# main--/rust-lz-fear

Hardware: AMD Instinct MI355X
Metric: GiB/s compress + decompress, 4 MiB independent blocks, 1/2/4/8 MI355X (higher is better)
Workload: dtype u8

## Files before the change

rust-lz-fear_amd/build.py:

```python
import hashlib
import os
import subprocess
from concurrent.futures import ThreadPoolExecutor

PKG_DIR = os.path.dirname(os.path.abspath(__file__))
CSRC = os.path.join(PKG_DIR, "csrc")
ROOT = os.path.dirname(PKG_DIR)
LIB_PATH = os.environ.get("LZF_LIB_PATH") or os.path.join(PKG_DIR, "liblzfear_hip.so")
ANALYSIS_LIB_PATH = os.path.join(PKG_DIR, "liblzfear_hip_analysis.so")

PRODUCT_HIP = ["capi.hip", "lz4_decompress_batched.hip", "lz4_decompress_paired.hip", "lz4_decompress_seg.hip", "lz4_decompress_fed.hip", "lz4_decoded_size.hip", "lz4_compress.hip",
               "lz4_compress_compact.hip", "lz4_compress_team.hip", "aux_kernels.hip", "frame_device.hip"]
ANALYSIS_HIP = ["analysis/lz4_decompress.hip"]
CXX_SOURCES = ["frame.cpp", "host_staging.cpp"]
HEADERS = ["kernels.h", "lzf_device.h", "lz4_decompress_batch_phase.inc", "lz4_decompress_parse_phase.inc", "lz4_decompress_feed_phase.inc",
           "analysis/capi_analysis.inc",
           "lzf_copy_helpers.h", "lzf_parse_helpers.h", "lzf_compress_common.h", "lzf_simt.h", "lz4_compress_team.inc",
           "host_staging.h", "lzf_frame_scan.h", "frame_jobs.h", "lzf_frame_layout.h", "lzf_size_rules.h", "lzf_chain_step.h", "frame_deliver_body.inc",
           os.path.join(ROOT, "include", "lzfear_hip.h"), os.path.join(ROOT, "include", "lzfear_frame.h")]


def _path(d):
    return d if os.path.isabs(d) else os.path.join(CSRC, d)


def hipcc():
    for c in ("/opt/rocm/bin/hipcc", "hipcc"):
        if os.path.isabs(c) and os.path.exists(c):
            return c
    return "hipcc"


def _sources(analysis):
    return PRODUCT_HIP + (ANALYSIS_HIP if analysis else []) + CXX_SOURCES


def _newest_header():
    return max((os.path.getmtime(_path(h)) for h in HEADERS if os.path.exists(_path(h))), default=0.0)


LAST_BUILD = {}


def build_library(force=False, verbose=False, defines=(), out=None, analysis=False):
    defines = list(defines)
    if (analysis or any(d.startswith("LZF_DBG") for d in defines)) and "LZF_ANALYSIS" not in defines:
        defines.append("LZF_ANALYSIS")
    analysis = "LZF_ANALYSIS" in defines
    extra = sorted(d for d in defines if d != "LZF_ANALYSIS")
    if out is None and extra:
        out = os.path.join(PKG_DIR, "liblzfear_hip_" + hashlib.sha1(" ".join(extra).encode()).hexdigest()[:10] + ".so")
    out = out or (ANALYSIS_LIB_PATH if analysis else LIB_PATH)
    srcs_t = max([os.path.getmtime(_path(s)) for s in _sources(analysis)] + [_newest_header()])
    if not force and os.path.exists(out) and os.path.getmtime(out) >= srcs_t:
        LAST_BUILD[out] = "reused (the library is newer than every source and header)"
        if verbose:
            print(f"[build] {os.path.basename(out)}: {LAST_BUILD[out]}", flush=True)
        return out
    tag = "product" if not defines else hashlib.sha1(" ".join(sorted(defines)).encode()).hexdigest()[:12]
    objdir = os.path.join(PKG_DIR, "_obj", tag)
    os.makedirs(objdir, exist_ok=True)
    hdr_t = _newest_header()
    base = [hipcc(), "--offload-arch=gfx950", "-O3", "-std=c++17", "-fPIC", "-I", os.path.join(ROOT, "include")] + [f"-D{d}" for d in defines]
    jobs = []
    for s in _sources(analysis):
        src = _path(s)
        obj = os.path.join(objdir, os.path.splitext(os.path.basename(s))[0] + ".o")
        stale = force or not os.path.exists(obj) or os.path.getmtime(obj) < max(os.path.getmtime(src), hdr_t)
        jobs.append((src, obj, stale))
    todo = [(s, o) for s, o, st in jobs if st]

    def compile_one(so):
        cmd = base + ["-c", so[0], "-o", so[1]]
        if verbose:
            print(" ".join(cmd), flush=True)
        subprocess.check_call(cmd)

    if todo:
        with ThreadPoolExecutor(max_workers=min(len(todo), os.cpu_count() or 4)) as ex:
            list(ex.map(compile_one, todo))
    objs = [o for _, o, _ in jobs]
    if todo or not os.path.exists(out) or os.path.getmtime(out) < max(os.path.getmtime(o) for o in objs):
        cmd = [hipcc(), "--offload-arch=gfx950", "-shared", "-fPIC", "-o", out] + objs + ["-lpthread"]
        if verbose:
            print(" ".join(cmd), flush=True)
        subprocess.check_call(cmd)
    LAST_BUILD[out] = f"compiled {len(todo)} of {len(jobs)} sources with hipcc --offload-arch=gfx950, linked"
    if verbose:
        print(f"[build] {os.path.basename(out)}: {LAST_BUILD[out]}", flush=True)
    return out


DIST_LIB_PATH = os.path.join(PKG_DIR, "liblzfear_dist.so")


def build_dist_library(force=False, verbose=False):
    core = build_library(force=False, verbose=verbose)
    src = _path("dist_gather.hip")
    deps = [src, os.path.join(ROOT, "include", "lzfear_dist.h"), os.path.join(ROOT, "include", "lzfear_hip.h")]
    out = DIST_LIB_PATH
    if not force and os.path.exists(out) and os.path.getmtime(out) >= max(os.path.getmtime(d) for d in deps):
        LAST_BUILD[out] = "reused (the library is newer than every source and header)"
    else:
        cmd = [hipcc(), "--offload-arch=gfx950", "-O3", "-std=c++17", "-fPIC", "-shared", "-I", os.path.join(ROOT, "include"), "-o", out, src,
               "-L", os.path.dirname(core), "-l:" + os.path.basename(core), "-L", "/opt/rocm/lib", "-lrccl", "-Wl,-rpath,$ORIGIN", "-Wl,-rpath,/opt/rocm/lib"]
        if verbose:
            print(" ".join(cmd), flush=True)
        subprocess.check_call(cmd)
        LAST_BUILD[out] = "compiled dist_gather.hip with hipcc --offload-arch=gfx950, linked against librccl + liblzfear_hip"
    if verbose:
        print(f"[build] {os.path.basename(out)}: {LAST_BUILD[out]}", flush=True)
    return out


def build_analysis_library(force=False, verbose=False):
    return build_library(force=force, verbose=verbose, analysis=True)


if __name__ == "__main__":
    import sys
    print(build_library(force="--force" in sys.argv, verbose=True, analysis="--analysis" in sys.argv))
```

rust-lz-fear_amd/csrc/capi.hip:

```cpp
#include <hip/hip_runtime.h>
#include <cstdio>
#include <cstdlib>
#include <cstring>
#include <string>
#include <mutex>
#include <vector>
#include "kernels.h"
#include "host_staging.h"

namespace {

thread_local std::string g_last_error;
thread_local const char* g_last_decompress = "";
thread_local const char* g_last_compress = "";

int fail_hip(hipError_t e, const char* what) {
    char buf[256];
    snprintf(buf, sizeof buf, "%s: %s", what, hipGetErrorString(e));
    g_last_error = buf;
    return LZF_E_HIP;
}
#define HIP_TRY(expr)                                          \
    do {                                                       \
        hipError_t e__ = (expr);                               \
        if (e__ != hipSuccess) return fail_hip(e__, #expr);    \
    } while (0)
#define LAUNCH(...)                                            \
    do {                                                       \
        hipLaunchKernelGGL(__VA_ARGS__);                       \
        HIP_TRY(hipGetLastError());                            \
    } while (0)

int ensure_device() {
    int n = 0;
    hipError_t e = hipGetDeviceCount(&n);
    if (e != hipSuccess || n <= 0) {
        g_last_error = "no HIP device available (the lz-fear HIP codec has no CPU fallback)";
        (void)hipGetLastError();
        return LZF_E_NO_DEVICE;
    }
    return n;
}

struct Geometry { uint32_t cu, lds, wall_khz; };
const Geometry& geometry() {
    static const Geometry g = [] {
        Geometry r{256u, 160u * 1024u, 100000u};
        hipDeviceProp_t p; int dev = 0;
        if (hipGetDevice(&dev) == hipSuccess && hipGetDeviceProperties(&p, dev) == hipSuccess) {
            r.cu = (uint32_t)p.multiProcessorCount;
            if (p.maxSharedMemoryPerMultiProcessor >= 64u * 1024u) r.lds = (uint32_t)p.maxSharedMemoryPerMultiProcessor;
            int khz = 0;
            if (hipDeviceGetAttribute(&khz, hipDeviceAttributeWallClockRate, dev) == hipSuccess && khz >= 1000) r.wall_khz = (uint32_t)khz; else (void)hipGetLastError();
        } else (void)hipGetLastError();
#ifdef LZF_ANALYSIS
        if (const char* e = getenv("LZF_FAKE_CU")) { const long v = atol(e); if (v >= 1 && v <= 4096) r.cu = (uint32_t)v; }
#endif
        return r;
    }();
    return g;
}
uint32_t cu_count() { return geometry().cu; }
uint32_t per_cu(uint32_t lds_bytes) { const uint32_t n = geometry().lds / lds_bytes; return n ? n : 1u; }

inline size_t align_up(size_t v, size_t a) { return (v + a - 1) / a * a; }

struct AsyncScratch {
    void* p = nullptr; hipStream_t st = nullptr;
    ~AsyncScratch() { if (p) { (void)hipFreeAsync(p, st); } }
    hipError_t release() { void* q = p; p = nullptr; return q ? hipFreeAsync(q, st) : hipSuccess; }
};

void keep_pool_memory() {
    static thread_local int done_for = -1;
    int dev = 0;
    if (hipGetDevice(&dev) != hipSuccess || dev == done_for) return;
    hipMemPool_t pool = nullptr;
    if (hipDeviceGetDefaultMemPool(&pool, dev) == hipSuccess) {
        uint64_t keep = ~0ull;
        (void)hipMemPoolSetAttribute(pool, hipMemPoolAttrReleaseThreshold, &keep);
    }
    (void)hipGetLastError();
    done_for = dev;
}

constexpr auto k_paired48 = lzf::lzf_decompress_paired_kernel<4096, 48, 640>;
constexpr auto k_paired24 = lzf::lzf_decompress_paired_kernel<4096, 24, 384>;
constexpr auto k_staged16 = lzf::lzf_decompress_batched_kernel<4096, 16, 256, true>;
constexpr auto k_compact = lzf::lzf_compress_compact_kernel<false>;
constexpr auto k_compact_dry = lzf::lzf_compress_compact_kernel<true>;
constexpr auto k_general_u32 = lzf::lzf_compress_wave_kernel<LZF_TABLE_U32>;
constexpr auto k_general_u16 = lzf::lzf_compress_wave_kernel<LZF_TABLE_U16>;
constexpr uint32_t kTeamLds = 163840u;
constexpr uint32_t kTeamRounds = 1u;

constexpr uint32_t kSegMaxIn = 4u * 1024u * 1024u + 32u * 1024u;
constexpr uint32_t kSegMinIn = 64u * 1024u;
constexpr uint32_t kSegRingSlack = 8u * 1024u;
inline uint32_t seg_blocks_per_cu(uint32_t ring) { return per_cu(ring + kSegRingSlack); }
constexpr uint32_t kSegRankMax = 1024u;
inline uint32_t seg_max_jobs() { const uint32_t n = seg_blocks_per_cu(32768u) * cu_count(); return n < kSegRankMax ? n : kSegRankMax; }
inline uint32_t seg_ring_for(uint32_t n) {
    return n <= seg_blocks_per_cu(131072u) * cu_count() && geometry().lds >= 131072u + kSegRingSlack ? 131072u
         : n <= seg_blocks_per_cu(65536u) * cu_count() && geometry().lds >= 65536u + kSegRingSlack ? 65536u : 32768u;
}
constexpr uint64_t kSegRecsPerJob = 448u * 1024u;

struct SegScratch {
    void* base = nullptr;
    lzf::seg_ctx ctx{};
    size_t bytes = 0;
    uint32_t* est = nullptr;
};
inline uint32_t seg_nch_host(uint32_t len) { return len <= lzf::kSegChunk ? 1u : 1u + (len - lzf::kSegChunk + lzf::kSegStride - 1u) / lzf::kSegStride; }

bool seg_alloc(SegScratch& s, const lzf_decompress_job* d_jobs, lzf_job_result* d_results, uint32_t n, uint32_t min_in, hipStream_t st, uint64_t max_in_hint = ~0ull) {
    lzf::seg_ctx& c = s.ctx;
    c.jobs = d_jobs; c.results = d_results; c.n_jobs = n;
#ifdef LZF_ANALYSIS
    { static const uint32_t force = [] { const char* e = getenv("LZF_SEG_FORCE"); return !e ? 0u : !strcmp(e, "stager") ? 1u : !strcmp(e, "resolver") ? 2u : !strcmp(e, "noscratch") ? 3u : !strcmp(e, "swait") ? 8u : 0u; }();
      if (force == 3u) return false;
      c.dbg_force = force; }
#endif
    const uint32_t max_in = max_in_hint < kSegMaxIn ? (uint32_t)(max_in_hint < lzf::kSegChunk ? lzf::kSegChunk : max_in_hint) : kSegMaxIn;
    c.max_in = max_in; c.min_in = min_in;
    c.maxch = seg_nch_host(max_in);
    c.maxtile = (max_in + lzf::kSegTile - 1u) / lzf::kSegTile;
    { const uint64_t per_job = (uint64_t)max_in / 3u + 192u; c.rec_cap = (uint64_t)n * (per_job < kSegRecsPerJob ? per_job : kSegRecsPerJob); }
    c.ring_bytes = seg_ring_for(n);
#ifdef LZF_ANALYSIS
    { static const uint32_t ring = [] { const char* e = getenv("LZF_SEG_RING"); return e ? (uint32_t)atol(e) : 0u; }();
      if (ring == 32768u || ring == 65536u || ring == 131072u) c.ring_bytes = ring; }
#endif
    size_t off = 0;
    auto take = [&](size_t bytes) { const size_t o = off; off = align_up(off + bytes, 256); return o; };
    const size_t o_st = take(sizeof(lzf::seg_job) * (size_t)n);
    const size_t o_top = take(sizeof(unsigned long long));
    const size_t o_x = take(sizeof(uint32_t) * (size_t)n * c.maxch);
    const size_t o_vf = take(sizeof(uint32_t) * (size_t)n * c.maxch);
    const size_t o_tt = take(sizeof(uint32_t) * (size_t)n * c.maxtile);
    const size_t o_to = take(sizeof(uint32_t) * (size_t)n * c.maxtile);
    const size_t o_bits = take(sizeof(uint32_t) * (size_t)n * c.maxch * lzf::kSegChunkWords);
    const size_t o_recs = take(sizeof(lzf::u32x4) * (size_t)c.rec_cap);
    const size_t o_ord = take(sizeof(uint32_t) * (size_t)n);
    const size_t o_len = take(sizeof(uint32_t) * (size_t)n);
    const size_t o_est = take(sizeof(uint32_t) * (size_t)n);
    if (hipMallocAsync(&s.base, off, st) != hipSuccess) { (void)hipGetLastError(); s.base = nullptr; return false; }
    s.bytes = off;
    uint8_t* b = static_cast<uint8_t*>(s.base);
    c.st = reinterpret_cast<lzf::seg_job*>(b + o_st);
    c.rec_top = reinterpret_cast<unsigned long long*>(b + o_top);
    c.xexit = reinterpret_cast<uint32_t*>(b + o_x);
    c.vfrom = reinterpret_cast<uint32_t*>(b + o_vf);
    c.tile_tok = reinterpret_cast<uint32_t*>(b + o_tt);
    c.tile_out = reinterpret_cast<uint32_t*>(b + o_to);
    c.bits = reinterpret_cast<uint32_t*>(b + o_bits);
    c.recs = reinterpret_cast<lzf::u32x4*>(b + o_recs);
    c.n_cu = cu_count();
    c.order = (n > c.n_cu && n <= seg_max_jobs()) ? reinterpret_cast<uint32_t*>(b + o_ord) : nullptr;
    c.by_len = (n >= (c.n_cu + 7u) / 8u && n <= seg_max_jobs()) ? reinterpret_cast<uint32_t*>(b + o_len) : nullptr;
    c.rec_by_len = n >= (c.n_cu + 3u) / 4u ? 1u : 0u;
    c.g_off = 0u; c.g_n = n; c.grouped = 0u; c.res_prio = 0u; c.fed = 0u;
    s.est = reinterpret_cast<uint32_t*>(b + o_est);
    return true;
}
inline uint32_t seg_grid(uint32_t target, uint32_t n, uint32_t cap) {
    uint32_t g = target / n; if (g < 1u) g = 1u; if (g > cap) g = cap; return g;
}
int seg_launch_prep(const lzf::seg_ctx& c, hipStream_t st) {
    if (c.by_len && !c.grouped) LAUNCH(lzf::lzf_seg_by_len_kernel, dim3(1), dim3(1024), 0, st, c);
    LAUNCH(lzf::lzf_seg_plan_kernel, dim3((c.n_jobs + 255u) / 256u), dim3(256), 0, st, c);
    return LZF_OK;
}
int seg_launch_front(const lzf::seg_ctx& c, uint32_t upto, hipStream_t st) {
    const uint32_t n = c.g_n;
    uint32_t tg_parse = 1024u * c.n_cu, tg_tile = 2048u * c.n_cu;
#ifdef LZF_ANALYSIS
    { static const char* e = getenv("LZF_SEG_GRID"); if (e) { unsigned a = 0, b = 0; if (sscanf(e, "%u,%u", &a, &b) == 2 && a && b) { tg_parse = a; tg_tile = b; } } }
#endif
    if (upto >= 2) LAUNCH(lzf::lzf_seg_parse_kernel, dim3(seg_grid(tg_parse, n, c.maxch), n), dim3(64), 0, st, c);
    if (upto >= 3) LAUNCH(lzf::lzf_seg_seam_kernel, dim3(n), dim3(64), 0, st, c);
    if (upto >= 4) LAUNCH(lzf::lzf_seg_tilesum_kernel, dim3(seg_grid(tg_tile, n, c.maxtile), n), dim3(64), 0, st, c);
    if (upto >= 5) LAUNCH(lzf::lzf_seg_scan_kernel, dim3(n), dim3(64), 0, st, c);
    if (upto >= 6 && c.order) LAUNCH(lzf::lzf_seg_order_kernel, dim3(1), dim3(1024), 0, st, c);
    if (upto >= 6) LAUNCH(lzf::lzf_seg_records_kernel, dim3(seg_grid(tg_tile, n, c.maxtile), n), dim3(64), 0, st, c);
    return LZF_OK;
}
int seg_launch_records(const lzf::seg_ctx& c, hipStream_t st) {
    const uint32_t n = c.g_n;
    uint32_t tg_tile = 2048u * c.n_cu;
#ifdef LZF_ANALYSIS
    { static const char* e = getenv("LZF_SEG_GRID"); if (e) { unsigned a = 0, b = 0; if (sscanf(e, "%u,%u", &a, &b) == 2 && a && b) tg_tile = b; } }
#endif
    uint32_t pad = 0;
#ifdef LZF_ANALYSIS
    { static const uint32_t e = [] { const char* v = getenv("LZF_SEG_REC_PAD"); return v ? (uint32_t)atol(v) : 0u; }(); pad = e; }
#endif
    LAUNCH(lzf::lzf_seg_records_kernel, dim3(seg_grid(tg_tile, n, c.maxtile), n), dim3(64), pad, st, c);
    return LZF_OK;
}
int seg_launch_resolve(const lzf::seg_ctx& c, hipStream_t st) {
    const uint32_t n = c.g_n;
    if (c.ring_bytes == 131072u) LAUNCH(lzf::lzf_seg_resolve_pair_kernel<131072>, dim3(n), dim3(128), 0, st, c);
    else if (c.ring_bytes == 65536u) LAUNCH(lzf::lzf_seg_resolve_pair_kernel<65536>, dim3(n), dim3(128), 0, st, c);
    else LAUNCH(lzf::lzf_seg_resolve_pair_kernel<32768>, dim3(n), dim3(128), 0, st, c);
    return LZF_OK;
}
int seg_launch(const lzf::seg_ctx& c, uint32_t upto, hipStream_t st) {
    int rc = seg_launch_prep(c, st);
    if (rc == LZF_OK) rc = seg_launch_front(c, upto, st);
    if (rc == LZF_OK && upto >= 8) rc = seg_launch_resolve(c, st);
    return rc;
}

constexpr uint32_t kSegMaxGroups = 4;
struct SegGroups { uint32_t n = 1; uint32_t size[kSegMaxGroups] = {}; };
SegGroups seg_groups(uint32_t n_jobs) {
    SegGroups g; g.size[0] = n_jobs;
    if (n_jobs > seg_max_jobs()) return g;
    const uint32_t ncu = cu_count();
    uint32_t pct[kSegMaxGroups] = {100}; uint32_t k = 1;
    if (n_jobs >= (ncu + 7u) / 8u) { pct[0] = pct[1] = pct[2] = pct[3] = 25; k = 4; }
#ifdef LZF_ANALYSIS
    { static const char* e = getenv("LZF_SEG_GROUPS");
      if (e) { uint32_t v[kSegMaxGroups] = {}, got = 0, sum = 0; const char* q = e;
               while (got < kSegMaxGroups && *q) { char* end = nullptr; const unsigned long x = strtoul(q, &end, 10); if (end == q) break; v[got++] = (uint32_t)x; sum += (uint32_t)x; q = *end == ',' ? end + 1 : end; if (*end != ',') break; }
               if (got >= 1 && sum == 100u && v[0]) { for (uint32_t i = 0; i < kSegMaxGroups; ++i) pct[i] = v[i]; k = got; } } }
#endif
    if (k <= 1u || n_jobs < 2u * k) return g;
    uint32_t left = n_jobs; g.n = 0;
    for (uint32_t i = 0; i < k && left; ++i) {
        uint32_t sz = i + 1u == k ? left : (uint32_t)((uint64_t)n_jobs * pct[i] / 100u);
        if (sz > left) sz = left;
        if (!sz) continue;
        g.size[g.n++] = sz; left -= sz;
    }
    if (left && g.n) g.size[g.n - 1u] += left;
    return g;
}
struct SegLanes {
    std::mutex mu;
    hipStream_t s[kSegMaxGroups - 1u] = {};
    hipEvent_t front[kSegMaxGroups - 1u] = {}, done[kSegMaxGroups - 1u] = {};
    bool ok = false;
};
SegLanes* seg_lanes() {
    constexpr int kMaxDev = 64;
    static std::mutex mu;
    static SegLanes* by_dev[kMaxDev] = {};
    int dev = 0;
    if (hipGetDevice(&dev) != hipSuccess || dev < 0 || dev >= kMaxDev) { (void)hipGetLastError(); return nullptr; }
    std::lock_guard<std::mutex> lk(mu);
    if (!by_dev[dev]) {
        SegLanes* L = new SegLanes();
        int least = 0, greatest = 0;
        if (hipDeviceGetStreamPriorityRange(&least, &greatest) != hipSuccess) { (void)hipGetLastError(); least = greatest = 0; }
        bool ok = true;
        for (uint32_t i = 0; i < kSegMaxGroups - 1u && ok; ++i)
            ok = hipStreamCreateWithPriority(&L->s[i], hipStreamNonBlocking, greatest) == hipSuccess &&
                 hipEventCreateWithFlags(&L->front[i], hipEventDisableTiming) == hipSuccess &&
                 hipEventCreateWithFlags(&L->done[i], hipEventDisableTiming) == hipSuccess;
        if (!ok) (void)hipGetLastError();
        L->ok = ok;
        by_dev[dev] = L;
    }
    return by_dev[dev]->ok ? by_dev[dev] : nullptr;
}
int seg_enqueue_groups(SegScratch& s, const SegGroups& g, SegLanes& L, hipStream_t st) {
    lzf::seg_ctx c = s.ctx;
    std::lock_guard<std::mutex> lk(L.mu);
    int rc = seg_launch_prep(c, st);
    if (rc == LZF_OK) rc = seg_launch_front(c, 5u, st);
    if (rc != LZF_OK) return rc;
    static_assert(kSegMaxGroups == 4, "lzf_seg_rank_kernel takes the group sizes as a uint4");
    LAUNCH(lzf::lzf_seg_rank_kernel, dim3(1), dim3(1024), 0, st, c, s.est, make_uint4(g.size[0], g.n > 1u ? g.size[1] : 0u, g.n > 2u ? g.size[2] : 0u, g.n > 3u ? g.size[3] : 0u));
    c.by_len = s.est; c.grouped = 1u; c.res_prio = 1u;
#ifdef LZF_ANALYSIS
    { static const int pr = [] { const char* e = getenv("LZF_SEG_PRIO"); return e ? atoi(e) : 1; }(); c.res_prio = pr ? 1u : 0u; }
#endif
    uint32_t off = 0, forked = 0;
    const uint32_t ticks_per_us = geometry().wall_khz / 1000u;
    uint32_t pause_ticks = 10u * ticks_per_us;
#ifdef LZF_ANALYSIS
    { static const int us = [] { const char* e = getenv("LZF_SEG_PAUSE_US"); return e ? atoi(e) : -1; }(); if (us >= 0) pause_ticks = (uint32_t)us * ticks_per_us; }
#endif
    for (uint32_t k = 0; k < g.n && rc == LZF_OK; ++k) {
        c.g_off = off; c.g_n = g.size[k]; off += g.size[k];
        rc = seg_launch_records(c, st);
        if (rc != LZF_OK) break;
        if (k + 1u < g.n) {
            if (hipEventRecord(L.front[k], st) != hipSuccess || hipStreamWaitEvent(L.s[k], L.front[k], 0) != hipSuccess) { (void)hipGetLastError(); rc = LZF_E_HIP; break; }
            rc = seg_launch_resolve(c, L.s[k]);
            ++forked;
            if (pause_ticks) LAUNCH(lzf::lzf_seg_pause_kernel, dim3(1), dim3(64), 0, st, pause_ticks);
            if (hipEventRecord(L.done[k], L.s[k]) != hipSuccess) { (void)hipGetLastError(); --forked; if (rc == LZF_OK) rc = LZF_E_HIP; if (hipStreamSynchronize(L.s[k]) != hipSuccess) (void)hipGetLastError(); }
        } else {
            rc = seg_launch_resolve(c, st);
        }
    }
    for (uint32_t k = 0; k < forked; ++k)
        if (hipStreamWaitEvent(st, L.done[k], 0) != hipSuccess) { (void)hipGetLastError(); if (hipStreamSynchronize(L.s[k]) != hipSuccess) (void)hipGetLastError(); if (rc == LZF_OK) rc = LZF_E_HIP; }
    return rc;
}
int seg_launch_grouped(SegScratch& s, const SegGroups& g, SegLanes& L, hipStream_t st) {
    const int rc = seg_enqueue_groups(s, g, L, st);
    if (rc != LZF_OK)
        for (uint32_t k = 0; k < kSegMaxGroups - 1u; ++k) if (hipStreamSynchronize(L.s[k]) != hipSuccess) (void)hipGetLastError();
    return rc;
}
int seg_decompress(const lzf_decompress_job* d_jobs, lzf_job_result* d_results, uint32_t n, uint32_t min_in, hipStream_t st, bool* used, uint64_t max_in_hint, uint32_t* ring_used) {
    SegScratch s;
    *used = false; *ring_used = 0u;
    if (max_in_hint < min_in) return LZF_OK;
    if (!seg_alloc(s, d_jobs, d_results, n, min_in, st, max_in_hint)) return LZF_OK;
    *used = true; *ring_used = s.ctx.ring_bytes;
    const SegGroups g = seg_groups(n);
    SegLanes* lanes = g.n > 1u ? seg_lanes() : nullptr;
    int rc = lanes ? seg_launch_grouped(s, g, *lanes, st) : seg_launch(s.ctx, 8u, st);
    if (rc == LZF_OK) {
        hipLaunchKernelGGL(k_paired48, dim3(n), dim3(128), 0, st, d_jobs, d_results, n, (const uint32_t*)nullptr, (const lzf::seg_job*)s.ctx.st);
        if (hipGetLastError() != hipSuccess) rc = LZF_E_HIP;
    }
    if (hipFreeAsync(s.base, st) != hipSuccess && rc == LZF_OK) rc = LZF_E_HIP;
    if (rc != LZF_OK) g_last_error = "segmented decompress: launch failed";
    return rc;
}

constexpr auto k_fed32 = lzf::lzf_decompress_fed_kernel<4096, 32, 352>;
constexpr uint32_t kFedMinInDefault = 65536u;
constexpr uint64_t kFedMinHint = 262144u;
inline uint32_t fed_min_in() {
#ifdef LZF_ANALYSIS
    static const long v = [] { const char* e = getenv("LZF_FED_MIN_IN"); return e ? atol(e) : -1L; }();
    if (v >= 0) return (uint32_t)v;
#endif
    return kFedMinInDefault;
}
inline uint64_t fed_min_hint() {
#ifdef LZF_ANALYSIS
    static const bool open_ = getenv("LZF_FED_MIN_IN") != nullptr;
    if (open_) return 0u;
#endif
    return kFedMinHint;
}
constexpr uint64_t kFedMaxScratch = 24ull << 30;
constexpr uint32_t kFedMaxJobs = 65535u;
constexpr uint32_t kFedLdsAlloc = 6400u;
constexpr uint32_t kFedWavesPerCu = 4u * (LZF_FED_WAVES > 0 ? (uint32_t)LZF_FED_WAVES : 5u);
struct FedGeometry { uint32_t slots, xcc_mask; };
FedGeometry fed_geometry(hipStream_t st) {
    constexpr int kMaxDev = 64;
    static std::mutex mu;
    static FedGeometry by_dev[kMaxDev] = {};
    int dev = 0;
    if (hipGetDevice(&dev) != hipSuccess || dev < 0 || dev >= kMaxDev) { (void)hipGetLastError(); return FedGeometry{8u * cu_count(), 0u}; }
    std::lock_guard<std::mutex> lk(mu);
    if (by_dev[dev].slots) return by_dev[dev];
    FedGeometry answer{0u, 0u};
    uint32_t* d = nullptr;
    if (hipMalloc(&d, 4u * sizeof(uint32_t)) == hipSuccess) {
        const uint32_t init[4] = {0u, 0xFFFFFFFFu, 0u, 0u};
        lzf::fed_args a{}; a.census = d;
        if (hipMemcpyAsync(d, init, sizeof init, hipMemcpyHostToDevice, st) == hipSuccess) {
            hipLaunchKernelGGL(k_fed32, dim3(40u * cu_count()), dim3(64), 0, st, a);
            uint32_t got[4] = {0, 0, 0, 0};
            if (hipGetLastError() == hipSuccess && hipMemcpyAsync(got, d, sizeof got, hipMemcpyDeviceToHost, st) == hipSuccess && hipStreamSynchronize(st) == hipSuccess &&
                got[1] != 0xFFFFFFFFu && got[1] >= cu_count()) { answer.slots = got[1]; answer.xcc_mask = got[2]; }
        }
        (void)hipFree(d);
    }
    (void)hipGetLastError();
    if (!answer.slots) {
        const uint32_t by_lds = per_cu(kFedLdsAlloc);
        answer.slots = (by_lds < kFedWavesPerCu ? by_lds : kFedWavesPerCu) * cu_count();
    }
#ifdef LZF_ANALYSIS
    if (getenv("LZF_FED_VERBOSE")) fprintf(stderr, "[lzf] bitmap-fed kernel: %u workgroups resident at once (%u compute units), XCD mask 0x%x\n", answer.slots, cu_count(), answer.xcc_mask);
#endif
    by_dev[dev] = answer;
    return answer;
}
struct FedCall {
    SegScratch s; const lzf_decompress_job* jobs = nullptr; lzf_job_result* res = nullptr; uint32_t n = 0; const uint32_t* perm = nullptr;
    size_t o_tick = 0, o_fst = 0; bool live = false;
};
int fed_front(FedCall& f, const lzf_decompress_job* d_jobs, lzf_job_result* d_results, uint32_t n, const uint32_t* perm, hipStream_t st, uint64_t max_in_hint) {
    f.jobs = d_jobs; f.res = d_results; f.n = n; f.perm = perm; f.live = false;
    lzf::seg_ctx& c = f.s.ctx;
    c = lzf::seg_ctx{};
    c.jobs = d_jobs; c.results = d_results; c.n_jobs = n;
    const uint32_t max_in = max_in_hint < kSegMaxIn ? (uint32_t)(max_in_hint < lzf::kSegChunk ? lzf::kSegChunk : max_in_hint) : kSegMaxIn;
    c.max_in = max_in; c.min_in = fed_min_in();
    c.maxch = seg_nch_host(max_in);
    c.maxtile = (max_in + lzf::kSegTile - 1u) / lzf::kSegTile;
    c.n_cu = cu_count();
    c.g_off = 0u; c.g_n = n; c.fed = 1u;
    size_t off = 0;
    auto take = [&](size_t bytes) { const size_t o = off; off = align_up(off + bytes, 256); return o; };
    const size_t o_st = take(sizeof(lzf::seg_job) * (size_t)n);
    const size_t o_top = take(sizeof(unsigned long long));
    const size_t o_x = take(sizeof(uint32_t) * (size_t)n * c.maxch);
    const size_t o_vf = take(sizeof(uint32_t) * (size_t)n * c.maxch);
    const size_t o_bits = take(sizeof(uint32_t) * (size_t)n * c.maxch * lzf::kSegChunkWords);
    f.o_tick = take(sizeof(uint32_t) * 32u * lzf::kFedTicketStride);
    f.o_fst = take(sizeof(lzf::fed_state) * (size_t)n);
    if (off > kFedMaxScratch) return LZF_OK;
    if (hipMallocAsync(&f.s.base, off, st) != hipSuccess) { (void)hipGetLastError(); f.s.base = nullptr; return LZF_OK; }
    uint8_t* b = static_cast<uint8_t*>(f.s.base);
    c.st = reinterpret_cast<lzf::seg_job*>(b + o_st);
    c.rec_top = reinterpret_cast<unsigned long long*>(b + o_top);
    c.xexit = reinterpret_cast<uint32_t*>(b + o_x);
    c.vfrom = reinterpret_cast<uint32_t*>(b + o_vf);
    c.bits = reinterpret_cast<uint32_t*>(b + o_bits);
    f.live = true;
    const int rc = seg_launch(c, 3u, st);
    if (rc != LZF_OK) { (void)hipFreeAsync(f.s.base, st); f.s.base = nullptr; f.live = false; g_last_error = "bitmap-fed decompress: launch failed"; }
    return rc;
}
int fed_back(FedCall& f, hipStream_t st, uint32_t slots_per_cu) {
    if (!f.live) return LZF_OK;
    lzf::seg_ctx& c = f.s.ctx;
    const uint32_t n = f.n;
    uint8_t* b = static_cast<uint8_t*>(f.s.base);
    const FedGeometry fg = fed_geometry(st);
    uint32_t slots = fg.slots;
    if (slots_per_cu && slots_per_cu * cu_count() < slots) slots = slots_per_cu * cu_count();
    uint32_t pieces = n > slots && fg.xcc_mask ? 16u : 1u;
    uint32_t pad = 0;
#ifdef LZF_ANALYSIS
    { static const long e = [] { const char* v = getenv("LZF_FED_PIECES"); return v ? atol(v) : 0L; }(); if (e >= 1 && e <= 4096) pieces = (uint32_t)e; }
    { static const long e = [] { const char* v = getenv("LZF_FED_SLOTS"); return v ? atol(v) : 0L; }(); if (e > 0 && !slots_per_cu) slots = (uint32_t)e * cu_count(); }
    { static const uint32_t e = [] { const char* v = getenv("LZF_FED_PAD_LDS"); return v ? (uint32_t)atol(v) : 0u; }(); pad = e; }
#endif
    if ((uint64_t)n * pieces > 0xFFFFFFF0ull) pieces = 1u;
    if (!fg.xcc_mask) pieces = 1u;
    int rc = LZF_OK;
    lzf::fed_args a{f.jobs, f.res, c.st, c.bits, c.vfrom, f.perm, reinterpret_cast<lzf::fed_state*>(b + f.o_fst), reinterpret_cast<uint32_t*>(b + f.o_tick), fg.xcc_mask ? fg.xcc_mask : 1u, n, c.maxch, pieces, nullptr};
    hipLaunchKernelGGL(lzf::lzf_fed_reset_kernel, dim3((n + 255u) / 256u), dim3(256), 0, st, a);
    hipLaunchKernelGGL(k_fed32, dim3(slots < n ? slots : n), dim3(64), pad, st, a);
    if (hipGetLastError() != hipSuccess) rc = LZF_E_HIP;
    if (rc == LZF_OK) {
        hipLaunchKernelGGL(k_paired24, dim3(n), dim3(128), 0, st, f.jobs, f.res, n, f.perm, (const lzf::seg_job*)c.st);
        if (hipGetLastError() != hipSuccess) rc = LZF_E_HIP;
    }
    if (hipFreeAsync(f.s.base, st) != hipSuccess && rc == LZF_OK) rc = LZF_E_HIP;
    f.s.base = nullptr; f.live = false;
    if (rc != LZF_OK) g_last_error = "bitmap-fed decompress: launch failed";
    return rc;
}
int fed_decompress(const lzf_decompress_job* d_jobs, lzf_job_result* d_results, uint32_t n, const uint32_t* perm, hipStream_t st, bool* used, uint64_t max_in_hint) {
    *used = false;
    if (n > kFedMaxJobs || max_in_hint <= fed_min_in() || max_in_hint <= fed_min_hint()) return LZF_OK;
    FedCall f;
    int rc = fed_front(f, d_jobs, d_results, n, perm, st, max_in_hint);
    if (rc != LZF_OK || !f.live) return rc;
    *used = true;
    return fed_back(f, st, 0u);
}

#ifdef LZF_ANALYSIS
#include "analysis/capi_analysis.inc"
#endif

}

extern "C" {

int lzf_abi_version(void) { return LZFEAR_ABI_VERSION; }
const char* lzf_last_error(void) { return g_last_error.c_str(); }
const char* lzf_last_decompress_launch(void) { return g_last_decompress; }
const char* lzf_last_compress_launch(void) { return g_last_compress; }
int lzf_device_count(void) { return ensure_device(); }

int lzf_compress_batch(const lzf_compress_job* d_jobs, lzf_job_result* d_results, uint32_t n_jobs,
                       uint32_t table_kinds, void* hip_stream) {
    if (n_jobs == 0) return LZF_OK;
    if (!d_jobs || !d_results) { g_last_error = "lzf_compress_batch: NULL job/result array"; return LZF_E_INVALID; }
    int rc = ensure_device();
    if (rc < 0) return rc;
    hipStream_t st = static_cast<hipStream_t>(hip_stream);
    keep_pool_memory();
    if ((table_kinds & (LZF_KINDS_U32 | LZF_KINDS_U16)) == 0) table_kinds |= LZF_KINDS_U32 | LZF_KINDS_U16;
    uint32_t use_compact = 1u, use_order = 1u;
    uint32_t team_max = geometry().lds >= kTeamLds ? kTeamRounds * cu_count() : 0u;
#ifdef LZF_ANALYSIS
    { static const uint32_t which = [] { const char* e = getenv("LZF_COMPRESS_KERNEL"); return !e ? 0u : !strcmp(e, "general") ? 1u : !strcmp(e, "compact") ? 3u : 0u; }();
      static const uint32_t order = analysis_order("LZF_COMPRESS_ORDER");
      use_compact = which == 1u ? 0u : 1u; use_order = order;
      static const long tm = [] { const char* e = getenv("LZF_COMPRESS_TEAM_MAX"); return e ? atol(e) : -1L; }();
      if (tm >= 0 && geometry().lds >= kTeamLds) team_max = (uint32_t)tm;
      if (which != 0u) team_max = 0u; }
#endif
    const bool use_team = use_compact && n_jobs <= team_max;
    const bool fresh_only = use_compact && (table_kinds & LZF_KINDS_U32_FRESH_ONLY);
    uint32_t* perm = nullptr;
    AsyncScratch scratch_owner; scratch_owner.st = st;
    void*& scratch = scratch_owner.p;
    const bool want_order = use_order && use_compact && (table_kinds & LZF_KINDS_U32) && (use_order == 2u || n_jobs > per_cu(lzf::kCompactLdsBytes) * cu_count() || (fresh_only && n_jobs > 4u * cu_count()));
    uint32_t piece = 65536u, parts = 1u;
#ifdef LZF_ANALYSIS
    { static const char* e = getenv("LZF_PROBE"); if (e) { unsigned a = 0, b = 0; if (sscanf(e, "%u,%u", &a, &b) == 2 && a >= 4096u && b >= 1u && b <= 16u) { piece = a; parts = b; } } }
#endif
    const size_t n_probes = want_order ? (size_t)n_jobs * parts : 0u;
    const size_t probes_off = 256;
    const size_t res_off = probes_off + align_up(sizeof(lzf_compress_job) * n_probes, 256);
    const size_t perm_off = res_off + align_up(sizeof(lzf_job_result) * n_probes, 256);
    if (want_order) {
        if (hipMallocAsync(&scratch, perm_off + sizeof(uint32_t) * (want_order ? (size_t)n_jobs : 0u), st) != hipSuccess) { (void)hipGetLastError(); scratch = nullptr; }
    }
    if (scratch && want_order) {
        lzf_compress_job* probes = reinterpret_cast<lzf_compress_job*>(static_cast<uint8_t*>(scratch) + probes_off);
        lzf_job_result* pres = reinterpret_cast<lzf_job_result*>(static_cast<uint8_t*>(scratch) + res_off);
        perm = reinterpret_cast<uint32_t*>(static_cast<uint8_t*>(scratch) + perm_off);
        LAUNCH(lzf::lzf_cost_probe_jobs_kernel, dim3((uint32_t)((n_probes + 255u) / 256u)), dim3(256), 0, st, d_jobs, probes, n_jobs, piece, parts);
        LAUNCH(k_compact_dry, dim3((uint32_t)n_probes), dim3(64), 0, st, probes, pres, (uint32_t)n_probes, (const uint32_t*)nullptr, 0u);
        LAUNCH(lzf::lzf_order_by_cost_kernel, dim3(1), dim3(1024), 0, st, d_jobs, pres, perm, n_jobs, piece, parts);
    }
    if (table_kinds & LZF_KINDS_U32) {
#ifdef LZF_DBG_DRY_MAIN
        if (use_compact) LAUNCH(k_compact_dry, dim3(n_jobs), dim3(64), 0, st, d_jobs, d_results, n_jobs, (const uint32_t*)perm, 0u);
#else
        if (use_team) {
            LAUNCH(lzf::lzf_compress_team_kernel, dim3(n_jobs), dim3(192), 0, st, d_jobs, d_results, n_jobs, (const uint32_t*)perm, fresh_only ? 1u : 0u);
            if (!fresh_only) LAUNCH(lzf::lzf_compress_team_carry_kernel, dim3(n_jobs), dim3(192), 0, st, d_jobs, d_results, n_jobs, (const uint32_t*)perm);
        }
        else if (use_compact) {
            uint32_t pad = 0;
#ifdef LZF_ANALYSIS
            { static const uint32_t e = [] { const char* v = getenv("LZF_COMPACT_PAD_LDS"); return v ? (uint32_t)atol(v) : 0u; }(); pad = e; }
#endif
            LAUNCH(k_compact, dim3(n_jobs), dim3(64), pad, st, d_jobs, d_results, n_jobs, (const uint32_t*)perm, fresh_only ? 1u : 0u);
        }
#endif
        if (!fresh_only) LAUNCH(k_general_u32, dim3(n_jobs), dim3(64), 0, st, d_jobs, d_results, n_jobs, use_team ? 2u : use_compact, (const uint32_t*)perm);
    }
    if (table_kinds & LZF_KINDS_U16)
        LAUNCH(k_general_u16, dim3(n_jobs), dim3(64), 0, st, d_jobs, d_results, n_jobs, 0u, (const uint32_t*)perm);
    g_last_compress = !(table_kinds & LZF_KINDS_U32) ? "lzf_compress_wave_kernel<U16>"
                    : !use_compact ? "lzf_compress_wave_kernel (analysis: general)"
                    : use_team ? (fresh_only ? "lzf_compress_team_kernel" : "lzf_compress_team_kernel + lzf_compress_team_carry_kernel + lzf_compress_wave_kernel")
                               : (fresh_only ? "lzf_compress_compact_kernel" : "lzf_compress_compact_kernel + lzf_compress_wave_kernel");
    HIP_TRY(scratch_owner.release());
    return LZF_OK;
}

int lzf_decompress_batch(const lzf_decompress_job* d_jobs, lzf_job_result* d_results, uint32_t n_jobs, void* hip_stream) {
    return lzf_decompress_batch_sized(d_jobs, d_results, n_jobs, ~0ull, hip_stream);
}

int lzf_decompress_batch_sized(const lzf_decompress_job* d_jobs, lzf_job_result* d_results, uint32_t n_jobs, uint64_t max_input_len, void* hip_stream) {
    if (n_jobs == 0) return LZF_OK;
    if (!d_jobs || !d_results) { g_last_error = "lzf_decompress_batch: NULL job/result array"; return LZF_E_INVALID; }
    int rc = ensure_device();
    if (rc < 0) return rc;
    hipStream_t st = static_cast<hipStream_t>(hip_stream);
    keep_pool_memory();
    uint32_t use_order = 1u;
    bool perm_ok = true;
#ifdef LZF_ANALYSIS
    const int forced = analysis_decompress_variant();
    { static const uint32_t order = analysis_order("LZF_DECOMPRESS_ORDER"); use_order = order; }
    if (forced != kVariantAuto) perm_ok = analysis_perm_ok(forced);
#endif
    AsyncScratch perm_owner; perm_owner.st = st;
    uint32_t* perm = nullptr;
    if (perm_ok && (use_order == 2u || (use_order == 1u && n_jobs > per_cu(20u * 1024u) * cu_count()))) {
        if (hipMallocAsync(&perm_owner.p, 2u * sizeof(uint32_t) * (size_t)n_jobs, st) != hipSuccess) { (void)hipGetLastError(); perm_owner.p = nullptr; }
        perm = static_cast<uint32_t*>(perm_owner.p);
        if (perm) {
            uint32_t* const est = perm + n_jobs;
            uint32_t len_shift = 2u;
#ifdef LZF_ANALYSIS
            { static const uint32_t k = [] { const char* e = getenv("LZF_ORDER_LEN_SHIFT"); return e ? (uint32_t)atol(e) : 2u; }(); len_shift = k; }
#endif
            LAUNCH(lzf::lzf_decompress_cost_kernel, dim3(n_jobs), dim3(64), 0, st, d_jobs, n_jobs, est, len_shift);
            LAUNCH(lzf::lzf_order_by_estimate_kernel, dim3(1), dim3(1024), 0, st, (const uint32_t*)est, perm, n_jobs);
        }
    }
    const uint32_t* cperm = perm;
#ifdef LZF_ANALYSIS
    if (forced != kVariantAuto) {
        g_last_decompress = "analysis variant (LZF_DECOMPRESS_KERNEL)";
        rc = analysis_launch_decompress(forced, d_jobs, d_results, n_jobs, cperm, st);
        HIP_TRY(perm_owner.release());
        return rc;
    }
#endif
    uint32_t seg_min_in = kSegMinIn; bool seg_on = n_jobs <= seg_max_jobs();
#ifdef LZF_ANALYSIS
    { static const int mode = [] { const char* e = getenv("LZF_DECOMPRESS_KERNEL"); return !e ? 0 : !strcmp(e, "seg") ? 1 : (!strcmp(e, "noseg") || !strcmp(e, "fed")) ? 2 : 0; }();
      static const uint32_t min_in = [] { const char* e = getenv("LZF_SEG_MIN_IN"); return e ? (uint32_t)atol(e) : 0u; }();
      if (mode == 1) { seg_on = true; seg_min_in = min_in; }
      if (mode == 2) seg_on = false; }
#endif
    if (seg_on) {
        bool used = false; uint32_t ring = 0;
        rc = seg_decompress(d_jobs, d_results, n_jobs, seg_min_in, st, &used, max_input_len, &ring);
        if (used) g_last_decompress = ring == 131072u ? "segmented: lzf_seg_resolve_pair_kernel<131072> + lzf_decompress_paired_kernel<4096,48,640>"
                                     : ring == 65536u ? "segmented: lzf_seg_resolve_pair_kernel<65536> + lzf_decompress_paired_kernel<4096,48,640>"
                                                      : "segmented: lzf_seg_resolve_pair_kernel<32768> + lzf_decompress_paired_kernel<4096,48,640>";
        if (rc != LZF_OK || used) { HIP_TRY(perm_owner.release()); return rc; }
    }
    const uint32_t resident48 = per_cu(20u * 1024u) * cu_count();
    const uint32_t resident24 = per_cu(12800u) * cu_count();
    bool fed_on = n_jobs > resident24;
#ifdef LZF_ANALYSIS
    { static const int mode = [] { const char* e = getenv("LZF_DECOMPRESS_KERNEL"); return !e ? 0 : !strcmp(e, "fed") ? 1 : !strcmp(e, "nofed") ? 2 : 0; }();
      if (mode == 1) fed_on = true;
      if (mode == 2) fed_on = false; }
#endif
    if (fed_on) {
        bool used = false;
        rc = fed_decompress(d_jobs, d_results, n_jobs, cperm, st, &used, max_input_len);
        if (used) g_last_decompress = "bitmap-fed: lzf_seg_parse_kernel + lzf_decompress_fed_kernel<4096,32,352> + lzf_decompress_paired_kernel<4096,24,384>";
        if (rc != LZF_OK || used) { HIP_TRY(perm_owner.release()); return rc; }
    }
    g_last_decompress = n_jobs <= resident48 ? "lzf_decompress_paired_kernel<4096,48,640>" : n_jobs <= 8u * resident48 ? "lzf_decompress_paired_kernel<4096,24,384>"
                                                                                                             : "lzf_decompress_batched_kernel<4096,16,256,staged>";
    if (n_jobs <= resident48)
        LAUNCH(k_paired48, dim3(n_jobs), dim3(128), 0, st, d_jobs, d_results, n_jobs, cperm, (const lzf::seg_job*)nullptr);
    else if (n_jobs <= 8u * resident48)
        LAUNCH(k_paired24, dim3(n_jobs), dim3(128), 0, st, d_jobs, d_results, n_jobs, cperm, (const lzf::seg_job*)nullptr);
    else
        LAUNCH(k_staged16, dim3(n_jobs), dim3(64), 0, st, d_jobs, d_results, n_jobs, cperm);
    HIP_TRY(perm_owner.release());
    return LZF_OK;
}

int lzf_decompressed_size_batch(const lzf_decompress_job* d_jobs, lzf_job_result* d_results, uint32_t n_jobs, uint64_t max_input_len, void* hip_stream) {
    (void)max_input_len;
    if (n_jobs == 0) return LZF_OK;
    if (!d_jobs || !d_results) { g_last_error = "lzf_decompressed_size_batch: NULL job/result array"; return LZF_E_INVALID; }
    int rc = ensure_device();
    if (rc < 0) return rc;
    hipStream_t st = static_cast<hipStream_t>(hip_stream);
    keep_pool_memory();
    constexpr auto k_size = lzf::lzf_decoded_size_kernel<48, 768>;
    static thread_local int resident_for = -1; static thread_local uint32_t resident = 0;
    int dev = 0;
    HIP_TRY(hipGetDevice(&dev));
    if (dev != resident_for) {
        int per = 0;
        HIP_TRY(hipOccupancyMaxActiveBlocksPerMultiprocessor(&per, k_size, 64, 0));
        resident = per > 0 ? (uint32_t)per : 1u; resident_for = dev;
    }
    const uint64_t room = (uint64_t)resident * cu_count();
    const bool ordered = n_jobs > room;
    AsyncScratch ticket; ticket.st = st;
    HIP_TRY(hipMallocAsync(&ticket.p, 256 + (ordered ? sizeof(uint32_t) * (size_t)n_jobs : 0u), st));
    HIP_TRY(hipMemsetAsync(ticket.p, 0, 4, st));
    uint32_t* const perm = ordered ? static_cast<uint32_t*>(ticket.p) + 64 : nullptr;
    if (ordered) LAUNCH(lzf::lzf_order_by_input_len_kernel, dim3(1), dim3(1024), 0, st, d_jobs, perm, n_jobs);
    const uint32_t grid = n_jobs < room ? n_jobs : (uint32_t)room;
    LAUNCH(k_size, dim3(grid), dim3(64), 0, st, d_jobs, d_results, n_jobs, static_cast<uint32_t*>(ticket.p), (const uint32_t*)perm);
    HIP_TRY(ticket.release());
    return LZF_OK;
}

int lzf_table_seed_from_dictionary(lzf_u32_table* d_table, const uint8_t* d_dict, uint64_t dict_len, void* hip_stream) {
    if (!d_table || (!d_dict && dict_len)) { g_last_error = "lzf_table_seed_from_dictionary: NULL argument"; return LZF_E_INVALID; }
    if (dict_len > 0xFFFFFFFFull) { g_last_error = "dictionary beyond u32 positions (reference panics, mod.rs:67)"; return LZF_E_INVALID; }
    int rc = ensure_device();
    if (rc < 0) return rc;
    hipStream_t st = static_cast<hipStream_t>(hip_stream);
    HIP_TRY(hipMemsetAsync(d_table, 0, sizeof(lzf_u32_table), st));
    if (dict_len >= 8) {
        const uint64_t count = (dict_len - 8) / 3 + 1;
        uint32_t blocks = (uint32_t)((count + 255) / 256);
        if (blocks > 1024) blocks = 1024;
        hipLaunchKernelGGL(lzf::lzf_seed_table_kernel, dim3(blocks), dim3(256), 0, st, d_table, d_dict, dict_len);
        HIP_TRY(hipGetLastError());
    }
    return LZF_OK;
}

int lzf_table_offset(void* d_table, uint32_t table_kind, uint64_t add, void* hip_stream) {
    if (!d_table || table_kind > LZF_TABLE_U16) { g_last_error = "lzf_table_offset: bad argument"; return LZF_E_INVALID; }
    int rc = ensure_device();
    if (rc < 0) return rc;
    hipLaunchKernelGGL(lzf::lzf_table_offset_kernel, dim3(1), dim3(64), 0, static_cast<hipStream_t>(hip_stream), d_table, table_kind, add);
    HIP_TRY(hipGetLastError());
    return LZF_OK;
}

int lzf_table_offset_batch(void* const* d_tables, const uint64_t* d_adds, uint32_t n, uint32_t table_kind, void* hip_stream) {
    if (n == 0) return LZF_OK;
    if (!d_tables || !d_adds || table_kind > LZF_TABLE_U16) { g_last_error = "lzf_table_offset_batch: bad argument"; return LZF_E_INVALID; }
    int rc = ensure_device();
    if (rc < 0) return rc;
    hipLaunchKernelGGL(lzf::lzf_table_offset_batch_kernel, dim3((n + 255u) / 256u), dim3(256), 0, static_cast<hipStream_t>(hip_stream), d_tables, d_adds, n, table_kind);
    HIP_TRY(hipGetLastError());
    return LZF_OK;
}

int lzf_chain_decompress_step(const lzf_chain_step* d_steps, lzf_chain_state* d_state, uint32_t n_streams,
                              lzf_decompress_job* d_jobs, const lzf_job_result* d_results, void* hip_stream) {
    if (n_streams == 0) return LZF_OK;
    if (!d_steps || !d_state || !d_jobs || !d_results) { g_last_error = "lzf_chain_decompress_step: NULL argument"; return LZF_E_INVALID; }
    int rc = ensure_device();
    if (rc < 0) return rc;
    hipLaunchKernelGGL(lzf::lzf_chain_decompress_step_kernel, dim3(n_streams), dim3(256), 0, static_cast<hipStream_t>(hip_stream), d_steps, d_state, n_streams, d_jobs, d_results);
    HIP_TRY(hipGetLastError());
    return LZF_OK;
}

int lzf_copy_ranges(const uint8_t* const* d_src, uint8_t* const* d_dst, const uint64_t* d_len, uint32_t n, uint64_t max_len, void* hip_stream) {
    if (n == 0 || max_len == 0) return LZF_OK;
    if (!d_src || !d_dst || !d_len) { g_last_error = "lzf_copy_ranges: NULL argument"; return LZF_E_INVALID; }
    int rc = ensure_device();
    if (rc < 0) return rc;
    const uint64_t pieces = (max_len + 65535ull) / 65536ull;
    if (pieces > 0x7FFFFFFFull) { g_last_error = "lzf_copy_ranges: max_len too large"; return LZF_E_INVALID; }
    for (uint32_t base = 0; base < n; base += 65535u) {
        const uint32_t cnt = n - base < 65535u ? n - base : 65535u;
        hipLaunchKernelGGL(lzf::lzf_copy_ranges_kernel, dim3((uint32_t)pieces, cnt), dim3(256), 0, static_cast<hipStream_t>(hip_stream),
                           d_src + base, d_dst + base, d_len + base, cnt);
    }
    HIP_TRY(hipGetLastError());
    return LZF_OK;
}

int lzf_xxh32_batch(const uint8_t* const* d_ptrs, const uint64_t* d_lens, uint32_t* d_out, uint32_t n, void* hip_stream) {
    if (n == 0) return LZF_OK;
    if (!d_ptrs || !d_lens || !d_out) { g_last_error = "lzf_xxh32_batch: NULL argument"; return LZF_E_INVALID; }
    int rc = ensure_device();
    if (rc < 0) return rc;
    if (n <= 8192u) hipLaunchKernelGGL(lzf::lzf_xxh32_wave_kernel, dim3(n), dim3(64), 0, static_cast<hipStream_t>(hip_stream), d_ptrs, d_lens, d_out, n);
    else hipLaunchKernelGGL(lzf::lzf_xxh32_kernel, dim3((n + 15) / 16), dim3(64), 0, static_cast<hipStream_t>(hip_stream), d_ptrs, d_lens, d_out, n);
    HIP_TRY(hipGetLastError());
    return LZF_OK;
}

#ifdef LZF_ANALYSIS
int lzf_debug_seg(const lzf_decompress_job* d_jobs, lzf_job_result* d_results, uint32_t n, uint32_t min_in, uint32_t upto,
                  void* h_state, void* h_bits, void* h_xexit, void* h_vfrom, void* h_tile_tok, void* h_tile_out, void* h_recs, uint64_t recs_bytes,
                  uint32_t* geom) {
    int rc = ensure_device();
    if (rc < 0) return rc;
    SegScratch s;
    if (!seg_alloc(s, d_jobs, d_results, n, min_in, nullptr)) return LZF_E_HIP;
    const lzf::seg_ctx& c = s.ctx;
    rc = seg_launch(c, upto, nullptr);
    HIP_TRY(hipDeviceSynchronize());
    if (geom) { geom[0] = c.maxch; geom[1] = c.maxtile; geom[2] = lzf::kSegChunkWords; geom[3] = (uint32_t)c.rec_cap; }
    if (h_state) HIP_TRY(hipMemcpy(h_state, c.st, sizeof(lzf::seg_job) * n, hipMemcpyDeviceToHost));
    if (h_bits) HIP_TRY(hipMemcpy(h_bits, c.bits, sizeof(uint32_t) * (size_t)n * c.maxch * lzf::kSegChunkWords, hipMemcpyDeviceToHost));
    if (h_xexit) HIP_TRY(hipMemcpy(h_xexit, c.xexit, sizeof(uint32_t) * (size_t)n * c.maxch, hipMemcpyDeviceToHost));
    if (h_vfrom) HIP_TRY(hipMemcpy(h_vfrom, c.vfrom, sizeof(uint32_t) * (size_t)n * c.maxch, hipMemcpyDeviceToHost));
    if (h_tile_tok) HIP_TRY(hipMemcpy(h_tile_tok, c.tile_tok, sizeof(uint32_t) * (size_t)n * c.maxtile, hipMemcpyDeviceToHost));
    if (h_tile_out) HIP_TRY(hipMemcpy(h_tile_out, c.tile_out, sizeof(uint32_t) * (size_t)n * c.maxtile, hipMemcpyDeviceToHost));
    if (h_recs) { uint64_t nb = sizeof(lzf::u32x4) * c.rec_cap; if (nb > recs_bytes) nb = recs_bytes; HIP_TRY(hipMemcpy(h_recs, c.recs, nb, hipMemcpyDeviceToHost)); }
    HIP_TRY(hipFree(s.base));
    return rc;
}
#endif

int lzf_compress_batch_host(const lzf_compress_job* jobs, lzf_job_result* results, uint32_t n_jobs) {
    if (n_jobs == 0) return LZF_OK;
    if (!jobs || !results) { g_last_error = "lzf_compress_batch_host: NULL argument"; return LZF_E_INVALID; }
    int rc = ensure_device();
    if (rc < 0) return rc;
    using lzf_host::Seg; using lzf_host::Staging;
    std::vector<size_t> in_off(n_jobs), out_off(n_jobs), tab_off(n_jobs);
    size_t in_total = 0, out_total = 0;
    uint32_t kinds = 0;
    std::vector<Seg> up;
    static_assert(sizeof(lzf_u32_table) == sizeof(lzf_u16_table), "table structs share a slab slot size");
    for (uint32_t i = 0; i < n_jobs; ++i) {
        if (jobs[i].table_kind > LZF_TABLE_U16) { g_last_error = "bad table_kind"; return LZF_E_INVALID; }
        kinds |= jobs[i].table_kind == LZF_TABLE_U32 ? LZF_KINDS_U32 : LZF_KINDS_U16;
        in_off[i] = in_total; in_total = align_up(in_total + jobs[i].input_len, 256);
        if (jobs[i].input_len) up.push_back({in_off[i], const_cast<uint8_t*>(jobs[i].input), (size_t)jobs[i].input_len});
    }
    for (uint32_t i = 0; i < n_jobs; ++i) {
        tab_off[i] = in_total;
        if (jobs[i].table) { up.push_back({tab_off[i], static_cast<uint8_t*>(jobs[i].table), sizeof(lzf_u32_table)}); in_total = align_up(in_total + sizeof(lzf_u32_table), 256); }
    }
    for (uint32_t i = 0; i < n_jobs; ++i) { out_off[i] = out_total; out_total = align_up(out_total + jobs[i].out_cap, 256); }
    Staging& sg = Staging::get();
    std::lock_guard<std::mutex> guard(sg.lock());
    hipStream_t cs = sg.stream(0);
    uint8_t* const din = static_cast<uint8_t*>(sg.device(0, in_total));
    uint8_t* const dout = static_cast<uint8_t*>(sg.device(1, out_total));
    lzf_compress_job* const djobs = static_cast<lzf_compress_job*>(sg.device(3, sizeof(lzf_compress_job) * n_jobs));
    lzf_job_result* const dres = static_cast<lzf_job_result*>(sg.device(4, sizeof(lzf_job_result) * n_jobs));
    if (!cs || !din || !dout || !djobs || !dres || !sg.pinned(in_total > out_total ? in_total : out_total)) return fail_hip(hipErrorOutOfMemory, "staging memory");
    std::vector<lzf_compress_job> dj(jobs, jobs + n_jobs);
    for (uint32_t i = 0; i < n_jobs; ++i) {
        dj[i].input = din + in_off[i];
        dj[i].out = dout + out_off[i];
        if (jobs[i].table) dj[i].table = din + tab_off[i];
    }
    HIP_TRY(sg.upload(up, in_total, din));
    HIP_TRY(hipMemcpyAsync(djobs, dj.data(), sizeof(lzf_compress_job) * n_jobs, hipMemcpyHostToDevice, cs));
    HIP_TRY(sg.join_copies(cs));
    rc = lzf_compress_batch(djobs, dres, n_jobs, kinds, cs);
    if (rc != LZF_OK) { (void)hipDeviceSynchronize(); return rc; }
    HIP_TRY(hipMemcpyAsync(results, dres, sizeof(lzf_job_result) * n_jobs, hipMemcpyDeviceToHost, cs));
    HIP_TRY(hipStreamSynchronize(cs));
    std::vector<Seg> down;
    for (uint32_t i = 0; i < n_jobs; ++i) {
        if (results[i].status == LZF_OK && results[i].out_len) down.push_back({out_off[i], jobs[i].out, (size_t)results[i].out_len});
        if (jobs[i].table && !(jobs[i].flags & LZF_CJOB_TABLE_READONLY) && results[i].status != LZF_CONTRACT)
            HIP_TRY(hipMemcpyAsync(jobs[i].table, din + tab_off[i], sizeof(lzf_u32_table), hipMemcpyDeviceToHost, cs));
    }
    HIP_TRY(sg.download(down, out_total, dout, cs));
    HIP_TRY(hipStreamSynchronize(cs));
    return LZF_OK;
}

int lzf_decompress_batch_host(const lzf_decompress_job* jobs, lzf_job_result* results, uint32_t n_jobs) {
    if (n_jobs == 0) return LZF_OK;
    if (!jobs || !results) { g_last_error = "lzf_decompress_batch_host: NULL argument"; return LZF_E_INVALID; }
    int rc = ensure_device();
    if (rc < 0) return rc;
    using lzf_host::Seg; using lzf_host::Staging;
    std::vector<size_t> in_off(n_jobs), pre_off(n_jobs), out_off(n_jobs);
    size_t in_total = 0, out_total = 0;
    std::vector<Seg> up, up_out;
    for (uint32_t i = 0; i < n_jobs; ++i) {
        if (jobs[i].out_existing_len > jobs[i].out_cap) { g_last_error = "out_existing_len > out_cap"; return LZF_E_INVALID; }
        in_off[i] = in_total; in_total = align_up(in_total + jobs[i].input_len, 256);
        if (jobs[i].input_len) up.push_back({in_off[i], const_cast<uint8_t*>(jobs[i].input), (size_t)jobs[i].input_len});
    }
    for (uint32_t i = 0; i < n_jobs; ++i) {
        pre_off[i] = in_total; in_total = align_up(in_total + jobs[i].prefix_len, 256);
        if (jobs[i].prefix_len) up.push_back({pre_off[i], const_cast<uint8_t*>(jobs[i].prefix), (size_t)jobs[i].prefix_len});
    }
    for (uint32_t i = 0; i < n_jobs; ++i) {
        out_off[i] = out_total; out_total = align_up(out_total + jobs[i].out_cap, 256);
        if (jobs[i].out_existing_len) up_out.push_back({out_off[i], jobs[i].out, (size_t)jobs[i].out_existing_len});
    }
    Staging& sg = Staging::get();
    std::lock_guard<std::mutex> guard(sg.lock());
    hipStream_t cs = sg.stream(0);
    uint8_t* const din = static_cast<uint8_t*>(sg.device(0, in_total));
    uint8_t* const dout = static_cast<uint8_t*>(sg.device(1, out_total));
    lzf_decompress_job* const djobs = static_cast<lzf_decompress_job*>(sg.device(3, sizeof(lzf_decompress_job) * n_jobs));
    lzf_job_result* const dres = static_cast<lzf_job_result*>(sg.device(4, sizeof(lzf_job_result) * n_jobs));
    if (!cs || !din || !dout || !djobs || !dres || !sg.pinned(in_total > out_total ? in_total : out_total)) return fail_hip(hipErrorOutOfMemory, "staging memory");
    std::vector<lzf_decompress_job> dj(jobs, jobs + n_jobs);
    for (uint32_t i = 0; i < n_jobs; ++i) {
        dj[i].input = din + in_off[i];
        dj[i].prefix = din + pre_off[i];
        dj[i].out = dout + out_off[i];
    }
    if (!up_out.empty()) {
        HIP_TRY(sg.upload(up_out, out_total, dout));
        HIP_TRY(sg.join_copies(cs));
        HIP_TRY(hipStreamSynchronize(cs));
    }
    HIP_TRY(sg.upload(up, in_total, din));
    HIP_TRY(hipMemcpyAsync(djobs, dj.data(), sizeof(lzf_decompress_job) * n_jobs, hipMemcpyHostToDevice, cs));
    HIP_TRY(sg.join_copies(cs));
    uint64_t max_in = 0;
    for (uint32_t i = 0; i < n_jobs; ++i) if (jobs[i].input_len > max_in) max_in = jobs[i].input_len;
    rc = lzf_decompress_batch_sized(djobs, dres, n_jobs, max_in, cs);
    if (rc != LZF_OK) { (void)hipDeviceSynchronize(); return rc; }
    HIP_TRY(hipMemcpyAsync(results, dres, sizeof(lzf_job_result) * n_jobs, hipMemcpyDeviceToHost, cs));
    HIP_TRY(hipStreamSynchronize(cs));
    std::vector<Seg> down;
    for (uint32_t i = 0; i < n_jobs; ++i) {
        uint64_t n = results[i].out_len;
        if (n > jobs[i].out_cap) n = jobs[i].out_cap;
        if (n > jobs[i].out_existing_len)
            down.push_back({out_off[i] + (size_t)jobs[i].out_existing_len, jobs[i].out + jobs[i].out_existing_len, (size_t)(n - jobs[i].out_existing_len)});
    }
    HIP_TRY(sg.download(down, out_total, dout, cs));
    return LZF_OK;
}

int lzf_decompressed_size_batch_host(const lzf_decompress_job* jobs, lzf_job_result* results, uint32_t n_jobs) {
    if (n_jobs == 0) return LZF_OK;
    if (!jobs || !results) { g_last_error = "lzf_decompressed_size_batch_host: NULL argument"; return LZF_E_INVALID; }
    int rc = ensure_device();
    if (rc < 0) return rc;
    using lzf_host::Seg; using lzf_host::Staging;
    std::vector<size_t> in_off(n_jobs);
    size_t in_total = 0;
    uint64_t max_in = 0;
    std::vector<Seg> up;
    for (uint32_t i = 0; i < n_jobs; ++i) {
        in_off[i] = in_total; in_total = align_up(in_total + jobs[i].input_len, 256);
        if (jobs[i].input_len) {
            if (!jobs[i].input) { g_last_error = "lzf_decompressed_size_batch_host: NULL input"; return LZF_E_INVALID; }
            up.push_back({in_off[i], const_cast<uint8_t*>(jobs[i].input), (size_t)jobs[i].input_len});
        }
        if (jobs[i].input_len > max_in) max_in = jobs[i].input_len;
    }
    Staging& sg = Staging::get();
    std::lock_guard<std::mutex> guard(sg.lock());
    hipStream_t cs = sg.stream(0);
    uint8_t* const din = static_cast<uint8_t*>(sg.device(0, in_total ? in_total : 256));
    lzf_decompress_job* const djobs = static_cast<lzf_decompress_job*>(sg.device(3, sizeof(lzf_decompress_job) * n_jobs));
    lzf_job_result* const dres = static_cast<lzf_job_result*>(sg.device(4, sizeof(lzf_job_result) * n_jobs));
    if (!cs || !din || !djobs || !dres || !sg.pinned(in_total ? in_total : 256)) return fail_hip(hipErrorOutOfMemory, "staging memory");
    std::vector<lzf_decompress_job> dj(jobs, jobs + n_jobs);
    for (uint32_t i = 0; i < n_jobs; ++i) dj[i].input = din + in_off[i];
    HIP_TRY(sg.upload(up, in_total, din));
    HIP_TRY(hipMemcpyAsync(djobs, dj.data(), sizeof(lzf_decompress_job) * n_jobs, hipMemcpyHostToDevice, cs));
    HIP_TRY(sg.join_copies(cs));
    rc = lzf_decompressed_size_batch(djobs, dres, n_jobs, max_in, cs);
    if (rc != LZF_OK) { (void)hipDeviceSynchronize(); return rc; }
    HIP_TRY(hipMemcpyAsync(results, dres, sizeof(lzf_job_result) * n_jobs, hipMemcpyDeviceToHost, cs));
    HIP_TRY(hipStreamSynchronize(cs));
    return LZF_OK;
}

int lzf_table_replace_host(void* table, uint32_t table_kind, const uint8_t* input, uint64_t input_len, uint64_t pos, uint64_t* previous) {
    if (!table || (!input && input_len) || table_kind > LZF_TABLE_U16) { g_last_error = "lzf_table_replace_host: bad argument"; return LZF_E_INVALID; }
    if (pos > input_len) return LZF_CONTRACT;
    const uint64_t rem = input_len - pos;
    if (table_kind == LZF_TABLE_U32) {
        lzf_u32_table* t = static_cast<lzf_u32_table*>(table);
        const uint64_t o = pos + t->offset;
        if (o > 0xFFFFFFFFull || o < pos) return LZF_CONTRACT;
        uint64_t v = 0;
        if (rem >= 8) memcpy(&v, input + pos, 8);
        const uint32_t slot = (uint32_t)(((v << 24) * 889523592379ull) >> 52);
        const uint32_t old = t->dict[slot];
        t->dict[slot] = (uint32_t)o;
        if (previous) *previous = old > t->offset ? old - t->offset : 0;
    } else {
        lzf_u16_table* t = static_cast<lzf_u16_table*>(table);
        const uint64_t o = pos + t->offset;
        if (o > 0xFFFFull || o < pos) return LZF_CONTRACT;
        if (rem < 4) return LZF_CONTRACT;
        uint32_t v; memcpy(&v, input + pos, 4);
        const uint32_t slot = (uint32_t)(v * 2654435761u) >> 19;
        const uint16_t old = t->dict[slot];
        t->dict[slot] = (uint16_t)o;
        if (previous) *previous = old > t->offset ? old - t->offset : 0;
    }
    return LZF_OK;
}

int lzf_table_offset_host(void* table, uint32_t table_kind, uint64_t add) {
    if (!table || table_kind > LZF_TABLE_U16) { g_last_error = "lzf_table_offset_host: bad argument"; return LZF_E_INVALID; }
    if (table_kind == LZF_TABLE_U32) static_cast<lzf_u32_table*>(table)->offset += add;
    else static_cast<lzf_u16_table*>(table)->offset += add;
    return LZF_OK;
}

int lzf_compress2_host_writer(const uint8_t* input, uint64_t input_len, uint64_t cursor, void* table, uint32_t table_kind,
                              lzf_write_all_fn write_all, void* ctx, int* writer_error) {
    if ((!input && input_len) || !write_all || table_kind > LZF_TABLE_U16) { g_last_error = "lzf_compress2_host_writer: bad argument"; return LZF_E_INVALID; }
    if (writer_error) *writer_error = 0;
    const uint64_t payload = cursor < input_len ? input_len - cursor : 0;
    const uint64_t bound = payload + payload / 255 + 16;
    std::vector<uint8_t> out(bound);
    static_assert(sizeof(lzf_u32_table) == sizeof(lzf_u16_table), "one scratch copy serves both table kinds");
    std::vector<uint8_t> t0(sizeof(lzf_u32_table), 0), t1;
    if (table) memcpy(t0.data(), table, t0.size());
    t1 = t0;
    lzf_compress_job job{};
    job.input = input; job.input_len = input_len; job.cursor = cursor;
    job.out = out.data(); job.out_cap = bound; job.table = table ? t1.data() : nullptr; job.table_kind = table_kind;
    lzf_job_result res{};
    int rc = lzf_compress_batch_host(&job, &res, 1);
    if (rc != LZF_OK) return rc;
    if (res.status != LZF_OK) return res.status;
    const uint8_t* p = out.data();
    const uint8_t* const end = p + res.out_len;
    int werr = 0;
    auto put = [&](const uint8_t* d, size_t n) -> bool { if (n == 0) return true; werr = write_all(ctx, d, n); return werr == 0; };
    auto put_tail = [&](const uint8_t*& q) -> bool {
        size_t k = 0; while (q[k] == 0xFF) ++k;
        for (size_t i = 0; i < k / 4; ++i) { if (!put(q, 4)) return false; q += 4; }
        for (size_t i = 0; i < k % 4; ++i) { if (!put(q, 1)) return false; q += 1; }
        if (!put(q, 1)) return false;
        q += 1;
        return true;
    };
    bool refused = false;
    const uint8_t* group = p;
    while (p < end && !refused) {
        group = p;
        const uint8_t tok = *p;
        const uint8_t* q = p + 1;
        if (!put(p, 1)) { refused = true; break; }
        size_t L = tok >> 4;
        if (L == 15) { const uint8_t* t = q; while (*t == 0xFF) { L += 255; ++t; } L += *t; if (!put_tail(q)) { refused = true; break; } }
        if (!put(q, L)) { refused = true; break; }
        q += L;
        if (q >= end) { p = q; break; }
        if (!put(q, 2)) { refused = true; break; }
        q += 2;
        if ((tok & 15) == 15) { if (!put_tail(q)) { refused = true; break; } }
        p = q;
    }
    if (!refused) {
        if (table) memcpy(table, t1.data(), t1.size());
        return LZF_OK;
    }
    if (writer_error) *writer_error = werr;
    if (table) {
        const uint8_t* q = group; const uint8_t tok = *q++; size_t L = tok >> 4;
        if (L == 15) { while (*q == 0xFF) { L += 255; ++q; } L += *q++; }
        q += L;
        if (q < end) { q += 2; if ((tok & 15) == 15) { while (*q == 0xFF) ++q; ++q; } }
        const uint64_t gsize = (uint64_t)(q - group);
        t1 = t0;
        job.out_cap = (uint64_t)(group - out.data()) + gsize - 1;
        job.table = t1.data();
        rc = lzf_compress_batch_host(&job, &res, 1);
        if (rc != LZF_OK) return rc;
        memcpy(table, t1.data(), t1.size());
    }
    return LZF_OUTPUT_FULL;
}

int lzf_xxh32_batch_host(const uint8_t* const* ptrs, const uint64_t* lens, uint32_t* out, uint32_t n) {
    if (n == 0) return LZF_OK;
    if (!ptrs || !lens || !out) { g_last_error = "lzf_xxh32_batch_host: NULL argument"; return LZF_E_INVALID; }
    int rc = ensure_device();
    if (rc < 0) return rc;
    using lzf_host::Seg; using lzf_host::Staging;
    std::vector<Seg> up; std::vector<const uint8_t*> dp(n);
    size_t total = 0;
    for (uint32_t i = 0; i < n; ++i) { if (lens[i]) up.push_back({total, const_cast<uint8_t*>(ptrs[i]), (size_t)lens[i]}); dp[i] = reinterpret_cast<const uint8_t*>(total); total = align_up(total + lens[i], 256); }
    Staging& sg = Staging::get();
    std::lock_guard<std::mutex> guard(sg.lock());
    hipStream_t cs = sg.stream(0);
    uint8_t* const din = static_cast<uint8_t*>(sg.device(0, total));
    const size_t lp = 0, ll = align_up(sizeof(void*) * n, 256), lo = ll + align_up(sizeof(uint64_t) * n, 256);
    uint8_t* const dl = static_cast<uint8_t*>(sg.device(5, lo + sizeof(uint32_t) * n));
    if (!cs || !din || !dl || !sg.pinned(total)) return fail_hip(hipErrorOutOfMemory, "staging memory");
    for (uint32_t i = 0; i < n; ++i) dp[i] = din + reinterpret_cast<size_t>(dp[i]);
    HIP_TRY(sg.upload(up, total, din));
    HIP_TRY(hipMemcpyAsync(dl + lp, dp.data(), sizeof(void*) * n, hipMemcpyHostToDevice, cs));
    HIP_TRY(hipMemcpyAsync(dl + ll, lens, sizeof(uint64_t) * n, hipMemcpyHostToDevice, cs));
    HIP_TRY(sg.join_copies(cs));
    rc = lzf_xxh32_batch(reinterpret_cast<const uint8_t* const*>(dl + lp), reinterpret_cast<const uint64_t*>(dl + ll), reinterpret_cast<uint32_t*>(dl + lo), n, cs);
    if (rc != LZF_OK) { (void)hipDeviceSynchronize(); return rc; }
    HIP_TRY(hipMemcpyAsync(out, dl + lo, sizeof(uint32_t) * n, hipMemcpyDeviceToHost, cs));
    HIP_TRY(hipStreamSynchronize(cs));
    return LZF_OK;
}

}
```

rust-lz-fear_amd/csrc/kernels.h:

```cpp
#pragma once
#include "lzf_device.h"

namespace lzf {
#ifdef LZF_ANALYSIS
__global__ void lzf_decompress_wave_kernel(const lzf_decompress_job* __restrict__ jobs,
                                           lzf_job_result* __restrict__ results, uint32_t n_jobs, const uint32_t* __restrict__ perm);
#endif
template <int RING, int S, int TOKCAP, bool STAGE>
__global__ __launch_bounds__(64) void lzf_decompress_batched_kernel(const lzf_decompress_job* __restrict__ jobs,
                                              lzf_job_result* __restrict__ results, uint32_t n_jobs, const uint32_t* __restrict__ perm);
#ifdef LZF_ANALYSIS
#define LZF_DECOMPRESS_VARIANTS(X) \
    X(staged16, 4096, 16, 256, true)    \
    X(staged32, 4096, 32, 512, true)    \
    X(direct4w, 4096, 256, 2048, false)
#else
#define LZF_DECOMPRESS_VARIANTS(X) X(staged16, 4096, 16, 256, true)
#endif
#define LZF_EXT(NAME, R, S_, T, ST) extern template __global__ void lzf_decompress_batched_kernel<R, S_, T, ST>(const lzf_decompress_job*, lzf_job_result*, uint32_t, const uint32_t*);
LZF_DECOMPRESS_VARIANTS(LZF_EXT)
#undef LZF_EXT
template <int S, int TOKCAP>
__global__ __launch_bounds__(64) void lzf_decoded_size_kernel(const lzf_decompress_job* __restrict__ jobs, lzf_job_result* __restrict__ results,
                                                              uint32_t n_jobs, uint32_t* __restrict__ ticket, const uint32_t* __restrict__ perm);
extern template __global__ void lzf_decoded_size_kernel<48, 768>(const lzf_decompress_job*, lzf_job_result*, uint32_t, uint32_t*, const uint32_t*);
struct seg_job;
template <int RING, int S, int TOKCAP>
__global__ __launch_bounds__(128) void lzf_decompress_paired_kernel(const lzf_decompress_job* __restrict__ jobs, lzf_job_result* __restrict__ results, uint32_t n_jobs,
                                             const uint32_t* __restrict__ perm, const seg_job* __restrict__ done);
#ifdef LZF_ANALYSIS
#define LZF_PAIRED_VARIANTS(X) \
    X(paired16, 4096, 16, 256) \
    X(paired24, 4096, 24, 384) \
    X(paired48, 4096, 48, 640) \
    X(paired128, 4096, 128, 1280) \
    X(paired256, 4096, 256, 2048)
#else
#define LZF_PAIRED_VARIANTS(X) \
    X(paired24, 4096, 24, 384) \
    X(paired48, 4096, 48, 640)
#endif
#define LZF_EXTP(NAME, RG, S_, T) extern template __global__ void lzf_decompress_paired_kernel<RG, S_, T>(const lzf_decompress_job*, lzf_job_result*, uint32_t, const uint32_t*, const seg_job*);
LZF_PAIRED_VARIANTS(LZF_EXTP)
#undef LZF_EXTP
struct seg_job {
    uint32_t eligible, failed, done, nch;
    uint32_t ntile, ntok, outb, pad;
    uint64_t rec_off;
    uint64_t pad2;
};
struct seg_ctx {
    const lzf_decompress_job* jobs;
    lzf_job_result* results;
    seg_job* st;
    uint32_t* bits;
    uint32_t* xexit;
    uint32_t* vfrom;
    uint32_t* tile_tok;
    uint32_t* tile_out;
    u32x4* recs;
    unsigned long long* rec_top;
    uint64_t rec_cap;
    uint32_t n_jobs, maxch, maxtile, max_in, min_in;
    uint32_t ring_bytes;
    uint32_t* order;
    uint32_t n_cu;
    uint32_t* by_len;
    uint32_t rec_by_len;
    uint32_t dbg_force;
    uint32_t g_off, g_n, grouped;
    uint32_t res_prio;
    uint32_t fed;
};
struct fed_state { uint32_t flag, cstart, expect, o; };
constexpr uint32_t kFedEnded = 0x80000000u;
constexpr uint32_t kFedTicketStride = 32u;
struct fed_args {
    const lzf_decompress_job* jobs;
    lzf_job_result* results;
    seg_job* st;
    const uint32_t* bits;
    const uint32_t* vfrom;
    const uint32_t* perm;
    fed_state* state;
    uint32_t* ticket;
    uint32_t xcc_mask;
    uint32_t n_jobs, maxch;
    uint32_t pieces;
    uint32_t* census;
};
__global__ void lzf_fed_reset_kernel(fed_args a);
#define LZF_FED_VARIANTS(X) X(fed32, 4096, 32, 352)
#ifdef LZF_DBG_FED_WAVES
#define LZF_FED_WAVES LZF_DBG_FED_WAVES
#else
#define LZF_FED_WAVES 6
#endif
#if LZF_FED_WAVES > 0
#define LZF_FED_BOUNDS __launch_bounds__(64, LZF_FED_WAVES)
#else
#define LZF_FED_BOUNDS __launch_bounds__(64)
#endif
template <int RING, int W, int TOKCAP>
__global__ LZF_FED_BOUNDS void lzf_decompress_fed_kernel(fed_args a);
#define LZF_EXTF(NAME, RG, W_, T) extern template __global__ void lzf_decompress_fed_kernel<RG, W_, T>(fed_args);
LZF_FED_VARIANTS(LZF_EXTF)
#undef LZF_EXTF
__device__ __forceinline__ uint32_t seg_job_of(const seg_ctx& c, uint32_t i) { return c.by_len ? c.by_len[i + c.g_off] : i + c.g_off; }
constexpr uint32_t kSegRegion = 256, kSegChunk = 64u * kSegRegion, kSegOverlap = 2048, kSegStride = kSegChunk - kSegOverlap;
constexpr uint32_t kSegChunkWords = kSegChunk / 32u, kSegTile = 2048;
__global__ void lzf_seg_plan_kernel(seg_ctx c);
__global__ void lzf_seg_order_kernel(seg_ctx c);
__global__ void lzf_seg_pause_kernel(uint32_t ticks);
__global__ void lzf_seg_rank_kernel(seg_ctx c, uint32_t* __restrict__ by_tok, uint4 group_sizes);
__global__ void lzf_seg_by_len_kernel(seg_ctx c);
__global__ void lzf_seg_parse_kernel(seg_ctx c);
__global__ void lzf_seg_seam_kernel(seg_ctx c);
__global__ void lzf_seg_tilesum_kernel(seg_ctx c);
__global__ void lzf_seg_scan_kernel(seg_ctx c);
__global__ void lzf_seg_records_kernel(seg_ctx c);
template <int R>
__global__ __launch_bounds__(128) void lzf_seg_resolve_pair_kernel(seg_ctx c);
extern template __global__ void lzf_seg_resolve_pair_kernel<32768>(seg_ctx);
extern template __global__ void lzf_seg_resolve_pair_kernel<65536>(seg_ctx);
extern template __global__ void lzf_seg_resolve_pair_kernel<131072>(seg_ctx);
template <int KIND>
__global__ __launch_bounds__(64) void lzf_compress_wave_kernel(const lzf_compress_job* __restrict__ jobs,
                                         lzf_job_result* __restrict__ results, uint32_t n_jobs, uint32_t skip_compact,
                                         const uint32_t* __restrict__ perm);
extern template __global__ void lzf_compress_wave_kernel<LZF_TABLE_U32>(const lzf_compress_job*, lzf_job_result*, uint32_t, uint32_t, const uint32_t*);
extern template __global__ void lzf_compress_wave_kernel<LZF_TABLE_U16>(const lzf_compress_job*, lzf_job_result*, uint32_t, uint32_t, const uint32_t*);
constexpr uint32_t kCompactLdsBytes = (4096u / 2u + 4096u / 32u + 64u) * 4u;
template <bool DRY>
__global__ __launch_bounds__(64) void lzf_compress_compact_kernel(const lzf_compress_job* __restrict__ jobs,
                                            lzf_job_result* __restrict__ results, uint32_t n_jobs, const uint32_t* __restrict__ perm,
                                            uint32_t alone);
extern template __global__ void lzf_compress_compact_kernel<false>(const lzf_compress_job*, lzf_job_result*, uint32_t, const uint32_t*, uint32_t);
extern template __global__ void lzf_compress_compact_kernel<true>(const lzf_compress_job*, lzf_job_result*, uint32_t, const uint32_t*, uint32_t);
__global__ void lzf_compress_team_kernel(const lzf_compress_job* __restrict__ jobs, lzf_job_result* __restrict__ results, uint32_t n_jobs,
                                         const uint32_t* __restrict__ perm, uint32_t alone);
__global__ void lzf_compress_team_carry_kernel(const lzf_compress_job* __restrict__ jobs, lzf_job_result* __restrict__ results, uint32_t n_jobs, const uint32_t* __restrict__ perm);
__global__ void lzf_cost_probe_jobs_kernel(const lzf_compress_job* __restrict__ jobs, lzf_compress_job* __restrict__ probes, uint32_t n,
                                           uint32_t piece, uint32_t parts);
__global__ void lzf_order_by_input_len_kernel(const lzf_decompress_job* __restrict__ jobs, uint32_t* __restrict__ perm, uint32_t n);
__global__ void lzf_decompress_cost_kernel(const lzf_decompress_job* __restrict__ jobs, uint32_t n, uint32_t* __restrict__ est, uint32_t len_shift);
__global__ void lzf_order_by_estimate_kernel(const uint32_t* __restrict__ est, uint32_t* __restrict__ perm, uint32_t n);
__global__ void lzf_order_by_cost_kernel(const lzf_compress_job* __restrict__ jobs, const lzf_job_result* __restrict__ probe_results,
                                         uint32_t* __restrict__ perm, uint32_t n, uint32_t piece, uint32_t parts);
__global__ void lzf_xxh32_kernel(const uint8_t* const* __restrict__ ptrs, const uint64_t* __restrict__ lens,
                                 uint32_t* __restrict__ out, uint32_t n);
__global__ void lzf_xxh32_wave_kernel(const uint8_t* const* __restrict__ ptrs, const uint64_t* __restrict__ lens,
                                      uint32_t* __restrict__ out, uint32_t n);
__global__ void lzf_copy_ranges_kernel(const uint8_t* const* __restrict__ src, uint8_t* const* __restrict__ dst,
                                       const uint64_t* __restrict__ len, uint32_t n);
__global__ void lzf_seed_table_kernel(lzf_u32_table* __restrict__ t, const uint8_t* __restrict__ dict, uint64_t dict_len);
__global__ void lzf_table_offset_kernel(void* table, uint32_t kind, uint64_t add);
__global__ void lzf_table_offset_batch_kernel(void* const* __restrict__ tables, const uint64_t* __restrict__ adds, uint32_t n, uint32_t kind);
__global__ void lzf_chain_decompress_step_kernel(const lzf_chain_step* __restrict__ steps, lzf_chain_state* __restrict__ state, uint32_t n,
                                                 lzf_decompress_job* __restrict__ jobs, const lzf_job_result* __restrict__ results);
}
```

rust-lz-fear_amd/csrc/lz4_decompress_fed.hip:

```cpp
#include "lzf_device.h"
#include "kernels.h"
#include "lzf_copy_helpers.h"

namespace lzf {

__device__ __forceinline__ uint32_t xcc_id() {
    uint32_t v; asm volatile("s_getreg_b32 %0, hwreg(HW_REG_XCC_ID)" : "=s"(v)); return v & 15u;
}

template <int RING, int W, int TOKCAP>
__global__ LZF_FED_BOUNDS void lzf_decompress_fed_kernel(fed_args a) {
    constexpr bool STAGE = true;
    constexpr uint32_t kMask = RING - 1;
    constexpr uint32_t kSpanMax = RING / 3;
    constexpr uint32_t kNearHist = RING - kSpanMax;
    constexpr uint32_t kRound = 32u * (uint32_t)W;
    constexpr uint32_t kCB = kRound + 128u;
    static_assert(W >= 1 && W <= 64 && (kSegTile % kRound) == 0, "a round is one bit-map word per lane and subdivides a tile");
    static_assert(TOKCAP >= (int)(kRound / 3u + 1u), "a round's tokens (at least three bytes each) fit the list");
    static_assert(kCB % 16 == 0, "the round is staged in 16-byte pieces");
    __shared__ __attribute__((aligned(16))) uint8_t ring[RING];
    __shared__ __attribute__((aligned(16))) uint8_t cbuf[kCB];
    __shared__ __attribute__((aligned(16))) uint16_t toks[TOKCAP];

    const uint32_t lane = threadIdx.x;
    if (a.census) {
        if (lane == 0u) {
            __hip_atomic_fetch_or(&a.census[2], 1u << (xcc_id() & 31u), __ATOMIC_RELAXED, __HIP_MEMORY_SCOPE_AGENT);
            __hip_atomic_fetch_add(&a.census[0], 1u, __ATOMIC_RELAXED, __HIP_MEMORY_SCOPE_AGENT);
            const unsigned long long t0 = wall_clock64();
            while (wall_clock64() - t0 < 30000ull) __builtin_amdgcn_s_sleep(16);
            const uint32_t seen = __hip_atomic_load(&a.census[0], __ATOMIC_RELAXED, __HIP_MEMORY_SCOPE_AGENT);
            __hip_atomic_fetch_min(&a.census[1], seen, __ATOMIC_RELAXED, __HIP_MEMORY_SCOPE_AGENT);
        }
        return;
    }
    const uint32_t n = a.n_jobs, pieces = a.pieces;
    const uint32_t xcc = xcc_id() & 31u;
    if (pieces > 1u && !((a.xcc_mask >> xcc) & 1u)) return;
    const uint32_t ng = pieces > 1u ? (uint32_t)__popc(a.xcc_mask) : 1u, g = pieces > 1u ? (uint32_t)__popc(a.xcc_mask & ((1u << xcc) - 1u)) : 0u;
    const uint32_t n_g = n > g ? (n - g + ng - 1u) / ng : 0u;
    const uint32_t n_tickets = n_g * pieces;
    for (;;) {
    uint32_t tk = 0;
    if (lane == 0u) tk = __hip_atomic_fetch_add(a.ticket + g * kFedTicketStride, 1u, __ATOMIC_RELAXED, __HIP_MEMORY_SCOPE_AGENT);
    tk = __builtin_amdgcn_readfirstlane(tk);
    if (tk >= n_tickets) break;
    const uint32_t piece = tk / n_g, k = (tk - piece * n_g) * ng + g;
    const uint32_t jid = a.perm ? a.perm[k] : k;
    const seg_job sj = a.st[jid];
    if (!sj.eligible || sj.failed || sj.done) continue;
    LZF_GLOBAL fed_state* const fs = (LZF_GLOBAL fed_state*)a.state + jid;
    const lzf_decompress_job job = a.jobs[jid];
    const long long t_start = clock64();
#ifdef LZF_DBG_TIMELINE
    const unsigned long long t_wall0 = wall_clock64();
#endif

    int status = LZF_OK;
    bool bailed = false, parked = false;
    uint32_t o = 0;
#ifdef LZF_DBG_PHASE_SEL
    long long ph_acc_out = 0;
#endif
    if (job.input_len >= kMaxPosB || job.out_existing_len >= kMaxPosB || job.prefix_len >= kMaxPosB || job.out_existing_len > job.out_cap) continue;
    {
        cgu8* __restrict__ in = as_global(job.input);
        cgu8* __restrict__ prefix = as_global(job.prefix);
        gu8* out = as_global(job.out);
        const uint32_t len = (uint32_t)job.input_len;
        const uint32_t plen = (uint32_t)job.prefix_len;
        const uint32_t cap = job.out_cap > kMaxPosB ? kMaxPosB : (uint32_t)job.out_cap;
        const uint64_t limit = job.output_limit;
        const uint32_t rb = (uint32_t)(reinterpret_cast<uintptr_t>(out) & 15u);
        const uint32_t ring_a = lds_addr(ring), cbuf_a = lds_addr(cbuf);
        const LZF_GLOBAL uint32_t* const fed_bits = (const LZF_GLOBAL uint32_t*)a.bits + (size_t)jid * a.maxch * kSegChunkWords;
        const LZF_GLOBAL uint32_t* const fed_vf = (const LZF_GLOBAL uint32_t*)a.vfrom + (size_t)jid * a.maxch;
#define RIDX(x) (((x) + rb) & kMask)

        auto ring_fill = [&](uint32_t a_, uint32_t b) {
            uint32_t nh = (16u - ((a_ + rb) & 15u)) & 15u; if (nh > b - a_) nh = b - a_;
            if (lane < nh) ring[RIDX(a_ + lane)] = out[a_ + lane];
            a_ += nh;
            const uint32_t nchunks = (b - a_) >> 4;
            for (uint32_t c = lane; c < nchunks; c += kWave)
                *reinterpret_cast<u32x4*>(&ring[RIDX(a_ + 16u * c)]) = *reinterpret_cast<const LZF_GLOBAL u32x4*>(out + a_ + 16u * c);
            a_ += nchunks << 4;
            if (lane < b - a_) ring[RIDX(a_ + lane)] = out[a_ + lane];
        };
        auto ring_flush = [&](uint32_t a_, uint32_t b) {
            uint32_t nh = (16u - ((a_ + rb) & 15u)) & 15u; if (nh > b - a_) nh = b - a_;
            if (lane < nh) out[a_ + lane] = ring[RIDX(a_ + lane)];
            a_ += nh;
            const uint32_t nchunks = (b - a_) >> 4;
            for (uint32_t c = lane; c < nchunks; c += kWave)
                *reinterpret_cast<LZF_GLOBAL u32x4*>(out + a_ + 16u * c) = *reinterpret_cast<const u32x4*>(&ring[RIDX(a_ + 16u * c)]);
            a_ += nchunks << 4;
            if (lane < b - a_) out[a_ + lane] = ring[RIDX(a_ + lane)];
        };

        uint32_t expect = 0;
        uint32_t cstart = 0;
        o = (uint32_t)job.out_existing_len;
        const uint32_t rounds = (len + kRound - 1u) / kRound, per = (rounds + pieces - 1u) / pieces;
        const uint32_t piece_end = (piece + 1u) * per >= rounds ? len : (piece + 1u) * per * kRound;
        if (piece > 0u) {
            uint32_t f = 0;
            for (uint32_t spin = 0; spin < (1u << 22); ++spin) {
                f = __hip_atomic_load(&fs->flag, __ATOMIC_RELAXED, __HIP_MEMORY_SCOPE_AGENT);
                if (f >= piece) break;
                __builtin_amdgcn_s_sleep(32);
            }
            f = __builtin_amdgcn_readfirstlane(f);
            if (f != piece) continue;
            __builtin_amdgcn_fence(__ATOMIC_ACQUIRE, "agent");
            cstart = fs->cstart; expect = fs->expect; o = fs->o;
        }
        uint32_t safe = o;
        if (o > 0) ring_fill(o > (uint32_t)RING ? o - RING : 0u, o);
#ifdef LZF_DBG_PHASE_SEL
        long long ph_t = clock64(), ph_acc = 0;
#define PHASE(i) do { const long long tn__ = clock64(); if ((i) == LZF_DBG_PHASE_SEL) ph_acc += tn__ - ph_t; ph_t = tn__; } while (0)
#else
#define PHASE(i) do { } while (0)
#endif
        while (cstart < len && expect < len && status == LZF_OK) {
            if (cstart >= piece_end) { parked = true; break; }
            __syncthreads();
#include "lz4_decompress_feed_phase.inc"
            if (Tc) {
#define LZF_FED_DECODE
#ifdef LZF_FED_FAR_LATE
#define LZF_FAR_LATE
#endif
#include "lz4_decompress_batch_phase.inc"
#undef LZF_FAR_LATE
#undef LZF_FED_DECODE
            }
            if (bail) { bailed = true; break; }
            const uint32_t nx = expect & ~(kRound - 1u);
            cstart = nx > cstart ? nx : cstart + kRound;
        }
        if (!parked && status == LZF_OK && expect < len) bailed = true;
#ifdef LZF_DBG_PHASE_SEL
        ph_acc_out = ph_acc;
#endif
#undef PHASE
#undef RIDX
        if (parked && status == LZF_OK && !bailed) {
            if (lane == 0u) { fs->cstart = cstart; fs->expect = expect; fs->o = o; }
            __builtin_amdgcn_fence(__ATOMIC_RELEASE, "workgroup");
            asm volatile("s_waitcnt vmcnt(0)" ::: "memory");
            if (lane == 0u) __hip_atomic_store(&fs->flag, piece + 1u, __ATOMIC_RELAXED, __HIP_MEMORY_SCOPE_AGENT);
            continue;
        }
    }
    if (pieces > 1u && lane == 0u) __hip_atomic_store(&fs->flag, kFedEnded, __ATOMIC_RELAXED, __HIP_MEMORY_SCOPE_AGENT);
    if (bailed || status != LZF_OK) continue;
    if (lane == 0) {
        a.results[jid].out_len = o;
        a.results[jid].status = LZF_OK;
#ifdef LZF_DBG_PHASE_SEL
        a.results[jid].reserved = (uint32_t)(ph_acc_out >> 10);
#elif defined(LZF_DBG_TIMELINE)
        a.results[jid].reserved = (uint32_t)(((t_wall0 >> 8) & 0xFFFFull) << 16) | (uint32_t)((wall_clock64() >> 8) & 0xFFFFull);
#else
        a.results[jid].reserved = (uint32_t)((clock64() - t_start) >> 10);
#endif
        a.st[jid].done = 1u;
    }
    }
}

__global__ __launch_bounds__(256) void lzf_fed_reset_kernel(fed_args a) {
    const uint32_t k = blockIdx.x * blockDim.x + threadIdx.x;
    if (k < 32u) a.ticket[k * kFedTicketStride] = 0u;
    if (k < a.n_jobs) a.state[k].flag = 0u;
}

#define LZF_INSTF(NAME, RG, W_, T) template __global__ void lzf_decompress_fed_kernel<RG, W_, T>(fed_args);
LZF_FED_VARIANTS(LZF_INSTF)
#undef LZF_INSTF

}
```

rust-lz-fear_amd/csrc/lz4_decompress_feed_phase.inc:

```
            uint32_t Tc = 0;
            bool bail = false;
            auto rdb = [&](uint32_t q) -> uint32_t {
                const uint32_t r = q - cstart;
                if (r < kCB) return lds_ld8(cbuf_a + r);
                return (uint32_t)in[q];
            };
            if (expect < cstart + kRound) {
                {
                    const uint32_t avail = len - cstart < kCB ? len - cstart : kCB;
                    cgu8* g = in + cstart;
                    constexpr uint32_t kPieces = (kCB + 1023u) / 1024u;
                    u32x4 v[kPieces];
#pragma unroll
                    for (uint32_t k = 0; k < kPieces; ++k) {
                        const uint32_t i = k * 1024u + lane * 16u;
                        v[k] = u32x4{0, 0, 0, 0};
                        if (i + 16u <= avail) v[k] = ld16(g + i);
                        else if (i < avail) { for (uint32_t t = 0; i + t < avail; ++t) v[k][(t >> 2) & 3u] |= (uint32_t)g[i + t] << ((t & 3u) * 8u); }
                    }
                    const uint32_t h = cstart < kSegChunk ? 0u : 1u + (cstart - kSegChunk) / kSegStride;
                    uint32_t w = 0;
                    if (lane < (uint32_t)W) {
                        w = fed_bits[(size_t)h * kSegChunkWords + ((cstart - h * kSegStride) >> 5) + lane];
                        const uint32_t vf = fed_vf[h];
                        const uint32_t wpos = cstart + lane * 32u;
                        if (vf == 0xFFFFFFFFu || vf >= wpos + 32u) w = 0u;
                        else if (vf > wpos) w &= ~((1u << (vf - wpos)) - 1u);
                        if (wpos >= len) w = 0u;
                        else if (len - wpos < 32u) w &= (1u << (len - wpos)) - 1u;
                    }
#pragma unroll
                    for (uint32_t k = 0; k < kPieces; ++k) {
                        const uint32_t i = k * 1024u + lane * 16u;
                        if (i < kCB) *reinterpret_cast<u32x4*>(&cbuf[i]) = v[k];
                    }
                    PHASE(6);
                    const uint32_t cnt = (uint32_t)__popc(w);
                    const uint32_t incl = wave_scan_add(cnt);
                    uint32_t k = incl - cnt;
                    Tc = __builtin_amdgcn_readlane(incl, 63);
                    if (Tc > (uint32_t)TOKCAP) { bail = true; Tc = 0; }
                    else while (w) { const uint32_t b = (uint32_t)__builtin_ctz(w); toks[k++] = lane * 32u + b; w &= w - 1u; }
                }
                PHASE(7);
                if (Tc == 0u && !bail) bail = true;
                if (bail) Tc = 0;
            }
```

rust-lz-fear_amd/csrc/lz4_decompress_seg.hip:

```cpp
#include "lzf_device.h"
#include "kernels.h"
#include "lzf_copy_helpers.h"
#include <type_traits>

namespace lzf {
namespace {

constexpr uint32_t S = kSegRegion;
constexpr uint32_t kCB = kSegChunk;
constexpr uint32_t kNone = 0xFFFFFFFFu;
constexpr uint32_t kLenClamp = 1u << 26;
constexpr uint32_t kTileStage = kSegTile + 128u;
constexpr uint32_t kTileTokMax = kSegTile / 3u + 2u;
constexpr uint32_t kFlagCoop = 1u;

struct __attribute__((packed, aligned(1))) S8B { uint64_t v; };
struct __attribute__((packed, aligned(1))) S4B { uint32_t v; };
struct __attribute__((packed, aligned(1))) S2B { uint16_t v; };
__device__ __forceinline__ void st8(gu8* p, uint64_t v) { reinterpret_cast<LZF_GLOBAL S8B*>(p)->v = v; }
__device__ __forceinline__ void st4(gu8* p, uint32_t v) { reinterpret_cast<LZF_GLOBAL S4B*>(p)->v = v; }
__device__ __forceinline__ void st2(gu8* p, uint32_t v) { reinterpret_cast<LZF_GLOBAL S2B*>(p)->v = (uint16_t)v; }

__device__ __forceinline__ void copy_small_gg(gu8* d, cgu8* g, uint32_t n) {
    if (n > 32u) {
        const uint64_t a0 = ld8(g), a1 = ld8(g + 8u), a2 = ld8(g + 16u), a3 = ld8(g + 24u);
        const uint64_t b0 = ld8(g + n - 32u), b1 = ld8(g + n - 24u), b2 = ld8(g + n - 16u), b3 = ld8(g + n - 8u);
        st8(d, a0); st8(d + 8u, a1); st8(d + 16u, a2); st8(d + 24u, a3);
        st8(d + n - 32u, b0); st8(d + n - 24u, b1); st8(d + n - 16u, b2); st8(d + n - 8u, b3);
    } else if (n >= 16u) {
        const uint64_t a0 = ld8(g), a1 = ld8(g + 8u), b0 = ld8(g + n - 16u), b1 = ld8(g + n - 8u);
        st8(d, a0); st8(d + 8u, a1); st8(d + n - 16u, b0); st8(d + n - 8u, b1);
    } else if (n >= 8u) {
        const uint64_t a0 = ld8(g), b0 = ld8(g + n - 8u);
        st8(d, a0); st8(d + n - 8u, b0);
    } else if (n >= 4u) {
        const uint32_t a0 = ld4(g), b0 = ld4(g + n - 4u);
        st4(d, a0); st4(d + n - 4u, b0);
    } else if (n >= 2u) {
        const uint32_t a0 = ld2(g), b0 = ld2(g + n - 2u);
        st2(d, a0); st2(d + n - 2u, b0);
    } else if (n == 1u) {
        d[0] = g[0];
    }
}

__device__ __forceinline__ void copy_medium_gg(gu8* d, cgu8* g, uint32_t n) {
    uint32_t t = 0;
    for (; t + 64u <= n; t += 64u) {
        const u32x4 a0 = ld16(g + t), a1 = ld16(g + t + 16u), a2 = ld16(g + t + 32u), a3 = ld16(g + t + 48u);
        st16(d + t, a0); st16(d + t + 16u, a1); st16(d + t + 32u, a2); st16(d + t + 48u, a3);
    }
    for (; t + 16u <= n; t += 16u) st16(d + t, ld16(g + t));
    if (t < n) st16(d + n - 16u, ld16(g + n - 16u));
}
__device__ __forceinline__ void wave_copy_long(gu8* __restrict__ dst, cgu8* __restrict__ src, uint32_t n, uint32_t lane) {
    uint32_t i = 0;
    for (; i + 4096u <= n; i += 4096u) {
        const uint32_t o = i + lane * 16u;
        const u32x4 a0 = ld16(src + o), a1 = ld16(src + o + 1024u), a2 = ld16(src + o + 2048u), a3 = ld16(src + o + 3072u);
        st16(dst + o, a0); st16(dst + o + 1024u, a1); st16(dst + o + 2048u, a2); st16(dst + o + 3072u, a3);
    }
    wave_copy(dst + i, src + i, n - i, lane);
}

__device__ __forceinline__ uint32_t seg_nch(uint32_t len) {
    return len <= kSegChunk ? 1u : 1u + (len - kSegChunk + kSegStride - 1u) / kSegStride;
}

template <class RD8, class RDB>
__device__ __forceinline__ uint32_t count_ff(uint32_t q, uint32_t len, RD8 rd8, RDB rdb) {
    uint32_t n = 0;
    while (len - q >= 8u) {
        const uint64_t w = rd8(q);
        if (w != ~0ull) return n + ((uint32_t)__builtin_ctzll(~w) >> 3);
        n += 8u; q += 8u;
    }
    while (q < len && rdb(q) == 255u) { ++n; ++q; }
    return n;
}
template <class RD8, class RDB>
__device__ __forceinline__ bool read_lsic_tail(uint32_t& q, uint32_t len, uint32_t& v, RD8 rd8, RDB rdb) {
    if (q >= len) return false;
    const uint32_t n = count_ff(q, len, rd8, rdb);
    if (q + n >= len) { q = len; return false; }
    const uint64_t vv = 15ull + 255ull * n + rdb(q + n);
    v = vv > kMaxPosB ? kMaxPosB : (uint32_t)vv;
    q += n + 1u;
    return true;
}
template <class RD8, class RDB>
__device__ __forceinline__ bool token_next_gen(uint32_t len, uint32_t p, uint32_t& next, RD8 rd8, RDB rdb) {
    const uint32_t tok = rdb(p);
    uint32_t q = p + 1u;
    uint32_t L = tok >> 4;
    if (L == 15u) { if (!read_lsic_tail(q, len, L, rd8, rdb)) return false; }
    if (len - q < L) return false;
    q += L;
    if (len - q < 2u) { next = len; return true; }
    q += 2u;
    if ((tok & 15u) == 15u) { uint32_t M; if (!read_lsic_tail(q, len, M, rd8, rdb)) return false; }
    next = q;
    return true;
}
__device__ __forceinline__ bool token_next_glb(cgu8* in, uint32_t len, uint32_t p, uint32_t& next) {
    return token_next_gen(len, p, next, [&](uint32_t q) -> uint64_t { return ld8(in + q); }, [&](uint32_t q) -> uint32_t { return (uint32_t)in[q]; });
}
__device__ __forceinline__ uint64_t lds_ld64u(uint32_t a) {
    uint64_t v; asm volatile("ds_read_b64 %0, %1\n\ts_waitcnt lgkmcnt(0)" : "=v"(v) : "v"(a) : "memory"); return v;
}

}

__global__ __launch_bounds__(256) void lzf_seg_plan_kernel(seg_ctx c) {
    const uint32_t j = blockIdx.x * blockDim.x + threadIdx.x;
    if (j == 0u) *c.rec_top = 0ull;
    if (j >= c.n_jobs) return;
    const lzf_decompress_job job = c.jobs[j];
    seg_job s;
    s.failed = 0; s.done = 0; s.ntok = 0; s.outb = 0; s.pad = 0; s.rec_off = 0; s.pad2 = 0;
    s.eligible = ((c.fed || (job.prefix_len == 0 && job.out_existing_len == 0)) && job.input_len >= c.min_in && job.input_len <= c.max_in &&
                  job.input != nullptr && job.out != nullptr) ? 1u : 0u;
    const uint32_t len = s.eligible ? (uint32_t)job.input_len : 0u;
    s.nch = s.eligible ? seg_nch(len) : 0u;
    s.ntile = (len + kSegTile - 1u) / kSegTile;
    if (s.nch > c.maxch || s.ntile > c.maxtile) { s.eligible = 0; s.nch = 0; s.ntile = 0; }
    c.st[j] = s;
}

__global__ __launch_bounds__(64) void lzf_seg_parse_kernel(seg_ctx c) {
    __shared__ __attribute__((aligned(16))) uint8_t lds_parse[2u * 64u * 8u * 4u + kCB];
    static_assert(sizeof(lds_parse) == 20480, "eight chunks per CU: an eighth of 160 KiB each");
    uint32_t* const rowsA = reinterpret_cast<uint32_t*>(lds_parse);
    uint32_t* const rowsB = rowsA + 64u * 8u;
    const uint32_t j = seg_job_of(c, blockIdx.y);
    const seg_job sj = c.st[j];
    if (!sj.eligible) return;
    const uint32_t lane = threadIdx.x & 63u;
    const lzf_decompress_job job = c.jobs[j];
    cgu8* __restrict__ in = as_global(job.input);
    const uint32_t len = (uint32_t)job.input_len;
    uint8_t* const cbuf = lds_parse + 2u * 64u * 8u * 4u;
    const uint32_t cbuf_a = lds_addr(cbuf);
#define ROWA(w) rowsA[(w) * 64u + lane]
#define ROWB(w) rowsB[(w) * 64u + lane]

    for (uint32_t h = blockIdx.x; h < sj.nch; h += gridDim.x) {
        const uint32_t cstart = h * kSegStride;
        __syncthreads();
        {
            const uint32_t avail = len - cstart < kCB ? len - cstart : kCB;
            cgu8* g = in + cstart;
#pragma unroll 1
            for (uint32_t b4 = 0; b4 < kCB; b4 += 4u * 1024u) {
                u32x4 v[4];
#pragma unroll
                for (uint32_t k = 0; k < 4u; ++k) {
                    const uint32_t i = b4 + k * 1024u + lane * 16u;
                    v[k] = u32x4{0, 0, 0, 0};
                    if (i + 16u <= avail) v[k] = ld16(g + i);
                }
#pragma unroll
                for (uint32_t k = 0; k < 4u; ++k) {
                    const uint32_t i = b4 + k * 1024u + lane * 16u;
                    if (i < kCB) *reinterpret_cast<u32x4*>(&cbuf[i]) = v[k];
                }
            }
            { const uint32_t t0 = avail & ~15u; if (t0 < kCB && lane < (avail & 15u)) cbuf[t0 + lane] = g[t0 + lane]; }
        }
#pragma unroll
        for (uint32_t i = 0; i < 8u; ++i) { ROWA(i) = 0u; ROWB(i) = 0u; }
        const uint32_t room = len - cstart;
        const uint32_t fe = room > 24u ? (room - 24u < kCB - 2u ? room - 24u : kCB - 2u) : 0u;
        const uint32_t rb0 = lane * S, end_r = rb0 + S;

        auto rdb = [&](uint32_t q) -> uint32_t { const uint32_t r_ = q - cstart; if (r_ < kCB) return (uint32_t)cbuf[r_]; return (uint32_t)in[q]; };
        auto rd8 = [&](uint32_t q) -> uint64_t { const uint32_t r_ = q - cstart; if (r_ + 8u <= kCB) return lds_ld64u(cbuf_a + r_); return ld8(in + q); };
        auto token_next = [&](uint32_t p, uint32_t& next) -> bool { return token_next_gen(len, p, next, rd8, rdb); };
        auto walk = [&](uint32_t r, bool go, bool& merged, auto MODE) -> uint32_t {
            constexpr int mode = decltype(MODE)::value;
            const uint32_t stop = go ? (end_r < fe ? end_r : fe) : 0u;
            for (;;) {
#ifndef LZF_SEG_NOASM
                {
                    uint32_t mxp = 0x100u, rprev = r, mg = merged ? 1u : 0u;
                    const uint32_t stopv = stop;
                    const unsigned long long m0 = __ballot(go && !merged && r < stop);
                    uint32_t a_, w_, t_, x_, rn_, mk_;
                    unsigned long long sv, sc;
                    const uint32_t rowa2 = lds_addr(rowsA) + lane * 4u - (lane << 11), rowd = lds_addr(rowsB) - lds_addr(rowsA);
                    const uint32_t vzero = 0u, vff = 0xFFu, v100 = 0x100u;
                    if (mode == 0) {
                        asm volatile(
                            "s_mov_b64 %[sv], exec\n\t"
                            "s_and_b64 exec, exec, %[m0]\n\t"
                            "s_cbranch_execz Ld%=\n"
                            "Lw%=:\n\t"
                            "v_add_u32 %[a], %[cbm1], %[r]\n\t"
                            "ds_read_b32 %[w], %[a]\n\t"
                            "s_waitcnt lgkmcnt(0)\n\t"
                            "v_cmp_eq_u32_sdwa vcc, %[w], %[mxp] src0_sel:BYTE_0 src1_sel:DWORD\n\t"
                            "v_cndmask_b32 %[r], %[r], %[rprev], vcc\n\t"
                            "s_andn2_b64 exec, exec, vcc\n\t"
                            "v_cmpx_lt_u32 vcc, %[r], %[stop]\n\t"
                            "v_bfe_u32 %[x], %[w], 12, 4\n\t"
                            "v_cmp_eq_u32 vcc, 15, %[x]\n\t"
                            "v_cndmask_b32_sdwa %[t], %[vz], %[w], vcc dst_sel:DWORD dst_unused:UNUSED_PAD src0_sel:DWORD src1_sel:BYTE_2\n\t"
                            "v_addc_co_u32 %[rn], vcc, %[x], %[t], vcc\n\t"
                            "v_add3_u32 %[rn], %[rn], %[r], 3\n\t"
                            "v_and_b32 %[t], 0xfff000, %[w]\n\t"
                            "v_cmpx_ne_u32 vcc, 0xfff000, %[t]\n\t"
                            "v_and_b32 %[x], 0xf00, %[w]\n\t"
                            "v_cmp_eq_u32 vcc, 0xf00, %[x]\n\t"
                            "v_addc_co_u32 %[rn], %[sc], 0, %[rn], vcc\n\t"
                            "v_cndmask_b32 %[mxp], %[v100], %[vff], vcc\n\t"
                            "v_cmpx_gt_u32 vcc, %[fe], %[rn]\n\t"
                            "v_lshrrev_b32 %[x], 5, %[r]\n\t"
                            "v_lshl_add_u32 %[x], %[x], 8, %[rowa2]\n\t"
                            "v_lshlrev_b32 %[a], %[r], 1\n\t"
                            "ds_or_b32 %[x], %[a]\n\t"
                            "v_mov_b32 %[rprev], %[r]\n\t"
                            "v_mov_b32 %[r], %[rn]\n\t"
                            "s_cbranch_execnz Lw%=\n"
                            "Ld%=:\n\t"
                            "s_mov_b64 exec, %[sv]"
                            : [r] "+v"(r), [rprev] "+v"(rprev), [mxp] "+v"(mxp),
                              [a] "=&v"(a_), [w] "=&v"(w_), [t] "=&v"(t_), [x] "=&v"(x_), [rn] "=&v"(rn_), [sv] "=&s"(sv), [sc] "=&s"(sc)
                            : [cbm1] "s"(cbuf_a - 1u), [fe] "s"(fe), [stop] "v"(stopv), [rowa2] "v"(rowa2), [vz] "v"(vzero), [vff] "v"(vff), [v100] "v"(v100), [m0] "s"(m0)
                            : "vcc", "memory");
                    } else {
                        asm volatile(
                            "s_mov_b64 %[sv], exec\n\t"
                            "s_and_b64 exec, exec, %[m0]\n\t"
                            "s_cbranch_execz Ld%=\n"
                            "Lw%=:\n\t"
                            "v_add_u32 %[a], %[cbm1], %[r]\n\t"
                            "v_lshrrev_b32 %[x], 5, %[r]\n\t"
                            "ds_read_b32 %[w], %[a]\n\t"
                            "v_lshl_add_u32 %[x], %[x], 8, %[rowa2]\n\t"
                            "ds_read_b32 %[mk], %[x]\n\t"
                            "s_waitcnt lgkmcnt(0)\n\t"
                            "v_cmp_eq_u32_sdwa vcc, %[w], %[mxp] src0_sel:BYTE_0 src1_sel:DWORD\n\t"
                            "v_cndmask_b32 %[r], %[r], %[rprev], vcc\n\t"
                            "s_andn2_b64 exec, exec, vcc\n\t"
                            "v_cmpx_lt_u32 vcc, %[r], %[stop]\n\t"
                            "v_lshrrev_b32 %[mk], %[r], %[mk]\n\t"
                            "v_and_b32 %[mk], 1, %[mk]\n\t"
                            "v_or_b32 %[mg], %[mg], %[mk]\n\t"
                            "v_cmpx_eq_u32 vcc, 0, %[mk]\n\t"
                            "v_bfe_u32 %[mk], %[w], 12, 4\n\t"
                            "v_cmp_eq_u32 vcc, 15, %[mk]\n\t"
                            "v_cndmask_b32_sdwa %[t], %[vz], %[w], vcc dst_sel:DWORD dst_unused:UNUSED_PAD src0_sel:DWORD src1_sel:BYTE_2\n\t"
                            "v_addc_co_u32 %[rn], vcc, %[mk], %[t], vcc\n\t"
                            "v_add3_u32 %[rn], %[rn], %[r], 3\n\t"
                            "v_and_b32 %[t], 0xfff000, %[w]\n\t"
                            "v_cmpx_ne_u32 vcc, 0xfff000, %[t]\n\t"
                            "v_and_b32 %[mk], 0xf00, %[w]\n\t"
                            "v_cmp_eq_u32 vcc, 0xf00, %[mk]\n\t"
                            "v_addc_co_u32 %[rn], %[sc], 0, %[rn], vcc\n\t"
                            "v_cndmask_b32 %[mxp], %[v100], %[vff], vcc\n\t"
                            "v_cmpx_gt_u32 vcc, %[fe], %[rn]\n\t"
                            "v_add_u32 %[x], %[x], %[rowd]\n\t"
                            "v_lshlrev_b32 %[a], %[r], 1\n\t"
                            "ds_or_b32 %[x], %[a]\n\t"
                            "v_mov_b32 %[rprev], %[r]\n\t"
                            "v_mov_b32 %[r], %[rn]\n\t"
                            "s_cbranch_execnz Lw%=\n"
                            "Ld%=:\n\t"
                            "s_mov_b64 exec, %[sv]"
                            : [r] "+v"(r), [rprev] "+v"(rprev), [mxp] "+v"(mxp), [mg] "+v"(mg),
                              [a] "=&v"(a_), [w] "=&v"(w_), [t] "=&v"(t_), [x] "=&v"(x_), [rn] "=&v"(rn_), [mk] "=&v"(mk_), [sv] "=&s"(sv), [sc] "=&s"(sc)
                            : [cbm1] "s"(cbuf_a - 1u), [fe] "s"(fe), [stop] "v"(stopv), [rowa2] "v"(rowa2), [rowd] "v"(rowd), [vz] "v"(vzero), [vff] "v"(vff), [v100] "v"(v100), [m0] "s"(m0)
                            : "vcc", "memory");
                    }
                    merged = mg != 0u;
                }
#else
                uint32_t mxp = 0, rprev = r;
                bool act = go && !merged && r < stop;
                while (__any(act)) {
                    uint32_t lo;
                    asm volatile("ds_read_b32 %0, %1" : "=v"(lo) : "v"(cbuf_a + (act ? r : 0u) - 1u) : "memory");
                    uint32_t mk = 0;
                    const uint32_t bi = (act ? r : rb0) - rb0;
                    if (mode == 1) mk = *reinterpret_cast<const volatile uint32_t*>(&ROWA((bi >> 5) & 7u)) >> (bi & 31u);
                    asm volatile("s_waitcnt lgkmcnt(0)" ::: "memory");
                    const uint32_t e0 = lo & 255u;
                    if (act && mxp != 0u && e0 == 255u) { r = rprev; act = false; }
                    if (act && r >= stop) act = false;
                    if (mode == 1) { if (act && (mk & 1u)) { merged = true; act = false; } }
                    if (act) {
                        const uint32_t L0 = (lo >> 12) & 15u, M0 = (lo >> 8) & 15u, b1 = (lo >> 16) & 255u;
                        const uint32_t isx = L0 == 15u ? 1u : 0u;
                        const uint32_t Lt = L0 + (isx ? b1 : 0u);
                        const uint32_t mx = M0 == 15u ? 1u : 0u;
                        const uint32_t rn = r + 3u + isx + Lt + mx;
                        const bool plain = !(isx && b1 == 255u) && rn < fe;
                        if (plain) {
                            if (mode == 0) ROWA((bi >> 5) & 7u) |= 1u << (bi & 31u); else ROWB((bi >> 5) & 7u) |= 1u << (bi & 31u);
                            rprev = r; r = rn; mxp = mx;
                        } else {
                            act = false;
                        }
                    }
                }
#endif
                const uint32_t pa = cstart + r;
                const bool slow = go && !merged && r < end_r && pa < len;
                if (!__any(slow)) break;
                if (slow) {
                    const uint32_t bi = r - rb0;
                    if (mode == 1 && ((ROWA((bi >> 5) & 7u) >> (bi & 31u)) & 1u)) merged = true;
                    else {
                        if (mode == 0) ROWA((bi >> 5) & 7u) |= 1u << (bi & 31u); else ROWB((bi >> 5) & 7u) |= 1u << (bi & 31u);
                        uint32_t nx;
                        if (!token_next(pa, nx)) nx = len;
                        r = nx - cstart;
                    }
                }
            }
            return r;
        };
        using M0T = std::integral_constant<int, 0>; using M1T = std::integral_constant<int, 1>;
        const bool in_input = cstart + rb0 < len;
        bool mdummy = false;
        const uint32_t x0 = walk(rb0, in_input, mdummy, M0T{});
        uint32_t X = in_input ? x0 : 0u, walked = rb0, mpos = rb0;
        for (uint32_t pass = 0; pass < 80u; ++pass) {
            const uint32_t entry = wave_prev(wave_scan_max(X), 0u);
            const bool redo = in_input && entry != walked && lane != 0u;
            if (!__any(redo)) break;
            const bool inreg = redo && entry < end_r && cstart + entry < len;
            if (redo) {
                walked = entry;
#pragma unroll
                for (uint32_t i = 0; i < 8u; ++i) ROWB(i) = 0u;
            }
            bool mg = false;
            const uint32_t x1 = walk(inreg ? entry : end_r, inreg, mg, M1T{});
            if (redo) {
                if (!inreg) { X = entry; mpos = end_r; }
                else if (mg) { X = x0; mpos = x1; }
                else { X = x1; mpos = end_r; }
            }
        }
        {
            const uint32_t mb = mpos - rb0;
            u32x4 o0, o1;
#pragma unroll
            for (uint32_t i = 0; i < 8u; ++i) {
                const uint32_t wb = mb >> 5;
                const uint32_t keep = i < wb ? 0u : i == wb ? ~((1u << (mb & 31u)) - 1u) : ~0u;
                const uint32_t v = in_input ? ((ROWA(i) & keep) | ROWB(i)) : 0u;
                if (i < 4u) o0[i] = v; else o1[i - 4u] = v;
            }
            LZF_GLOBAL u32x4* dst = (LZF_GLOBAL u32x4*)(c.bits + ((size_t)j * c.maxch + h) * kSegChunkWords + lane * 8u);
            dst[0] = o0; dst[1] = o1;
            const uint32_t xm = __builtin_amdgcn_readlane(wave_scan_max(X), 63);
            uint64_t xe = (uint64_t)cstart + xm;
            if (xe > len) xe = len;
            if (lane == 0u) c.xexit[(size_t)j * c.maxch + h] = (uint32_t)xe;
        }
    }
}

#undef ROWA
#undef ROWB

__global__ __launch_bounds__(64) void lzf_seg_seam_kernel(seg_ctx c) {
    __shared__ uint16_t patch[kSegStride / 3u + 8u];
    constexpr uint32_t kWin = 2048;
    __shared__ __attribute__((aligned(16))) uint8_t wbytes[kWin + 128u];
    __shared__ uint32_t wbits[kWin / 32u + 2u];
    if (blockIdx.x >= c.g_n) return;
    const uint32_t j = c.grouped ? seg_job_of(c, blockIdx.x) : blockIdx.x;
    const seg_job sj = c.st[j];
    if (!sj.eligible) return;
    const uint32_t lane = threadIdx.x & 63u;
    const lzf_decompress_job job = c.jobs[j];
    cgu8* __restrict__ in = as_global(job.input);
    const uint32_t len = (uint32_t)job.input_len;
    LZF_GLOBAL uint32_t* const X = (LZF_GLOBAL uint32_t*)c.xexit + (size_t)j * c.maxch;
    LZF_GLOBAL uint32_t* const VF = (LZF_GLOBAL uint32_t*)c.vfrom + (size_t)j * c.maxch;
    LZF_GLOBAL uint32_t* const B = (LZF_GLOBAL uint32_t*)c.bits + (size_t)j * c.maxch * kSegChunkWords;
    auto bit = [&](uint32_t h, uint32_t pos) -> bool {
        const uint32_t r = pos - h * kSegStride;
        return (B[(size_t)h * kSegChunkWords + (r >> 5)] >> (r & 31u)) & 1u;
    };
    if (lane == 0u) VF[0] = 0u;
    bool carry_valid = false; uint32_t carry_e = 0;
    bool failed = false;
    for (uint32_t h0 = 1; h0 < sj.nch && !failed; h0 += 64u) {
        const uint32_t gn = sj.nch - h0 < 64u ? sj.nch - h0 : 64u;
        const uint32_t h = h0 + lane;
        const bool act = lane < gn;
        const uint32_t e = act ? X[h - 1u] : 0u;
        const uint32_t endh = h * kSegStride + kSegChunk;
        uint32_t code = 0;
        if (act) code = (e >= len || e >= endh) ? 1u : (bit(h, e) ? 0u : 2u);
        uint32_t k = 0;
        while (k < gn && !failed) {
            uint32_t e_true;
            if (!carry_valid) {
                const uint32_t kk0 = first_lane(__ballot(act && lane >= k && code != 0u));
                const uint32_t kk = kk0 < gn ? kk0 : gn;
                if (act && lane >= k && lane < kk) VF[h] = e;
                k = kk;
                if (k >= gn) break;
                e_true = __builtin_amdgcn_readlane(e, k);
            } else e_true = carry_e;
            const uint32_t hk = h0 + k;
            const uint32_t base = hk * kSegStride, endk = base + kSegChunk, ostart = base + kSegOverlap;
            if (e_true >= len || e_true >= endk) {
                if (lane == 0u) VF[hk] = kNone;
                carry_valid = true; carry_e = e_true;
            } else if (bit(hk, e_true)) {
                if (lane == 0u) VF[hk] = e_true;
                carry_valid = false;
            } else {
                uint32_t p = e_true, np = 0, mg = 0, err = 0;
                while (p < endk && p < len && !mg && !err) {
                    const uint32_t ws = p;
                    __syncthreads();
                    {
                        const uint32_t avail = len - ws < kWin + 128u ? len - ws : kWin + 128u;
                        for (uint32_t i = lane * 16u; i < kWin + 128u; i += 1024u) {
                            u32x4 v = u32x4{0, 0, 0, 0};
                            if (i + 16u <= avail) v = ld16(in + ws + i);
                            else if (i < avail) { for (uint32_t b = 0; i + b < avail; ++b) v[(b >> 2) & 3u] |= (uint32_t)in[ws + i + b] << ((b & 3u) * 8u); }
                            *reinterpret_cast<u32x4*>(&wbytes[i]) = v;
                        }
                        const uint32_t w0 = (ws - base) >> 5;
                        for (uint32_t i = lane; i < kWin / 32u + 2u; i += 64u)
                            wbits[i] = w0 + i < kSegChunkWords ? B[(size_t)hk * kSegChunkWords + w0 + i] : 0u;
                    }
                    __syncthreads();
                    if (lane == 0u) {
                        const uint32_t wb_a = lds_addr(wbytes);
                        auto rdb = [&](uint32_t q) -> uint32_t { const uint32_t r_ = q - ws; if (r_ < kWin + 128u) return (uint32_t)wbytes[r_]; return (uint32_t)in[q]; };
                        auto rd8 = [&](uint32_t q) -> uint64_t { const uint32_t r_ = q - ws; if (r_ + 8u <= kWin + 128u) return lds_ld64u(wb_a + r_); return ld8(in + q); };
                        const uint32_t bit0 = ((ws - base) >> 5) << 5;
                        while (p < endk && p < len && p - ws < kWin) {
                            const uint32_t rbit = p - base - bit0;
                            if (p != e_true && ((wbits[rbit >> 5] >> (rbit & 31u)) & 1u)) { mg = 1; break; }
                            patch[np++] = (uint16_t)(p - ostart);
                            uint32_t nx;
                            {
                                uint32_t w;
                                asm volatile("ds_read_b32 %0, %1\n\ts_waitcnt lgkmcnt(0)" : "=v"(w) : "v"(wb_a + (p - ws)) : "memory");
                                const uint32_t L0 = (w >> 4) & 15u, M0 = w & 15u, b1 = (w >> 8) & 255u;
                                const uint32_t q2 = p + 1u + (L0 == 15u ? 1u + 15u + b1 : L0);
                                if (!(L0 == 15u && b1 == 255u) && q2 + 3u <= len && q2 - ws + 3u <= kWin + 128u &&
                                    !(M0 == 15u && wbytes[q2 + 2u - ws] == 255u)) { p = q2 + 2u + (M0 == 15u ? 1u : 0u); continue; }
                            }
                            if (!token_next_gen(len, p, nx, rd8, rdb)) { err = 1; break; }
                            p = nx;
                        }
                    }
                    p = __builtin_amdgcn_readfirstlane(p); np = __builtin_amdgcn_readfirstlane(np);
                    mg = __builtin_amdgcn_readfirstlane(mg); err = __builtin_amdgcn_readfirstlane(err);
                }
                if (err) { failed = true; break; }
                uint32_t m = mg ? p : endk;
                {
                    const uint32_t w0 = kSegOverlap / 32u, mr = m - base;
                    for (uint32_t w = w0 + lane; w * 32u < mr; w += 64u) {
                        LZF_GLOBAL uint32_t* wp = &B[(size_t)hk * kSegChunkWords + w];
                        if (w * 32u + 32u <= mr) *wp = 0u;
                        else *wp &= ~((1u << (mr & 31u)) - 1u);
                    }
                    __threadfence();
                    for (uint32_t i = lane; i < np; i += 64u) {
                        const uint32_t r = (uint32_t)patch[i] + kSegOverlap;
                        atomicOr((uint32_t*)&B[(size_t)hk * kSegChunkWords + (r >> 5)], 1u << (r & 31u));
                    }
                    __threadfence();
                }
                if (lane == 0u) VF[hk] = ostart;
                if (mg) carry_valid = false; else { carry_valid = true; carry_e = p; }
            }
            ++k;
        }
    }
    if (failed && lane == 0u) c.st[j].failed = 1u;
}

namespace {
struct TileCtx {
    uint32_t tstart;
    uint32_t stage_a;
    uint32_t len;
    cgu8* in;
};
__device__ __forceinline__ uint32_t tile_rdb(const TileCtx& t, uint32_t q) {
    const uint32_t r = q - t.tstart;
    if (r < kTileStage) return lds_ld8(t.stage_a + r);
    return (uint32_t)t.in[q];
}
__device__ __forceinline__ uint32_t tile_enumerate(const seg_ctx& c, uint32_t j, uint32_t t, uint32_t lane, uint32_t len, cgu8* in,
                                                   uint8_t* stage, uint16_t* list) {
    const uint32_t tstart = t * kSegTile;
    {
        const uint32_t avail = len - tstart < kTileStage ? len - tstart : kTileStage;
        cgu8* g = in + tstart;
        for (uint32_t i = lane * 16u; i < kTileStage; i += 1024u) {
            u32x4 v = u32x4{0, 0, 0, 0};
            if (i + 16u <= avail) v = ld16(g + i);
            else if (i < avail) { for (uint32_t b = 0; i + b < avail; ++b) v[(b >> 2) & 3u] |= (uint32_t)g[i + b] << ((b & 3u) * 8u); }
            *reinterpret_cast<u32x4*>(&stage[i]) = v;
        }
    }
    const uint32_t h = t < kSegChunk / kSegTile ? 0u : 1u + (t - kSegChunk / kSegTile) / (kSegStride / kSegTile);
    const uint32_t widx = t * (kSegTile / 32u) - h * (kSegStride / 32u) + lane;
    uint32_t w = c.bits[((size_t)j * c.maxch + h) * kSegChunkWords + widx];
    const uint32_t vf = c.vfrom[(size_t)j * c.maxch + h];
    const uint32_t wpos = tstart + lane * 32u;
    if (vf == kNone || vf >= wpos + 32u) w = 0u;
    else if (vf > wpos) w &= ~((1u << (vf - wpos)) - 1u);
    if (wpos >= len) w = 0u;
    else if (len - wpos < 32u) w &= (1u << (len - wpos)) - 1u;
    const uint32_t cnt = (uint32_t)__popc(w);
    const uint32_t incl = wave_scan_add(cnt);
    uint32_t k = incl - cnt;
    while (w) { const uint32_t b = (uint32_t)__builtin_ctz(w); list[k++] = (uint16_t)(lane * 32u + b); w &= w - 1u; }
    __syncthreads();
    return __builtin_amdgcn_readlane(incl, 63);
}
struct Tok { uint32_t L, M, off, src; bool err; };
template <bool WANT_OFF = true>
__device__ __forceinline__ Tok tile_decode(const TileCtx& t, uint32_t p) {
    Tok k; k.err = false; k.M = 0; k.off = 0;
    const uint32_t len = t.len;
    uint32_t w;
    if (p - t.tstart + 4u <= kTileStage) { asm volatile("ds_read_b32 %0, %1\n\ts_waitcnt lgkmcnt(0)" : "=v"(w) : "v"(t.stage_a + (p - t.tstart)) : "memory"); }
    else { w = 0; for (uint32_t i = 0; i < 4u && p + i < len; ++i) w |= tile_rdb(t, p + i) << (8u * i); }
    const uint32_t tok = w & 255u;
    uint32_t q = p + 1u;
    uint32_t L = tok >> 4;
    auto rd8 = [&](uint32_t x) -> uint64_t { const uint32_t r = x - t.tstart; if (r + 8u <= kTileStage) return lds_ld64u(t.stage_a + r); return ld8(t.in + x); };
    auto rdb = [&](uint32_t x) -> uint32_t { return tile_rdb(t, x); };
    if (L == 15u) {
        if (((w >> 8) & 255u) != 255u && q < len) { L += (w >> 8) & 255u; ++q; }
        else if (!read_lsic_tail(q, len, L, rd8, rdb) || L > kLenClamp) k.err = true;
    }
    k.L = L; k.src = q;
    if (k.err) return k;
    if (len - q < L) { k.err = true; return k; }
    q += L;
    if (len - q < 2u) return k;
    if (WANT_OFF) k.off = tile_rdb(t, q) | (tile_rdb(t, q + 1u) << 8);
    q += 2u;
    uint32_t M = tok & 15u;
    if (M == 15u) { if (!read_lsic_tail(q, len, M, rd8, rdb) || M > kLenClamp) k.err = true; }
    k.M = M + 4u;
    return k;
}
}

__global__ __launch_bounds__(64) void lzf_seg_tilesum_kernel(seg_ctx c) {
    __shared__ __attribute__((aligned(16))) uint8_t stage[kTileStage];
    __shared__ uint16_t list[kTileTokMax + 64u];
    const uint32_t j = seg_job_of(c, blockIdx.y);
    const seg_job sj = c.st[j];
    if (!sj.eligible || sj.failed) return;
    const uint32_t lane = threadIdx.x & 63u;
    const lzf_decompress_job job = c.jobs[j];
    cgu8* __restrict__ in = as_global(job.input);
    const uint32_t len = (uint32_t)job.input_len;
    for (uint32_t t = blockIdx.x; t < sj.ntile; t += gridDim.x) {
        __syncthreads();
        const uint32_t n = tile_enumerate(c, j, t, lane, len, in, stage, list);
        TileCtx tc{t * kSegTile, lds_addr(stage), len, in};
        uint32_t sum = 0; bool err = false;
        for (uint32_t i0 = 0; i0 < n; i0 += 64u) {
            if (i0 + lane < n) {
                const Tok k = tile_decode<false>(tc, tc.tstart + list[i0 + lane]);
                err = err || k.err;
                sum += k.L + k.M;
            }
        }
        const uint64_t tot = (uint64_t)__builtin_amdgcn_readlane(wave_scan_add(sum & 0xFFFFu), 63) +
                             ((uint64_t)__builtin_amdgcn_readlane(wave_scan_add(sum >> 16), 63) << 16);
        if (tot > 0x7FFFFFFFull) err = true;
        if (lane == 0u) { c.tile_tok[(size_t)j * c.maxtile + t] = (n + 63u) / 64u; c.tile_out[(size_t)j * c.maxtile + t] = (uint32_t)tot; }
        if (__ballot(err) && lane == 0u) c.st[j].failed = 1u;
    }
}

__global__ __launch_bounds__(64) void lzf_seg_scan_kernel(seg_ctx c) {
    if (blockIdx.x >= c.g_n) return;
    const uint32_t j = c.grouped ? seg_job_of(c, blockIdx.x) : blockIdx.x;
    const seg_job sj = c.st[j];
    if (!sj.eligible || sj.failed) return;
    const uint32_t lane = threadIdx.x & 63u;
    const lzf_decompress_job job = c.jobs[j];
    LZF_GLOBAL uint32_t* const TT = (LZF_GLOBAL uint32_t*)c.tile_tok + (size_t)j * c.maxtile;
    LZF_GLOBAL uint32_t* const TO = (LZF_GLOBAL uint32_t*)c.tile_out + (size_t)j * c.maxtile;
    uint64_t ctok = 0, cout = 0;
    for (uint32_t t8 = 0; t8 < sj.ntile; t8 += 512u) {
        uint32_t av[8], bv[8];
#pragma unroll
        for (uint32_t k = 0; k < 8u; ++k) { const uint32_t t = t8 + 64u * k + lane; av[k] = t < sj.ntile ? TT[t] : 0u; bv[k] = t < sj.ntile ? TO[t] : 0u; }
#pragma unroll
        for (uint32_t k = 0; k < 8u; ++k) {
            const uint32_t t = t8 + 64u * k + lane;
            const uint32_t a = av[k], b = bv[k];
            const uint32_t ia = wave_scan_add(a);
            uint32_t blo = b & 0xFFFFu, bhi = b >> 16;
            const uint32_t ilo = wave_scan_add(blo), ihi = wave_scan_add(bhi);
            const uint64_t ib = (uint64_t)ilo + ((uint64_t)ihi << 16);
            const uint64_t eo = cout + ib - b;
            if (t < sj.ntile) { TT[t] = (uint32_t)(ctok + ia - a); TO[t] = eo > 0xFFFFFFFFull ? 0xFFFFFFFFu : (uint32_t)eo; }
            ctok += __builtin_amdgcn_readlane(ia, 63);
            cout += (uint64_t)__builtin_amdgcn_readlane(ilo, 63) + ((uint64_t)__builtin_amdgcn_readlane(ihi, 63) << 16);
        }
    }
    if (lane == 0u) {
        const uint64_t cap = job.out_cap > kMaxPosB ? kMaxPosB : job.out_cap;
        ctok *= 64ull;
        bool ok = cout <= cap && ctok < 0x7FFFFFFFull;
        uint64_t off = 0;
        if (ok) {
            const uint64_t need = ctok + 64ull;
            off = atomicAdd(c.rec_top, (unsigned long long)need);
            if (off + need > c.rec_cap) ok = false;
        }
        if (!ok) c.st[j].failed = 1u;
        else { c.st[j].ntok = (uint32_t)ctok; c.st[j].outb = (uint32_t)cout; c.st[j].rec_off = off; }
    }
}

__global__ __launch_bounds__(64) void lzf_seg_records_kernel(seg_ctx c) {
    __shared__ __attribute__((aligned(16))) uint8_t stage[kTileStage];
    __shared__ uint16_t list[kTileTokMax + 64u];
    const uint32_t j = (c.rec_by_len || c.grouped) ? seg_job_of(c, blockIdx.y) : blockIdx.y;
    const seg_job sj = c.st[j];
    if (!sj.eligible || sj.failed) return;
    const uint32_t lane = threadIdx.x & 63u;
    const lzf_decompress_job job = c.jobs[j];
    cgu8* __restrict__ in = as_global(job.input);
    gu8* out = as_global(job.out);
    const uint32_t len = (uint32_t)job.input_len;
    const uint32_t cap = job.out_cap > kMaxPosB ? kMaxPosB : (uint32_t)job.out_cap;
    const uint64_t limit = job.output_limit;
    LZF_GLOBAL u32x4* const recs = (LZF_GLOBAL u32x4*)c.recs + sj.rec_off;
    const uint32_t R = c.ring_bytes, kSpan = R / 8u, kAheadB = 3u * kSpan + 64u;
    const uint32_t rb = (uint32_t)(reinterpret_cast<uintptr_t>(job.out) & 15u);
    for (uint32_t t = blockIdx.x; t < sj.ntile; t += gridDim.x) {
        __syncthreads();
        const uint32_t n = tile_enumerate(c, j, t, lane, len, in, stage, list);
        TileCtx tc{t * kSegTile, lds_addr(stage), len, in};
        const uint32_t tbase = c.tile_tok[(size_t)j * c.maxtile + t] * 64u;
        uint32_t obase = c.tile_out[(size_t)j * c.maxtile + t];
        bool bad = false;
        for (uint32_t i0 = 0; i0 < n; i0 += 64u) {
            const uint32_t nb = n - i0 < 64u ? n - i0 : 64u;
            const bool act = lane < nb;
            Tok k; k.L = 0; k.M = 0; k.off = 0; k.src = 0; k.err = false;
            if (act) k = tile_decode(tc, tc.tstart + list[i0 + lane]);
            const uint32_t tot = k.L + k.M;
            const uint32_t incl = wave_scan_add(tot);
            const uint32_t ob = obase;
            const uint32_t lo = obase + (incl - tot), mo = lo + k.L;
            obase += __builtin_amdgcn_readlane(incl, 63);
            bool ok = act && !k.err;
            if (ok) {
                if (lo > cap || cap - lo < k.L) ok = false;
                else if (k.M && ((uint64_t)mo + k.M > limit || k.off == 0u || k.off > mo || cap - mo < k.M)) ok = false;
            }
            bad = bad || (act && !ok);
            if (ok) {
                if (k.L > 0u && k.L <= 64u) copy_small_gg(out + lo, in + k.src, k.L);
                else if (k.L > 64u && k.L <= 256u) copy_medium_gg(out + lo, in + k.src, k.L);
            }
            for (unsigned long long m = __ballot(ok && k.L > 256u); m; m &= m - 1ull) {
                const uint32_t q = (uint32_t)__builtin_ctzll(m);
                wave_copy_long(out + __builtin_amdgcn_readlane(lo, q), in + __builtin_amdgcn_readlane(k.src, q), __builtin_amdgcn_readlane(k.L, q), lane);
            }
            if (__ballot(bad)) continue;
            const uint32_t M = k.M, off = k.off;
            const bool has = act && M != 0u;
            const uint32_t span = M < off ? M : off;
            const uint32_t s0 = mo - off, e0 = s0 + span;
            uint32_t lvl = has ? 1u : 0u;
            const bool dep = has && e0 > ob;
            auto from_lane = [](uint32_t l, uint32_t v) -> uint32_t { return (uint32_t)__builtin_amdgcn_ds_bpermute((int)((l & 63u) << 2), (int)v); };
            if (__any(dep)) {
                const uint32_t endv = act ? mo + M : 0xFFFFFFFFu, mov = act ? mo : 0xFFFFFFFFu;
                uint32_t a = 0, bb = 0;
#pragma unroll
                for (uint32_t step = 32u; step; step >>= 1) {
                    if (from_lane(a + step - 1u, endv) <= s0) a += step;
                    if (from_lane(bb + step - 1u, mov) < e0) bb += step;
                }
                const uint32_t ilo = a, ihi = bb - 1u;
                const bool any_dep = dep && bb >= 1u && ilo <= ihi && ihi < lane;
                if (__any(any_dep)) {
                    const bool wide = any_dep && ihi - ilo > 1u;
                    const bool any_wide = __any(wide);
                    for (uint32_t it = 0; it < 64u; ++it) {
                        const uint32_t la = from_lane(ilo, lvl), lb = from_lane(ihi, lvl);
                        uint32_t m = la > lb ? la : lb;
                        if (any_wide) { const uint32_t pm = from_lane(ihi, wave_scan_max(lvl)); if (wide) m = pm; }
                        const uint32_t nl = any_dep ? 1u + m : lvl;
                        const bool ch = nl != lvl;
                        lvl = nl;
                        if (!__any(ch)) break;
                    }
                }
            }
            const uint32_t endp = mo + M;
            uint32_t sub = 0, cls = 0;
            uint32_t a = 0, sidx = 0;
            while (a < nb) {
                const uint32_t sob = __builtin_amdgcn_readlane(lo, a);
                const uint32_t bb0 = first_lane(__ballot(lane >= a && lane < nb && endp - sob > kSpan));
                uint32_t e = bb0 < nb ? bb0 : nb;
                const bool giant = e == a;
                if (giant) e = a + 1u;
                const uint32_t oe = __builtin_amdgcn_readlane(endp, e - 1u);
                if (lane >= a && lane < e) {
                    sub = sidx;
                    if (giant) cls = 8u;
                    else if (M != 0u) {
                        const uint32_t fpw = ((oe + rb + 15u) & ~15u) + kAheadB;
                        const uint32_t lov = fpw > R ? fpw - R : 0u;
                        const uint32_t sy = s0 + rb, dy = mo + rb;
                        const uint32_t di = dy & (R - 1u), si = sy & (R - 1u);
                        const bool wrap = di + M > R || si + M > R;
                        if (sy < lov) cls = 7u;
                        else if (M > 64u || wrap) cls = 6u;
                        else if (off < M) cls = (off == 1u || off == 2u || off == 4u) ? (M < 8u ? 9u : M <= 16u ? 10u : M <= 32u ? 11u : 12u) : 5u;
                        else cls = M < 8u ? 1u : M <= 16u ? 2u : M <= 32u ? 3u : 4u;
                    }
                }
                a = e; ++sidx;
            }
            {
                const uint32_t last_end = __builtin_amdgcn_readlane(endp, (nb - 1u) & 63u);
                const uint32_t last_sub = __builtin_amdgcn_readlane(sub, (nb - 1u) & 63u);
                u32x4 w;
                w[0] = act ? M : 0u; w[1] = (act ? mo : last_end) + rb;
                const uint32_t fl = !act ? 0u : ((cls == 1u || cls == 9u) ? 1u : 0u) | (((cls >= 2u && cls <= 4u) || (cls >= 10u && cls <= 12u)) ? 2u : 0u) |
                                    ((cls == 3u || cls == 4u || cls == 11u || cls == 12u) ? 4u : 0u) | ((cls == 4u || cls == 12u) ? 8u : 0u) |
                                    ((cls == 5u || cls == 6u) ? 16u : 0u) | ((cls >= 9u && cls <= 12u) ? 32u : 0u);
                w[2] = (act ? sub : last_sub) | (fl << 8) | ((act ? lvl : 0u) << 16) | ((act ? cls : 0u) << 24); w[3] = act ? off : 0u;
                recs[tbase + i0 + lane] = w;
            }
        }
        if (__ballot(bad) && lane == 0u) c.st[j].failed = 1u;
    }
}

__global__ __launch_bounds__(1024) void lzf_seg_by_len_kernel(seg_ctx c) {
    __shared__ uint32_t cost[1024];
    const uint32_t i = threadIdx.x, n = c.n_jobs;
    if (n > 1024u) return;
    if (i < n) { const uint64_t l = c.jobs[i].input_len; cost[i] = l > 0xFFFFFFFFull ? 0xFFFFFFFFu : (uint32_t)l; }
    __syncthreads();
    if (i >= n) return;
    const uint32_t mine = cost[i];
    uint32_t r = 0;
    for (uint32_t k = 0; k < n; ++k) { const uint32_t o = cost[k]; r += (o > mine || (o == mine && k < i)) ? 1u : 0u; }
    c.by_len[r] = i;
}
__global__ __launch_bounds__(64) void lzf_seg_pause_kernel(uint32_t ticks) {
    const uint64_t t0 = wall_clock64();
    while (wall_clock64() - t0 < ticks) __builtin_amdgcn_s_sleep(32);
}
__global__ __launch_bounds__(1024) void lzf_seg_rank_kernel(seg_ctx c, uint32_t* __restrict__ by_tok, uint4 gs) {
    __shared__ uint32_t cost[1024];
    const uint32_t i = threadIdx.x, n = c.n_jobs;
    if (n > 1024u) return;
    if (i < n) { const seg_job s = c.st[i]; cost[i] = (s.eligible && !s.failed) ? s.ntok : 0u; }
    __syncthreads();
    if (i >= n) return;
    const uint32_t mine = cost[i];
    uint32_t r = 0;
    for (uint32_t k = 0; k < n; ++k) { const uint32_t o = cost[k]; r += (o > mine || (o == mine && k < i)) ? 1u : 0u; }
    by_tok[r] = i;
    if (!c.order) return;
    const uint32_t sz[4] = {gs.x, gs.y, gs.z, gs.w};
    uint32_t off = 0, gn = 0;
    for (uint32_t k = 0; k < 4u; ++k) { if (r >= off + sz[k]) off += sz[k]; else { gn = sz[k]; break; } }
    if (!gn) return;
    const uint32_t rr = r - off;
    const uint32_t ncu = c.n_cu ? c.n_cu : 256u;
    const uint32_t row = rr / ncu, col = rr % ncu;
    const uint32_t rowlen = gn - row * ncu < ncu ? gn - row * ncu : ncu;
    c.order[off + row * ncu + ((row & 1u) ? rowlen - 1u - col : col)] = i;
}
__global__ __launch_bounds__(1024) void lzf_seg_order_kernel(seg_ctx c) {
    __shared__ uint32_t cost[1024];
    const uint32_t i = threadIdx.x, n = c.g_n;
    if (n > 1024u) return;
    const uint32_t job = i < n ? (c.grouped ? seg_job_of(c, i) : i) : 0u;
    if (i < n) { const seg_job s = c.st[job]; cost[i] = (s.eligible && !s.failed) ? s.ntok : 0u; }
    __syncthreads();
    if (i >= n) return;
    const uint32_t mine = cost[i];
    uint32_t r = 0;
    for (uint32_t k = 0; k < n; ++k) { const uint32_t o = cost[k]; r += (o > mine || (o == mine && k < i)) ? 1u : 0u; }
    const uint32_t ncu = c.n_cu ? c.n_cu : 256u;
    const uint32_t row = r / ncu, col = r % ncu;
    const uint32_t rowlen = n - row * ncu < ncu ? n - row * ncu : ncu;
    c.order[c.g_off + row * ncu + ((row & 1u) ? rowlen - 1u - col : col)] = job;
}

template <int R>
__global__ __launch_bounds__(128) void lzf_seg_resolve_pair_kernel(seg_ctx c) {
    constexpr uint32_t kMask = (uint32_t)R - 1u;
    constexpr uint32_t kSpan = (uint32_t)R / 8u;
    constexpr uint32_t NS = 3;
    constexpr uint32_t NT = 32;
    __shared__ __attribute__((aligned(16))) uint8_t lds_all[64 + R];
    uint8_t* const ring = lds_all + 64;
    uint32_t* const ctl = reinterpret_cast<uint32_t*>(lds_all);
    if (blockIdx.x >= c.g_n) return;
    const uint32_t j = c.order ? c.order[c.g_off + blockIdx.x] : c.grouped ? seg_job_of(c, blockIdx.x) : blockIdx.x;
    const seg_job sj = c.st[j];
    if (!sj.eligible || sj.failed) return;
    if (c.ring_bytes != (uint32_t)R) return;
    if (c.res_prio) __builtin_amdgcn_s_setprio(3);
    const uint32_t lane = threadIdx.x & 63u;
    const uint32_t role = __builtin_amdgcn_readfirstlane(threadIdx.x >> 6);
    const lzf_decompress_job job = c.jobs[j];
    const long long t_start = clock64();
    gu8* const out = as_global(job.out);
    const uint32_t rb = (uint32_t)(reinterpret_cast<uintptr_t>(out) & 15u);
    gu8* const outb = out - rb;
    const LZF_GLOBAL u32x4* const recs = (const LZF_GLOBAL u32x4*)c.recs + sj.rec_off;
    const uint32_t n = sj.ntok, total = sj.outb;
    const uint32_t ring_a = lds_addr(ring);
    if (threadIdx.x < 4u) ctl[threadIdx.x] = 0u;
    __syncthreads();
    const uint32_t ctl_a = lds_addr(ctl);
    auto flag_get = [&](uint32_t i) -> uint32_t { uint32_t v; asm volatile("ds_read_b32 %0, %1\n\ts_waitcnt lgkmcnt(0)" : "=v"(v) : "v"(ctl_a + 4u * i) : "memory"); return __builtin_amdgcn_readfirstlane(v); };
    auto flag_set = [&](uint32_t i, uint32_t v) { asm volatile("s_waitcnt lgkmcnt(0)\n\tds_write_b32 %0, %1" ::"v"(ctl_a + 4u * i), "v"(v) : "memory"); };
    auto flag_wait_above = [&](uint32_t i, uint32_t below) -> bool {
        for (uint32_t spin = 0;; ++spin) {
            if (flag_get(i) > below) return true;
            if ((spin & 63u) == 63u && (flag_get(3) != 0u || spin > (1u << 22))) { if (lane == 0u) flag_set(3, 1u); return false; }
            __builtin_amdgcn_s_sleep(1);
        }
    };

    auto ring_copy = [&](uint32_t d, uint32_t s_, uint32_t nbytes) {
        if (nbytes >= 8u) {
            const uint32_t nu = (nbytes + 7u) >> 3;
            for (uint32_t u = lane; u < nu; u += kWave) {
                const uint32_t o = 8u * u + 8u <= nbytes ? 8u * u : nbytes - 8u;
                const uint32_t sa = (s_ + o) & kMask, da = (d + o) & kMask;
                if (sa + 8u <= (uint32_t)R && da + 8u <= (uint32_t)R) lds_st64(ring_a + da, lds_ld64u(ring_a + sa));
                else for (uint32_t t = 0; t < 8u; ++t) ring[(da + t) & kMask] = ring[(sa + t) & kMask];
            }
        } else if (lane < nbytes) ring[(d + lane) & kMask] = ring[(s_ + lane) & kMask];
    };
    auto ring_match = [&](uint32_t d, uint32_t off_, uint32_t M_) {
        uint32_t pos = 0, av = off_;
        while (pos < M_) { const uint32_t cc = av < M_ - pos ? av : M_ - pos; ring_copy(d + pos, d - off_, cc); pos += cc; av += cc; }
    };

    if (role == 0u) {
#ifdef LZF_SEG_TIME
        long long tm_wait = 0, tm_setup = 0, tm_asm = 0, tm_slow = 0, tm_t = clock64(); uint32_t n_rounds = 0;
#define RT(var) do { const long long t__ = clock64(); var += t__ - tm_t; tm_t = t__; } while (0)
#else
#define RT(var) do { } while (0)
#endif
        uint32_t t = 0, staged = 0;
        u32x4 rA = u32x4{0, 0, 0, 0}, rB = u32x4{0, 0, 0, 0};
        if (n) { rA = recs[lane < n ? lane : n - 1u]; rB = recs[64u + lane < n ? 64u + lane : n - 1u]; }
        auto wait_staged = [&](uint32_t tt) -> bool {
            if (staged > tt) return true;
            for (uint32_t spin = 0;; ++spin) {
                staged = flag_get(0);
                if (staged > tt) return true;
                if ((spin & 63u) == 63u && (flag_get(3) != 0u || spin > (1u << 22))) { if (lane == 0u) flag_set(3, 1u); return false; }
                __builtin_amdgcn_s_sleep(1);
            }
        };
        for (uint32_t i0 = 0; i0 < n; i0 += 64u) {
            const uint32_t nb = n - i0 < 64u ? n - i0 : 64u;
            const u32x4 r = rA;
            asm volatile("" ::: "memory");
            rA = rB;
            { const uint32_t ix = i0 + 128u + lane; rB = recs[ix < n ? ix : n - 1u]; }
            asm volatile("" ::: "memory");
            RT(tm_setup);
            if (!wait_staged(t)) break;
            RT(tm_wait);
            const uint32_t M = r[0], dy = r[1], off = r[3];
            const uint32_t sub = lane < nb ? (r[2] & 0xFFu) : 0xFFu, lvl = (r[2] >> 16) & 255u, cls = lane < nb ? r[2] >> 24 : 0u;
            const uint32_t nsub = __builtin_amdgcn_readlane(r[2] & 0xFFu, (nb - 1u) & 63u) + 1u;
            const uint32_t sa = ring_a + ((dy - off) & kMask), da = ring_a + (dy & kMask);
            const uint32_t o3 = M - 8u, a1 = M - 4u;
#if !defined(LZF_SEG_NOASM) && !defined(LZF_SEG_DBG_SKIP) && !defined(LZF_SEG_NORLE)
            const uint32_t fl = r[2] >> 8;
            const unsigned long long mA_b = __ballot((fl & 1u) != 0u), m2_b = __ballot((fl & 2u) != 0u), m3_b = __ballot((fl & 4u) != 0u),
                                     m4_b = __ballot((fl & 8u) != 0u), mS_b = __ballot((fl & 16u) != 0u), mR_b = __ballot((fl & 32u) != 0u);
            uint32_t rsel = 0, rsh = 0;
            if (mR_b) { rsel = off == 1u ? 0u : off == 2u ? 0x01000100u : 0x03020100u; rsh = M & (off - 1u); }
#else
            const unsigned long long mA_b = __ballot(cls == 1u), m2_b = __ballot(cls >= 2u && cls <= 4u), m3_b = __ballot(cls == 3u || cls == 4u),
                                     m4_b = __ballot(cls == 4u), mS_b = __ballot(cls == 5u || cls == 6u || (cls >= 9u && cls <= 12u));
#ifdef LZF_SEG_NORLE
            const unsigned long long mR_b = 0; const uint32_t rsel = 0, rsh = 0;
#endif
#endif
            bool gave_up = false;
            for (uint32_t s_i = 0; s_i < nsub; ++s_i, ++t) {
#ifdef LZF_ANALYSIS
                if (c.dbg_force == 2u && (j & 1u) && t >= 2u) { if (lane == 0u) flag_set(3, 1u); gave_up = true; break; }
#endif
                if (s_i) {
                    RT(tm_setup);
                    if (!wait_staged(t)) { gave_up = true; break; }
                    RT(tm_wait);
                }
                const unsigned long long msub = nsub == 1u ? ~0ull : __ballot(sub == s_i);
                unsigned long long todo = (mA_b | m2_b | mS_b) & msub;
#if defined(LZF_SEG_DBG_SKIP) && LZF_SEG_DBG_SKIP == 2
                todo = 0;
#endif
                for (uint32_t lv = 1; todo; ++lv) {
                    unsigned long long ml;
#if !defined(LZF_SEG_NOASM) && !defined(LZF_SEG_DBG_SKIP)
                    unsigned long long ts;
                    {
                        unsigned long long sv;
                        lv = __builtin_amdgcn_readfirstlane(lv);
                        if ((mR_b | mS_b) & msub)
                        asm volatile(
                            "s_mov_b64 %[sv], exec\n\t"
                            ".p2align 6\n\t"
                            "Lloop%=:\n\t"
                            "v_cmp_eq_u32_e32 vcc, %[lv], %[vl]\n\t"
                            "s_add_u32 %[lv], %[lv], 1\n\t"
                            "s_and_b64 %[ml], vcc, %[todo]\n\t"
                            "s_cbranch_scc0 Lempty%=\n\t"
#ifdef LZF_SEG_TIME
                            "s_add_u32 %[nr], %[nr], 1\n\t"
#endif
                            "s_and_b64 exec, %[ml], %[mA]\n\t"
                            "ds_read_b32 v116, %[sa]\n\t"
                            "ds_read_b32 v117, %[tsrc] offset:28\n\t"
                            "s_and_b64 exec, %[ml], %[m2]\n\t"
                            "ds_read_b64 v[100:101], %[sa]\n\t"
                            "ds_read_b64 v[106:107], %[tsrc] offset:24\n\t"
                            "s_and_b64 exec, %[ml], %[m3]\n\t"
                            "s_cbranch_execz Lr%=\n\t"
                            "ds_read_b64 v[102:103], %[sa] offset:8\n\t"
                            "ds_read_b64 v[104:105], %[tsrc] offset:16\n\t"
                            "s_and_b64 exec, %[ml], %[m4]\n\t"
                            "s_cbranch_execz Lr%=\n\t"
                            "ds_read_b64 v[108:109], %[sa] offset:16\n\t"
                            "ds_read_b64 v[110:111], %[sa] offset:24\n\t"
                            "ds_read_b64 v[112:113], %[tsrc]\n\t"
                            "ds_read_b64 v[114:115], %[tsrc] offset:8\n\t"
                            "Lr%=:\n\t"
                            "s_and_b64 exec, %[ml], %[mR]\n\t"
#ifndef LZF_SEG_DBG_NOWAIT
                            "s_waitcnt lgkmcnt(0)\n\t"
#endif
                            "s_cbranch_execz Lnr%=\n\t"
                            "v_perm_b32 v116, v116, v116, %[rsel]\n\t"
                            "v_perm_b32 v100, v100, v100, %[rsel]\n\t"
                            "v_alignbyte_b32 v117, v116, v116, %[rsh]\n\t"
                            "v_alignbyte_b32 v106, v100, v100, %[rsh]\n\t"
                            "v_mov_b32 v101, v100\n\t"
                            "v_mov_b32 v107, v106\n\t"
                            "v_mov_b64 v[102:103], v[100:101]\n\t"
                            "v_mov_b64 v[104:105], v[106:107]\n\t"
                            "v_mov_b64 v[108:109], v[100:101]\n\t"
                            "v_mov_b64 v[110:111], v[100:101]\n\t"
                            "v_mov_b64 v[112:113], v[106:107]\n\t"
                            "v_mov_b64 v[114:115], v[106:107]\n\t"
                            "Lnr%=:\n\t"
                            "s_and_b64 exec, %[ml], %[mA]\n\t"
                            "ds_write_b32 %[da], v116\n\t"
                            "ds_write_b32 %[tdst], v117 offset:28\n\t"
                            "s_and_b64 exec, %[ml], %[m2]\n\t"
                            "ds_write_b64 %[da], v[100:101]\n\t"
                            "ds_write_b64 %[tdst], v[106:107] offset:24\n\t"
                            "s_and_b64 exec, %[ml], %[m3]\n\t"
                            "s_cbranch_execz Lw%=\n\t"
                            "ds_write_b64 %[da], v[102:103] offset:8\n\t"
                            "ds_write_b64 %[tdst], v[104:105] offset:16\n\t"
                            "s_and_b64 exec, %[ml], %[m4]\n\t"
                            "s_cbranch_execz Lw%=\n\t"
                            "ds_write_b64 %[da], v[108:109] offset:16\n\t"
                            "ds_write_b64 %[da], v[110:111] offset:24\n\t"
                            "ds_write_b64 %[tdst], v[112:113]\n\t"
                            "ds_write_b64 %[tdst], v[114:115] offset:8\n\t"
                            "Lw%=:\n\t"
                            "s_mov_b64 exec, %[sv]\n\t"
                            "s_and_b64 %[ts], %[ml], %[mS]\n\t"
                            "s_cbranch_scc1 Lout%=\n\t"
                            "s_andn2_b64 %[todo], %[todo], %[ml]\n\t"
                            "s_cbranch_scc1 Lloop%=\n\t"
                            "s_branch Lout%=\n\t"
                            "Lempty%=:\n\t"
                            "s_mov_b64 %[ts], 0\n\t"
                            "s_cmp_le_u32 %[lv], 71\n\t"
                            "s_cbranch_scc1 Lloop%=\n\t"
                            "Lout%=:\n\t"
                            : [sv] "=&s"(sv), [ts] "=&s"(ts), [ml] "=&s"(ml), [todo] "+s"(todo), [lv] "+s"(lv)
#ifdef LZF_SEG_TIME
                              , [nr] "+s"(n_rounds)
#endif
                            : [mA] "s"(mA_b), [m2] "s"(m2_b), [m3] "s"(m3_b), [m4] "s"(m4_b), [mS] "s"(mS_b), [mR] "s"(mR_b), [vl] "v"(lvl), [rsel] "v"(rsel), [rsh] "v"(rsh),
                              [sa] "v"(sa), [tsrc] "v"(sa + M - 32u),
                              [da] "v"(da), [tdst] "v"(da + M - 32u)
                            : "memory", "vcc", "scc", "v100", "v101", "v102", "v103", "v104", "v105", "v106", "v107", "v108", "v109", "v110", "v111", "v112", "v113",
                              "v114", "v115", "v116", "v117");
                        else
                        asm volatile(
                            "s_mov_b64 %[sv], exec\n\t"
                            "s_mov_b64 %[ts], 0\n\t"
                            ".p2align 6\n\t"
                            "Lloop%=:\n\t"
                            "v_cmp_eq_u32_e32 vcc, %[lv], %[vl]\n\t"
                            "s_add_u32 %[lv], %[lv], 1\n\t"
                            "s_and_b64 %[ml], vcc, %[todo]\n\t"
                            "s_cbranch_scc0 Lempty%=\n\t"
#ifdef LZF_SEG_TIME
                            "s_add_u32 %[nr], %[nr], 1\n\t"
#endif
                            "s_and_b64 exec, %[ml], %[mA]\n\t"
                            "ds_read_b32 v116, %[sa]\n\t"
                            "ds_read_b32 v117, %[tsrc] offset:28\n\t"
                            "s_and_b64 exec, %[ml], %[m2]\n\t"
                            "ds_read_b64 v[100:101], %[sa]\n\t"
                            "ds_read_b64 v[106:107], %[tsrc] offset:24\n\t"
                            "s_and_b64 exec, %[ml], %[m3]\n\t"
                            "s_cbranch_execz Lr%=\n\t"
                            "ds_read_b64 v[102:103], %[sa] offset:8\n\t"
                            "ds_read_b64 v[104:105], %[tsrc] offset:16\n\t"
                            "s_and_b64 exec, %[ml], %[m4]\n\t"
                            "s_cbranch_execz Lr%=\n\t"
                            "ds_read_b64 v[108:109], %[sa] offset:16\n\t"
                            "ds_read_b64 v[110:111], %[sa] offset:24\n\t"
                            "ds_read_b64 v[112:113], %[tsrc]\n\t"
                            "ds_read_b64 v[114:115], %[tsrc] offset:8\n\t"
                            "Lr%=:\n\t"
                            "s_waitcnt lgkmcnt(0)\n\t"
                            "s_and_b64 exec, %[ml], %[mA]\n\t"
                            "ds_write_b32 %[da], v116\n\t"
                            "ds_write_b32 %[tdst], v117 offset:28\n\t"
                            "s_and_b64 exec, %[ml], %[m2]\n\t"
                            "ds_write_b64 %[da], v[100:101]\n\t"
                            "ds_write_b64 %[tdst], v[106:107] offset:24\n\t"
                            "s_and_b64 exec, %[ml], %[m3]\n\t"
                            "s_cbranch_execz Lw%=\n\t"
                            "ds_write_b64 %[da], v[102:103] offset:8\n\t"
                            "ds_write_b64 %[tdst], v[104:105] offset:16\n\t"
                            "s_and_b64 exec, %[ml], %[m4]\n\t"
                            "s_cbranch_execz Lw%=\n\t"
                            "ds_write_b64 %[da], v[108:109] offset:16\n\t"
                            "ds_write_b64 %[da], v[110:111] offset:24\n\t"
                            "ds_write_b64 %[tdst], v[112:113]\n\t"
                            "ds_write_b64 %[tdst], v[114:115] offset:8\n\t"
                            "Lw%=:\n\t"
                            "s_mov_b64 exec, %[sv]\n\t"
                            "s_andn2_b64 %[todo], %[todo], %[ml]\n\t"
                            "s_cbranch_scc1 Lloop%=\n\t"
                            "s_branch Lout%=\n\t"
                            "Lempty%=:\n\t"
                            "s_mov_b64 %[ts], 0\n\t"
                            "s_cmp_le_u32 %[lv], 71\n\t"
                            "s_cbranch_scc1 Lloop%=\n\t"
                            "Lout%=:\n\t"
                            : [sv] "=&s"(sv), [ts] "=&s"(ts), [ml] "=&s"(ml), [todo] "+s"(todo), [lv] "+s"(lv)
#ifdef LZF_SEG_TIME
                              , [nr] "+s"(n_rounds)
#endif
                            : [mA] "s"(mA_b), [m2] "s"(m2_b), [m3] "s"(m3_b), [m4] "s"(m4_b), [mS] "s"(mS_b), [mR] "s"(mR_b), [vl] "v"(lvl), [rsel] "v"(rsel), [rsh] "v"(rsh),
                              [sa] "v"(sa), [tsrc] "v"(sa + M - 32u),
                              [da] "v"(da), [tdst] "v"(da + M - 32u)
                            : "memory", "vcc", "scc", "v100", "v101", "v102", "v103", "v104", "v105", "v106", "v107", "v108", "v109", "v110", "v111", "v112", "v113",
                              "v114", "v115", "v116", "v117");
                        RT(tm_asm);
                        auto uni = [](unsigned long long x) { return (unsigned long long)(uint32_t)__builtin_amdgcn_readfirstlane((uint32_t)x) | ((unsigned long long)(uint32_t)__builtin_amdgcn_readfirstlane((uint32_t)(x >> 32)) << 32); };
                        ts = uni(ts); ml = uni(ml); todo = uni(todo); lv = __builtin_amdgcn_readfirstlane(lv);
                        if (!ts) break;
                        todo &= ~ml;
                        --lv;
                    }
#else
                    ml = __ballot(lvl == lv) & todo;
                    if (!ml) { if (lv > 70u) break; continue; }
                    todo &= ~ml;
#endif
#if !defined(LZF_SEG_NOASM) && !defined(LZF_SEG_DBG_SKIP)
                    const unsigned long long mA = 0, m2 = 0, m3 = 0, m4 = 0, mS = ts;
#else
#ifdef LZF_SEG_TIME
                    ++n_rounds;
#endif
                    const unsigned long long mA = ml & mA_b, m2 = ml & m2_b, m3 = ml & m3_b, m4 = ml & m4_b, mS = ml & mS_b;
#endif
                    RT(tm_setup);
#if defined(LZF_SEG_DBG_SKIP) && LZF_SEG_DBG_SKIP == 1
                    continue;
#endif
                    if (mA | m2) {
                        uint64_t v0, v1, v2, v3, v4, v5, v6, v7; uint32_t va0, va1; unsigned long long sv;
                        asm volatile(
                            "s_mov_b64 %[sv], exec\n\t"
                            "s_mov_b64 exec, %[mA]\n\t"
                            "ds_read_b32 %[va0], %[sa]\n\t"
                            "ds_read_b32 %[va1], %[s1]\n\t"
                            "s_mov_b64 exec, %[m2]\n\t"
                            "ds_read_b64 %[v0], %[sa]\n\t"
                            "ds_read_b64 %[v3], %[s3]\n\t"
                            "s_mov_b64 exec, %[m3]\n\t"
                            "s_cbranch_execz Lr3%=\n\t"
                            "ds_read_b64 %[v1], %[sa] offset:8\n\t"
                            "ds_read_b64 %[v2], %[s16]\n\t"
                            "s_mov_b64 exec, %[m4]\n\t"
                            "s_cbranch_execz Lr3%=\n\t"
                            "ds_read_b64 %[v4], %[sa] offset:16\n\t"
                            "ds_read_b64 %[v5], %[sa] offset:24\n\t"
                            "ds_read_b64 %[v6], %[s32]\n\t"
                            "ds_read_b64 %[v7], %[s32] offset:8\n\t"
                            "Lr3%=:\n\t"
                            "s_waitcnt lgkmcnt(0)\n\t"
                            "s_mov_b64 exec, %[mA]\n\t"
                            "ds_write_b32 %[da], %[va0]\n\t"
                            "ds_write_b32 %[d1], %[va1]\n\t"
                            "s_mov_b64 exec, %[m2]\n\t"
                            "ds_write_b64 %[da], %[v0]\n\t"
                            "ds_write_b64 %[d3], %[v3]\n\t"
                            "s_mov_b64 exec, %[m3]\n\t"
                            "s_cbranch_execz Lw3%=\n\t"
                            "ds_write_b64 %[da], %[v1] offset:8\n\t"
                            "ds_write_b64 %[d16], %[v2]\n\t"
                            "s_mov_b64 exec, %[m4]\n\t"
                            "s_cbranch_execz Lw3%=\n\t"
                            "ds_write_b64 %[da], %[v4] offset:16\n\t"
                            "ds_write_b64 %[da], %[v5] offset:24\n\t"
                            "ds_write_b64 %[d32], %[v6]\n\t"
                            "ds_write_b64 %[d32], %[v7] offset:8\n\t"
                            "Lw3%=:\n\t"
                            "s_mov_b64 exec, %[sv]\n\t"
                            : [v0] "=&v"(v0), [v1] "=&v"(v1), [v2] "=&v"(v2), [v3] "=&v"(v3), [v4] "=&v"(v4), [v5] "=&v"(v5), [v6] "=&v"(v6), [v7] "=&v"(v7),
                              [va0] "=&v"(va0), [va1] "=&v"(va1), [sv] "=&s"(sv)
                            : [mA] "s"(mA), [m2] "s"(m2), [m3] "s"(m3), [m4] "s"(m4), [sa] "v"(sa), [s1] "v"(sa + a1), [s3] "v"(sa + o3), [s16] "v"(sa + M - 16u), [s32] "v"(sa + M - 32u),
                              [da] "v"(da), [d1] "v"(da + a1), [d3] "v"(da + o3), [d16] "v"(da + M - 16u), [d32] "v"(da + M - 32u)
                            : "memory");
                    }
                    RT(tm_asm);
                    if (mS) {
                        uint32_t M_s = M, off_s = off, dy_s = dy;
                        asm volatile("" : "+v"(M_s), "+v"(off_s), "+v"(dy_s));
                        const uint32_t M = M_s, off = off_s, dy = dy_s;
                        const uint32_t sa = ring_a + ((dy - off) & kMask), da = ring_a + (dy & kMask);
                        const bool nowS = (mS >> lane) & 1ull;
                        const bool fits = nowS && (((dy - off) & kMask) + M <= (uint32_t)R) && ((dy & kMask) + M <= (uint32_t)R);
                        const bool rle = fits && (off == 1u || off == 2u || off == 4u);
                        if (__ballot(rle)) {
                            uint32_t w = 0;
                            if (rle) {
                                asm volatile("ds_read_b32 %0, %1\n\ts_waitcnt lgkmcnt(0)" : "=v"(w) : "v"(sa) : "memory");
                                if (off == 1u) w = (w & 0xFFu) * 0x01010101u; else if (off == 2u) w = (w & 0xFFFFu) * 0x00010001u;
                                const uint64_t pat = (uint64_t)w | ((uint64_t)w << 32);
                                if (M >= 8u) {
                                    if (M <= 64u) for (uint32_t k = 0; k + 8u < M; k += 8u) lds_st64(da + k, pat);
                                    const uint32_t ph = (M - 8u) & (off - 1u);
                                    const uint64_t rot = ph ? (pat >> (8u * ph)) | (pat << (64u - 8u * ph)) : pat;
                                    lds_st64(da + M - 8u, rot);
                                } else {
                                    lds_st32(da, w);
                                    const uint32_t ph = (M - 4u) & (off - 1u);
                                    lds_st32(da + M - 4u, ph ? (uint32_t)(pat >> (8u * ph)) : w);
                                }
                            }
                            for (unsigned long long m = __ballot(rle && M > 64u); m; m &= m - 1ull) {
                                const uint32_t q = (uint32_t)__builtin_ctzll(m);
                                const uint32_t qd = __builtin_amdgcn_readlane(da, q), qM = __builtin_amdgcn_readlane(M, q);
                                const uint32_t qw = __builtin_amdgcn_readlane(w, q);
                                const uint64_t qp = (uint64_t)qw | ((uint64_t)qw << 32);
                                for (uint32_t k = 8u * lane; k + 8u <= qM; k += 8u * kWave) lds_st64(qd + k, qp);
                            }
                        }
                        const bool lngc = fits && !rle && off >= M && M <= 160u;
                        const bool lng = lngc && __builtin_popcountll(__ballot(lngc)) >= 4;
                        if (lng) {
                            uint32_t k = 0;
                            for (;;) {
                                const uint32_t kk = k + 32u <= M ? k : M - 32u;
                                uint64_t x0, x1, x2, x3;
                                lds_ld64x4(sa + kk, sa + kk + 8u, sa + kk + 16u, sa + kk + 24u, x0, x1, x2, x3);
                                lds_st64(da + kk, x0); lds_st64(da + kk + 8u, x1); lds_st64(da + kk + 16u, x2); lds_st64(da + kk + 24u, x3);
                                if (k + 32u >= M) break;
                                k += 32u;
                            }
                        }
                        const bool dbl = fits && !rle && !lng && M <= 64u;
                        if (dbl) {
                            uint32_t pos = 0, av = off;
                            while (pos < M) { const uint32_t cc = av < M - pos ? av : M - pos; put_small_lds(da + pos, sa, cc); pos += cc; av += cc; }
                        }
                        for (unsigned long long m = __ballot(nowS && !rle && !lng && !dbl); m; m &= m - 1ull) {
                            const uint32_t q = (uint32_t)__builtin_ctzll(m);
                            ring_match(__builtin_amdgcn_readlane(dy, q), __builtin_amdgcn_readlane(off, q), __builtin_amdgcn_readlane(M, q));
                        }
                        RT(tm_slow);
                    }
                }
                if (lane == 0u) flag_set(1, t + 1u);
            }
            if (gave_up) break;
        }
#ifdef LZF_SEG_TIME
        if (lane == 0u) flag_set(2, (uint32_t)(tm_wait >> 10));
        if (lane == 0u) { reinterpret_cast<uint16_t*>(&c.st[j].pad)[0] = (uint16_t)(n_rounds >> 4);
            c.st[j].pad2 = (unsigned long long)(uint16_t)(tm_wait >> 14) | ((unsigned long long)(uint16_t)(tm_setup >> 14) << 16) | ((unsigned long long)(uint16_t)(tm_asm >> 14) << 32) | ((unsigned long long)(uint16_t)(tm_slow >> 14) << 48); }
#endif
#undef RT
    } else {
        uint32_t fp = 0, fl = rb, safe = 0;
        uint32_t ticket = 0;
        static_assert(NT <= 32, "the ends of the tickets in flight live in the lanes of one register");
        uint32_t endv = rb;
        uint32_t flushed_t = 0;
        auto flush_range = [&](uint32_t y0, uint32_t y1) {
            if (y1 <= y0) return;
            uint32_t nh = (16u - (y0 & 15u)) & 15u; if (nh > y1 - y0) nh = y1 - y0;
            if (nh) { if (lane < nh) outb[y0 + lane] = ring[(y0 + lane) & kMask]; y0 += nh; }
            const uint32_t ng = (y1 - y0) >> 4;
            for (uint32_t g = lane; g < ng; g += kWave)
                *reinterpret_cast<LZF_GLOBAL u32x4*>(outb + y0 + 16u * g) = *reinterpret_cast<const u32x4*>(&ring[(y0 + 16u * g) & kMask]);
            y0 += ng << 4;
            if (lane < y1 - y0) outb[y0 + lane] = ring[(y0 + lane) & kMask];
        };
        auto fill_to = [&](uint32_t g1) {
            for (uint32_t y = fp + 16u * lane; y < g1; y += 16u * kWave)
                *reinterpret_cast<u32x4*>(&ring[y & kMask]) = *reinterpret_cast<const LZF_GLOBAL u32x4*>(outb + y);
            if (g1 > fp) fp = g1;
        };
        u32x4 pfa = u32x4{0, 0, 0, 0}, pfb = u32x4{0, 0, 0, 0};
        uint32_t pf0 = 0, pf1 = 0;
        const uint32_t fill_lim = (total + rb + 15u) & ~15u;
        auto prefetch_issue = [&](uint32_t need) {
            pf0 = fp; pf1 = fp + 2048u < fill_lim ? fp + 2048u : fill_lim;
            if (pf1 <= pf0 || fp > need + 1024u) { pf0 = pf1 = 0; return; }
            const uint32_t ya = pf0 + 16u * lane, yb = ya + 1024u;
            if (ya < pf1) pfa = *reinterpret_cast<const LZF_GLOBAL u32x4*>(outb + ya);
            if (yb < pf1) pfb = *reinterpret_cast<const LZF_GLOBAL u32x4*>(outb + yb);
        };
        auto prefetch_commit = [&]() {
            if (pf1 > pf0 && pf0 == fp) {
                const uint32_t ya = pf0 + 16u * lane, yb = ya + 1024u;
                if (ya < pf1) *reinterpret_cast<u32x4*>(&ring[ya & kMask]) = pfa;
                if (yb < pf1) *reinterpret_cast<u32x4*>(&ring[yb & kMask]) = pfb;
                fp = pf1;
            }
            pf0 = pf1 = 0;
        };
        auto flush_resolved = [&](uint32_t upto_t) {
            if (flushed_t < upto_t) {
                const uint32_t e = __builtin_amdgcn_readlane(endv, (upto_t - 1u) & 63u);
                if (e > fl) { flush_range(fl, e); fl = e; }
                flushed_t = upto_t;
            }
        };
#ifdef LZF_SEG_TIME
        long long tm_swait = 0, tm_fill = 0, tm_old = 0;
        bool gave_up = false;
        auto wait_resolved = [&](uint32_t tt) { const long long t0 = clock64(); if (tt && !gave_up && !flag_wait_above(1, tt - 1u)) gave_up = true; tm_swait += clock64() - t0; };
#else
        bool gave_up = false;
        auto wait_resolved = [&](uint32_t tt) { if (tt && !gave_up && !flag_wait_above(1, tt - 1u)) gave_up = true; };
#endif
        u32x4 rA = u32x4{0, 0, 0, 0}, rB = u32x4{0, 0, 0, 0};
        if (n) { rA = recs[lane < n ? lane : n - 1u]; rB = recs[64u + lane < n ? 64u + lane : n - 1u]; }
        uint32_t prev_end = rb;
        uint64_t ov0 = 0, ov1 = 0, ov2 = 0, ov3 = 0;
        uint32_t o_for = kNone;
        bool o_have = false;
        for (uint32_t i0 = 0; i0 < n && !gave_up; i0 += 64u) {
#ifdef LZF_ANALYSIS
            if (c.dbg_force == 1u && (j & 1u) && i0 >= 128u) { gave_up = true; if (lane == 0u) flag_set(3, 1u); break; }
#endif
            const uint32_t nb = n - i0 < 64u ? n - i0 : 64u;
            const u32x4 r = rA;
            const uint32_t M = lane < nb ? r[0] : 0u, dy = r[1], off = r[3];
            const uint32_t sub = lane < nb ? (r[2] & 0xFFu) : 0xFFu, cls = lane < nb ? r[2] >> 24 : 0u;
            const uint32_t nsub = __builtin_amdgcn_readlane(r[2] & 0xFFu, (nb - 1u) & 63u) + 1u;
            asm volatile("" ::: "memory");
            rA = rB;
            { const uint32_t ix = i0 + 128u + lane; rB = recs[ix < n ? ix : n - 1u]; }
            asm volatile("" ::: "memory");
            const uint32_t endy = dy + M;
            for (uint32_t s_i = 0; s_i < nsub && !gave_up; ++s_i) {
                const unsigned long long msub = __ballot(sub == s_i);
                if (!msub) { gave_up = true; if (lane == 0u) flag_set(3, 1u); break; }
                const uint32_t last = 63u - (uint32_t)__builtin_clzll(msub);
                const uint32_t oe = __builtin_amdgcn_readlane(endy, last);
                if (const unsigned long long mg8 = __ballot(sub == s_i && cls == 8u)) {
                    const uint32_t gl = (uint32_t)__builtin_ctzll(mg8);
                    const uint32_t g_dy = __builtin_amdgcn_readlane(dy, gl), g_M = __builtin_amdgcn_readlane(M, gl), g_off = __builtin_amdgcn_readlane(off, gl);
                    wait_resolved(ticket);
                    flush_resolved(ticket);
                    pf0 = pf1 = 0;
                    if (fp < ((prev_end + 15u) & ~15u)) fill_to((prev_end + 15u) & ~15u);
                    flush_range(fl, prev_end); if (prev_end > fl) fl = prev_end;
                    wave_store_fence();
                    if (g_M) {
                        gu8* const src = outb + (g_dy - g_off);
                        uint32_t pos = 0, av = g_off;
                        while (pos < g_M) {
                            const uint32_t cc = av < g_M - pos ? av : g_M - pos;
                            wave_copy_long(outb + g_dy + pos, src, cc, lane);
                            pos += cc; av += cc;
                            if (pos < g_M) wave_store_fence();
                        }
                        wave_store_fence();
                    }
                    fl = oe; safe = oe;
                    {
                        const uint32_t keep = (uint32_t)R - (NS * kSpan + 128u);
                        const uint32_t g1 = (oe + 15u) & ~15u;
                        fp = g1 > keep ? (g1 - keep) & ~15u : 0u;
                        fill_to(g1);
                    }
                } else {
                    uint32_t rs = 0;
                    {
                        const uint32_t need = (oe + 15u) & ~15u;
#ifdef LZF_SEG_TIME
                        const long long t0 = clock64();
#endif
                        for (uint32_t spin = 0; !gave_up; ++spin) {
                            rs = flag_get(1);
                            const uint32_t er = rs < ticket ? __builtin_amdgcn_readlane(endv, rs & 63u) : need;
                            if (ticket - rs < NT && need <= er + 2u * kSpan + 16u) break;
                            if ((spin & 63u) == 63u && (flag_get(3) != 0u || spin > (1u << 22))) { if (lane == 0u) flag_set(3, 1u); gave_up = true; break; }
                            __builtin_amdgcn_s_sleep(1);
                        }
#ifdef LZF_SEG_TIME
                        tm_swait += clock64() - t0;
#endif
                    }
#if defined(LZF_SEG_DBG_SKIP) && LZF_SEG_DBG_SKIP == 3
                    if (false)
#endif
                    flush_resolved(rs < ticket ? rs : ticket);
#if defined(LZF_SEG_DBG_SKIP) && LZF_SEG_DBG_SKIP == 3
                    fp = (oe + 15u) & ~15u;
#endif
#ifdef LZF_SEG_TIME
                    const long long tf0 = clock64();
#endif
                    prefetch_commit();
                    fill_to((oe + 15u) & ~15u);
#ifdef LZF_SEG_TIME
                    asm volatile("s_waitcnt vmcnt(0) lgkmcnt(0)" ::: "memory");
                    tm_fill += clock64() - tf0;
#endif
                    prefetch_issue((oe + 15u) & ~15u);
                    bool old = sub == s_i && cls == 7u;
#ifdef LZF_SEG_TIME
                    const long long to0 = clock64();
#endif
                    {
                        const bool early = old && s_i == 0u && o_for == i0 && o_have;
                        if (__ballot(early)) {
                            if (early) {
                                const uint32_t d = ring_a + (dy & kMask);
                                if (M >= 8u) {
                                    lds_st64(d, ov0);
                                    if (M > 16u) { lds_st64(d + 8u, ov1); lds_st64(d + M - 16u, ov2); }
                                    lds_st64(d + M - 8u, ov3);
                                } else { lds_st32(d, (uint32_t)ov0); lds_st32(d + M - 4u, (uint32_t)ov3); }
                            }
                            old = old && !early;
                        }
                    }
                    if (__ballot(old)) {
                        uint32_t M_o = M, off_o = off, dy_o = dy;
                        asm volatile("" : "+v"(M_o), "+v"(off_o), "+v"(dy_o));
                        const uint32_t M = M_o, off = off_o, dy = dy_o;
                        const uint32_t span = M < off ? M : off;
                        const uint32_t sy = dy - off;
                        if (__ballot(old && sy + span > fl)) { wait_resolved(ticket); flush_resolved(ticket); }
                        if (__ballot(old && (sy + span > fl ? fl : sy + span) > safe)) { wave_store_fence(); safe = fl; }
                        const uint32_t di = dy & kMask;
                        const bool own = old && sy + span <= fl && M <= 64u && off >= M && di + M <= (uint32_t)R;
                        if (own) put_small_glb(ring_a + di, outb + sy, M);
                        for (unsigned long long m = __ballot(old && !own); m; m &= m - 1ull) {
                            const uint32_t q = (uint32_t)__builtin_ctzll(m);
                            const uint32_t qM = __builtin_amdgcn_readlane(M, q), qs = __builtin_amdgcn_readlane(sy, q), qd = __builtin_amdgcn_readlane(dy, q);
                            const uint32_t qo = __builtin_amdgcn_readlane(off, q);
                            for (uint32_t i = lane; i < qM; i += kWave) {
                                const uint32_t y = qs + (qo < qM ? i % qo : i);
                                ring[(qd + i) & kMask] = y < fl ? (uint8_t)outb[y] : ring[y & kMask];
                            }
                        }
                    }
#ifdef LZF_SEG_TIME
                    { asm volatile("s_waitcnt lgkmcnt(0)" ::: "memory"); tm_old += clock64() - to0; }
#endif
                }
                const uint32_t eg = oe & ~15u;
                if (lane == (ticket & 63u)) endv = eg;
                asm volatile("s_waitcnt lgkmcnt(0)" ::: "memory");
                ++ticket;
                if (lane == 0u) flag_set(0, ticket);
                prev_end = oe;
            }
            o_for = kNone; o_have = false;
            if (i0 + 64u < n && !gave_up) {
                const u32x4 q = rA;
                const uint32_t nbn = n - (i0 + 64u) < 64u ? n - (i0 + 64u) : 64u;
                const uint32_t Mn = q[0], dyn = q[1], offn = q[3];
                const uint32_t syn = dyn - offn, din = dyn & kMask;
                o_have = lane < nbn && (q[2] >> 24) == 7u && (q[2] & 0xFFu) == 0u && Mn >= 4u && Mn <= 32u && offn >= Mn &&
                         din + Mn <= (uint32_t)R && syn + Mn <= safe && syn + Mn <= fl;
                o_for = i0 + 64u;
                if (o_have) {
                    cgu8* g = outb + syn;
                    if (Mn >= 8u) { ov0 = ld8(g); ov3 = ld8(g + Mn - 8u); if (Mn > 16u) { ov1 = ld8(g + 8u); ov2 = ld8(g + Mn - 16u); } }
                    else { ov0 = ld4(g); ov3 = ld4(g + Mn - 4u); }
                }
            }
        }
        wait_resolved(ticket);
        if (gave_up || flag_get(3) != 0u) return;
#if !(defined(LZF_SEG_DBG_SKIP) && LZF_SEG_DBG_SKIP == 3)
        flush_resolved(ticket);
        flush_range(fl, total + rb);
#endif
        asm volatile("s_waitcnt vmcnt(0) lgkmcnt(0)" ::: "memory");

#ifdef LZF_SEG_TIME
        if (lane == 0u) reinterpret_cast<uint16_t*>(&c.st[j].pad)[1] = (uint16_t)(tm_swait >> 14);
#endif
        if (lane == 0u) {
            c.results[j].out_len = total;
            c.results[j].status = LZF_OK;
#ifdef LZF_SEG_TIME
            { auto b8 = [](long long v) -> uint32_t { const long long x = v >> 17; return x > 255 ? 255u : (uint32_t)x; };
              c.results[j].reserved = b8((long long)flag_get(2) << 10) | (b8(c.dbg_force == 8u ? tm_swait : tm_fill) << 8) | (b8(tm_old) << 16) | (b8(clock64() - t_start) << 24); }
#else
            c.results[j].reserved = (uint32_t)((clock64() - t_start) >> 10);
#endif
            c.st[j].done = 1u;
        }
    }
}
template __global__ void lzf_seg_resolve_pair_kernel<32768>(seg_ctx);
template __global__ void lzf_seg_resolve_pair_kernel<65536>(seg_ctx);
template __global__ void lzf_seg_resolve_pair_kernel<131072>(seg_ctx);

}
```

Baseline: 488.3.

## Parse fed-mode decompression in contiguous per-stretch runs into a flat bitmap

In fed mode, the parse kernel now gives each job a fixed number of stretches. Each workgroup walks consecutive chunks within its stretch and carries the token exit position from one chunk to the next. The per-chunk overlapped bitmap rows and the vfrom array are replaced by one flat per-job token bitmap. A new fed-specific seam kernel repairs the stretch boundaries in that bitmap, so the fed decoder no longer applies vfrom masking or computes chunk indices. This cuts redundant overlap parsing and scratch, at the cost of serial walking inside each stretch, fewer parallel workgroups per job, and a more complex seam fix-up.

New measurement: 498.9, median of 6. 1.02x the previous value.

```diff
diff --git a/rust-lz-fear_amd/build.py b/rust-lz-fear_amd/build.py
--- a/rust-lz-fear_amd/build.py
+++ b/rust-lz-fear_amd/build.py
@@ -16,7 +16,7 @@
 HEADERS = ["kernels.h", "lzf_device.h", "lz4_decompress_batch_phase.inc", "lz4_decompress_parse_phase.inc", "lz4_decompress_feed_phase.inc",
            "analysis/capi_analysis.inc",
            "lzf_copy_helpers.h", "lzf_parse_helpers.h", "lzf_compress_common.h", "lzf_simt.h", "lz4_compress_team.inc",
-           "host_staging.h", "lzf_frame_scan.h", "frame_jobs.h", "lzf_frame_layout.h", "lzf_size_rules.h", "lzf_chain_step.h", "frame_deliver_body.inc",
+           "host_staging.h", "lzf_frame_scan.h", "frame_jobs.h", "lzf_frame_layout.h", "lzf_size_rules.h", "lzf_chain_step.h", "frame_deliver_body.inc", "lzf_fed_parse_geometry.h",
            os.path.join(ROOT, "include", "lzfear_hip.h"), os.path.join(ROOT, "include", "lzfear_frame.h")]
 
 
diff --git a/rust-lz-fear_amd/csrc/capi.hip b/rust-lz-fear_amd/csrc/capi.hip
--- a/rust-lz-fear_amd/csrc/capi.hip
+++ b/rust-lz-fear_amd/csrc/capi.hip
@@ -6,6 +6,7 @@
 #include <mutex>
 #include <vector>
 #include "kernels.h"
+#include "lzf_fed_parse_geometry.h"
 #include "host_staging.h"
 
 namespace {
@@ -178,7 +179,11 @@
 #ifdef LZF_ANALYSIS
     { static const char* e = getenv("LZF_SEG_GRID"); if (e) { unsigned a = 0, b = 0; if (sscanf(e, "%u,%u", &a, &b) == 2 && a && b) { tg_parse = a; tg_tile = b; } } }
 #endif
-    if (upto >= 2) LAUNCH(lzf::lzf_seg_parse_kernel, dim3(seg_grid(tg_parse, n, c.maxch), n), dim3(64), 0, st, c);
+#ifdef LZF_ANALYSIS
+    if (upto >= 2 && c.fed && c.fed_sxj) { LAUNCH(lzf::lzf_seg_parse_kernel, dim3(c.fed_s, n), dim3(64), 0, st, c); } else
+#endif
+    if (upto >= 2 && c.fed) LAUNCH(lzf::lzf_seg_parse_kernel, dim3(n, c.fed_s), dim3(64), 0, st, c);
+    else if (upto >= 2) LAUNCH(lzf::lzf_seg_parse_kernel, dim3(seg_grid(tg_parse, n, c.maxch), n), dim3(64), 0, st, c);
     if (upto >= 3) LAUNCH(lzf::lzf_seg_seam_kernel, dim3(n), dim3(64), 0, st, c);
     if (upto >= 4) LAUNCH(lzf::lzf_seg_tilesum_kernel, dim3(seg_grid(tg_tile, n, c.maxtile), n), dim3(64), 0, st, c);
     if (upto >= 5) LAUNCH(lzf::lzf_seg_scan_kernel, dim3(n), dim3(64), 0, st, c);
@@ -344,6 +349,13 @@
     return kFedMinHint;
 }
 constexpr uint64_t kFedMaxScratch = 24ull << 30;
+inline uint32_t fed_stretches(uint32_t n) {
+#ifdef LZF_ANALYSIS
+    static const long v = [] { const char* e = getenv("LZF_FED_STRETCHES"); return e ? atol(e) : 0L; }();
+    if (v >= 1 && v <= (long)lzf_fedgeom::kMaxStretches) return (uint32_t)v;
+#endif
+    return lzf_fedgeom::stretches_for(n, cu_count());
+}
 constexpr uint32_t kFedMaxJobs = 65535u;
 constexpr uint32_t kFedLdsAlloc = 6400u;
 constexpr uint32_t kFedWavesPerCu = 4u * (LZF_FED_WAVES > 0 ? (uint32_t)LZF_FED_WAVES : 5u);
@@ -384,7 +396,8 @@
     SegScratch s; const lzf_decompress_job* jobs = nullptr; lzf_job_result* res = nullptr; uint32_t n = 0; const uint32_t* perm = nullptr;
     size_t o_tick = 0, o_fst = 0; bool live = false;
 };
-int fed_front(FedCall& f, const lzf_decompress_job* d_jobs, lzf_job_result* d_results, uint32_t n, const uint32_t* perm, hipStream_t st, uint64_t max_in_hint) {
+int fed_front(FedCall& f, const lzf_decompress_job* d_jobs, lzf_job_result* d_results, uint32_t n, const uint32_t* perm, hipStream_t st, uint64_t max_in_hint,
+              uint32_t stretches = 0u) {
     f.jobs = d_jobs; f.res = d_results; f.n = n; f.perm = perm; f.live = false;
     lzf::seg_ctx& c = f.s.ctx;
     c = lzf::seg_ctx{};
@@ -395,13 +408,18 @@
     c.maxtile = (max_in + lzf::kSegTile - 1u) / lzf::kSegTile;
     c.n_cu = cu_count();
     c.g_off = 0u; c.g_n = n; c.fed = 1u;
+    c.fed_s = stretches ? stretches : fed_stretches(n);
+    c.fed_words = lzf_fedgeom::row_words(max_in);
+#ifdef LZF_ANALYSIS
+    { static const bool sxj = [] { const char* e = getenv("LZF_FED_GRID"); return e && !strcmp(e, "sxj"); }(); c.fed_sxj = sxj ? 1u : 0u; }
+#endif
     size_t off = 0;
     auto take = [&](size_t bytes) { const size_t o = off; off = align_up(off + bytes, 256); return o; };
     const size_t o_st = take(sizeof(lzf::seg_job) * (size_t)n);
     const size_t o_top = take(sizeof(unsigned long long));
-    const size_t o_x = take(sizeof(uint32_t) * (size_t)n * c.maxch);
-    const size_t o_vf = take(sizeof(uint32_t) * (size_t)n * c.maxch);
-    const size_t o_bits = take(sizeof(uint32_t) * (size_t)n * c.maxch * lzf::kSegChunkWords);
+    const size_t o_x = take(sizeof(uint32_t) * (size_t)n * c.fed_s);
+    const size_t o_vf = take(sizeof(uint32_t) * (size_t)n * c.fed_s);
+    const size_t o_bits = take(sizeof(uint32_t) * (size_t)n * c.fed_words);
     f.o_tick = take(sizeof(uint32_t) * 32u * lzf::kFedTicketStride);
     f.o_fst = take(sizeof(lzf::fed_state) * (size_t)n);
     if (off > kFedMaxScratch) return LZF_OK;
@@ -417,6 +435,9 @@
     if (rc != LZF_OK) { (void)hipFreeAsync(f.s.base, st); f.s.base = nullptr; f.live = false; g_last_error = "bitmap-fed decompress: launch failed"; }
     return rc;
 }
+#ifdef LZF_ANALYSIS
+uint64_t g_fed_counts[4] = {0, 0, 0, 0};
+#endif
 int fed_back(FedCall& f, hipStream_t st, uint32_t slots_per_cu) {
     if (!f.live) return LZF_OK;
     lzf::seg_ctx& c = f.s.ctx;
@@ -435,7 +456,7 @@
     if ((uint64_t)n * pieces > 0xFFFFFFF0ull) pieces = 1u;
     if (!fg.xcc_mask) pieces = 1u;
     int rc = LZF_OK;
-    lzf::fed_args a{f.jobs, f.res, c.st, c.bits, c.vfrom, f.perm, reinterpret_cast<lzf::fed_state*>(b + f.o_fst), reinterpret_cast<uint32_t*>(b + f.o_tick), fg.xcc_mask ? fg.xcc_mask : 1u, n, c.maxch, pieces, nullptr};
+    lzf::fed_args a{f.jobs, f.res, c.st, c.bits, f.perm, reinterpret_cast<lzf::fed_state*>(b + f.o_fst), reinterpret_cast<uint32_t*>(b + f.o_tick), fg.xcc_mask ? fg.xcc_mask : 1u, n, c.fed_words, pieces, nullptr};
     hipLaunchKernelGGL(lzf::lzf_fed_reset_kernel, dim3((n + 255u) / 256u), dim3(256), 0, st, a);
     hipLaunchKernelGGL(k_fed32, dim3(slots < n ? slots : n), dim3(64), pad, st, a);
     if (hipGetLastError() != hipSuccess) rc = LZF_E_HIP;
@@ -443,6 +464,18 @@
         hipLaunchKernelGGL(k_paired24, dim3(n), dim3(128), 0, st, f.jobs, f.res, n, f.perm, (const lzf::seg_job*)c.st);
         if (hipGetLastError() != hipSuccess) rc = LZF_E_HIP;
     }
+#ifdef LZF_ANALYSIS
+    if (rc == LZF_OK && getenv("LZF_FED_VERBOSE")) {
+        std::vector<lzf::seg_job> hs(n);
+        if (hipStreamSynchronize(st) == hipSuccess && hipMemcpy(hs.data(), c.st, sizeof(lzf::seg_job) * n, hipMemcpyDeviceToHost) == hipSuccess) {
+            uint64_t el = 0, fin = 0;
+            for (const lzf::seg_job& q : hs) { el += q.eligible ? 1u : 0u; fin += (q.eligible && q.done) ? 1u : 0u; }
+            g_fed_counts[0] = el; g_fed_counts[1] = fin; g_fed_counts[2] = el - fin; g_fed_counts[3] = c.fed_s;
+            fprintf(stderr, "[lzf] bitmap-fed call: %u jobs, %llu eligible, %llu finished by the fed kernel, %llu left to the pair kernel (%u stretches, %u pieces)\n",
+                    n, (unsigned long long)el, (unsigned long long)fin, (unsigned long long)(el - fin), c.fed_s, pieces);
+        } else (void)hipGetLastError();
+    }
+#endif
     if (hipFreeAsync(f.s.base, st) != hipSuccess && rc == LZF_OK) rc = LZF_E_HIP;
     f.s.base = nullptr; f.live = false;
     if (rc != LZF_OK) g_last_error = "bitmap-fed decompress: launch failed";
@@ -753,6 +786,29 @@
     HIP_TRY(hipFree(s.base));
     return rc;
 }
+int lzf_debug_fed_map(const lzf_decompress_job* d_jobs, lzf_job_result* d_results, uint32_t n, uint64_t max_in_hint, uint32_t stretches,
+                      void* h_state, void* h_bits, void* h_xexit, void* h_vfrom, uint32_t* geom) {
+    int rc = ensure_device();
+    if (rc < 0) return rc;
+    if (n == 0 || stretches > lzf_fedgeom::kMaxStretches) return LZF_E_INVALID;
+    FedCall f;
+    rc = fed_front(f, d_jobs, d_results, n, nullptr, nullptr, max_in_hint, stretches);
+    if (rc != LZF_OK) return rc;
+    if (!f.live) return LZF_E_HIP;
+    const lzf::seg_ctx& c = f.s.ctx;
+    bool ok = hipDeviceSynchronize() == hipSuccess;
+    if (geom) { geom[0] = c.fed_words; geom[1] = c.fed_s; }
+    if (ok && h_state) ok = hipMemcpy(h_state, c.st, sizeof(lzf::seg_job) * n, hipMemcpyDeviceToHost) == hipSuccess;
+    if (ok && h_bits) ok = hipMemcpy(h_bits, c.bits, sizeof(uint32_t) * (size_t)n * c.fed_words, hipMemcpyDeviceToHost) == hipSuccess;
+    if (ok && h_xexit) ok = hipMemcpy(h_xexit, c.xexit, sizeof(uint32_t) * (size_t)n * c.fed_s, hipMemcpyDeviceToHost) == hipSuccess;
+    if (ok && h_vfrom) ok = hipMemcpy(h_vfrom, c.vfrom, sizeof(uint32_t) * (size_t)n * c.fed_s, hipMemcpyDeviceToHost) == hipSuccess;
+    if (hipFreeAsync(f.s.base, nullptr) != hipSuccess) ok = false;
+    f.s.base = nullptr; f.live = false;
+    if (hipDeviceSynchronize() != hipSuccess) ok = false;
+    if (!ok) { (void)hipGetLastError(); g_last_error = "lzf_debug_fed_map: a HIP call failed"; return LZF_E_HIP; }
+    return LZF_OK;
+}
+void lzf_debug_fed_counts(uint64_t* out4) { for (int i = 0; i < 4; ++i) out4[i] = g_fed_counts[i]; }
 #endif
 
 int lzf_compress_batch_host(const lzf_compress_job* jobs, lzf_job_result* results, uint32_t n_jobs) {
diff --git a/rust-lz-fear_amd/csrc/kernels.h b/rust-lz-fear_amd/csrc/kernels.h
--- a/rust-lz-fear_amd/csrc/kernels.h
+++ b/rust-lz-fear_amd/csrc/kernels.h
@@ -71,6 +71,10 @@
     uint32_t g_off, g_n, grouped;
     uint32_t res_prio;
     uint32_t fed;
+    uint32_t fed_s, fed_words;
+#ifdef LZF_ANALYSIS
+    uint32_t fed_sxj;
+#endif
 };
 struct fed_state { uint32_t flag, cstart, expect, o; };
 constexpr uint32_t kFedEnded = 0x80000000u;
@@ -80,12 +84,11 @@
     lzf_job_result* results;
     seg_job* st;
     const uint32_t* bits;
-    const uint32_t* vfrom;
     const uint32_t* perm;
     fed_state* state;
     uint32_t* ticket;
     uint32_t xcc_mask;
-    uint32_t n_jobs, maxch;
+    uint32_t n_jobs, words;
     uint32_t pieces;
     uint32_t* census;
 };
diff --git a/rust-lz-fear_amd/csrc/lz4_decompress_fed.hip b/rust-lz-fear_amd/csrc/lz4_decompress_fed.hip
--- a/rust-lz-fear_amd/csrc/lz4_decompress_fed.hip
+++ b/rust-lz-fear_amd/csrc/lz4_decompress_fed.hip
@@ -74,8 +74,7 @@
         const uint64_t limit = job.output_limit;
         const uint32_t rb = (uint32_t)(reinterpret_cast<uintptr_t>(out) & 15u);
         const uint32_t ring_a = lds_addr(ring), cbuf_a = lds_addr(cbuf);
-        const LZF_GLOBAL uint32_t* const fed_bits = (const LZF_GLOBAL uint32_t*)a.bits + (size_t)jid * a.maxch * kSegChunkWords;
-        const LZF_GLOBAL uint32_t* const fed_vf = (const LZF_GLOBAL uint32_t*)a.vfrom + (size_t)jid * a.maxch;
+        const LZF_GLOBAL uint32_t* const fed_bits = (const LZF_GLOBAL uint32_t*)a.bits + (size_t)jid * a.words;
 #define RIDX(x) (((x) + rb) & kMask)
 
         auto ring_fill = [&](uint32_t a_, uint32_t b) {
diff --git a/rust-lz-fear_amd/csrc/lz4_decompress_feed_phase.inc b/rust-lz-fear_amd/csrc/lz4_decompress_feed_phase.inc
--- a/rust-lz-fear_amd/csrc/lz4_decompress_feed_phase.inc
+++ b/rust-lz-fear_amd/csrc/lz4_decompress_feed_phase.inc
@@ -18,14 +18,10 @@
                         if (i + 16u <= avail) v[k] = ld16(g + i);
                         else if (i < avail) { for (uint32_t t = 0; i + t < avail; ++t) v[k][(t >> 2) & 3u] |= (uint32_t)g[i + t] << ((t & 3u) * 8u); }
                     }
-                    const uint32_t h = cstart < kSegChunk ? 0u : 1u + (cstart - kSegChunk) / kSegStride;
                     uint32_t w = 0;
                     if (lane < (uint32_t)W) {
-                        w = fed_bits[(size_t)h * kSegChunkWords + ((cstart - h * kSegStride) >> 5) + lane];
-                        const uint32_t vf = fed_vf[h];
+                        w = fed_bits[(cstart >> 5) + lane];
                         const uint32_t wpos = cstart + lane * 32u;
-                        if (vf == 0xFFFFFFFFu || vf >= wpos + 32u) w = 0u;
-                        else if (vf > wpos) w &= ~((1u << (vf - wpos)) - 1u);
                         if (wpos >= len) w = 0u;
                         else if (len - wpos < 32u) w &= (1u << (len - wpos)) - 1u;
                     }
diff --git a/rust-lz-fear_amd/csrc/lz4_decompress_seg.hip b/rust-lz-fear_amd/csrc/lz4_decompress_seg.hip
--- a/rust-lz-fear_amd/csrc/lz4_decompress_seg.hip
+++ b/rust-lz-fear_amd/csrc/lz4_decompress_seg.hip
@@ -1,6 +1,7 @@
 #include "lzf_device.h"
 #include "kernels.h"
 #include "lzf_copy_helpers.h"
+#include "lzf_fed_parse_geometry.h"
 #include <type_traits>
 
 namespace lzf {
@@ -12,6 +13,7 @@
 constexpr uint32_t kLenClamp = 1u << 26;
 constexpr uint32_t kTileStage = kSegTile + 128u;
 constexpr uint32_t kTileTokMax = kSegTile / 3u + 2u;
+static_assert(lzf_fedgeom::kChunk == kSegChunk && lzf_fedgeom::kRegion == kSegRegion && lzf_fedgeom::kRunUp == kSegOverlap, "the fed mode's stretches are made of the same chunks");
 constexpr uint32_t kFlagCoop = 1u;
 
 struct __attribute__((packed, aligned(1))) S8B { uint64_t v; };
@@ -132,7 +134,13 @@
     static_assert(sizeof(lds_parse) == 20480, "eight chunks per CU: an eighth of 160 KiB each");
     uint32_t* const rowsA = reinterpret_cast<uint32_t*>(lds_parse);
     uint32_t* const rowsB = rowsA + 64u * 8u;
-    const uint32_t j = seg_job_of(c, blockIdx.y);
+    const bool fed = c.fed != 0u;
+#ifdef LZF_ANALYSIS
+    const bool sxj = c.fed_sxj != 0u;
+#else
+    constexpr bool sxj = false;
+#endif
+    const uint32_t j = seg_job_of(c, fed && !sxj ? blockIdx.x : blockIdx.y);
     const seg_job sj = c.st[j];
     if (!sj.eligible) return;
     const uint32_t lane = threadIdx.x & 63u;
@@ -144,8 +152,28 @@
 #define ROWA(w) rowsA[(w) * 64u + lane]
 #define ROWB(w) rowsB[(w) * 64u + lane]
 
-    for (uint32_t h = blockIdx.x; h < sj.nch; h += gridDim.x) {
-        const uint32_t cstart = h * kSegStride;
+    const uint32_t fs = sxj ? blockIdx.x : blockIdx.y;
+    const uint32_t per = fed ? lzf_fedgeom::chunks_per_stretch(len, c.fed_s) : 0u;
+    if (fed && lzf_fedgeom::stretch_empty(len, per, fs)) return;
+    uint32_t carry = fed ? lzf_fedgeom::parse_start(per, fs) : 0u;
+    const uint32_t h_first = fed ? 0u : blockIdx.x, h_end = fed ? per : sj.nch, h_step = fed ? 1u : gridDim.x;
+    for (uint32_t h = h_first; h < h_end; h += h_step) {
+        uint32_t cstart, ent = 0;
+        if (!fed) cstart = h * kSegStride;
+        else {
+            const uint64_t cs64 = lzf_fedgeom::chunk_start64(per, fs, h);
+            if (cs64 >= len) break;
+            cstart = (uint32_t)cs64;
+            if (carry >= len || carry - cstart >= kCB) {
+                if (lzf_fedgeom::lane_stores(cstart, lane, fs, h, c.fed_words)) {
+                    LZF_GLOBAL u32x4* dst = (LZF_GLOBAL u32x4*)(c.bits + (size_t)j * c.fed_words + lzf_fedgeom::map_word(cstart, lane));
+                    dst[0] = u32x4{0, 0, 0, 0}; dst[1] = u32x4{0, 0, 0, 0};
+                }
+                continue;
+            }
+            ent = carry - cstart;
+        }
+        const uint32_t elane = ent >> 8;
         __syncthreads();
         {
             const uint32_t avail = len - cstart < kCB ? len - cstart : kCB;
@@ -321,13 +349,14 @@
             return r;
         };
         using M0T = std::integral_constant<int, 0>; using M1T = std::integral_constant<int, 1>;
-        const bool in_input = cstart + rb0 < len;
+        const bool in_input = cstart + rb0 < len && lane >= elane;
+        const uint32_t r0 = lane == elane ? ent : rb0;
         bool mdummy = false;
-        const uint32_t x0 = walk(rb0, in_input, mdummy, M0T{});
-        uint32_t X = in_input ? x0 : 0u, walked = rb0, mpos = rb0;
+        const uint32_t x0 = walk(r0, in_input, mdummy, M0T{});
+        uint32_t X = in_input ? x0 : 0u, walked = r0, mpos = r0;
         for (uint32_t pass = 0; pass < 80u; ++pass) {
             const uint32_t entry = wave_prev(wave_scan_max(X), 0u);
-            const bool redo = in_input && entry != walked && lane != 0u;
+            const bool redo = in_input && entry != walked && lane > elane;
             if (!__any(redo)) break;
             const bool inreg = redo && entry < end_r && cstart + entry < len;
             if (redo) {
@@ -353,23 +382,129 @@
                 const uint32_t v = in_input ? ((ROWA(i) & keep) | ROWB(i)) : 0u;
                 if (i < 4u) o0[i] = v; else o1[i - 4u] = v;
             }
-            LZF_GLOBAL u32x4* dst = (LZF_GLOBAL u32x4*)(c.bits + ((size_t)j * c.maxch + h) * kSegChunkWords + lane * 8u);
-            dst[0] = o0; dst[1] = o1;
             const uint32_t xm = __builtin_amdgcn_readlane(wave_scan_max(X), 63);
             uint64_t xe = (uint64_t)cstart + xm;
             if (xe > len) xe = len;
-            if (lane == 0u) c.xexit[(size_t)j * c.maxch + h] = (uint32_t)xe;
+            if (fed) {
+                if (lzf_fedgeom::lane_stores(cstart, lane, fs, h, c.fed_words)) {
+                    LZF_GLOBAL u32x4* dst = (LZF_GLOBAL u32x4*)(c.bits + (size_t)j * c.fed_words + lzf_fedgeom::map_word(cstart, lane));
+                    dst[0] = o0; dst[1] = o1;
+                }
+                carry = xe > cstart ? (uint32_t)xe : cstart;
+            } else {
+                LZF_GLOBAL u32x4* dst = (LZF_GLOBAL u32x4*)(c.bits + ((size_t)j * c.maxch + h) * kSegChunkWords + lane * 8u);
+                dst[0] = o0; dst[1] = o1;
+                if (lane == 0u) c.xexit[(size_t)j * c.maxch + h] = (uint32_t)xe;
+            }
         }
     }
+    if (fed && lane == 0u) c.xexit[(size_t)j * c.fed_s + fs] = carry;
 }
 
 #undef ROWA
 #undef ROWB
 
+namespace {
+constexpr uint32_t kWin = 2048;
+constexpr uint32_t kWinStage = kWin + 128u;
+__device__ __forceinline__ void seam_stage(uint8_t* wbytes, cgu8* in, uint32_t len, uint32_t ws, uint32_t lane) {
+    const uint32_t avail = len - ws < kWinStage ? len - ws : kWinStage;
+    for (uint32_t i = lane * 16u; i < kWinStage; i += 1024u) {
+        u32x4 v = u32x4{0, 0, 0, 0};
+        if (i + 16u <= avail) v = ld16(in + ws + i);
+        else if (i < avail) { for (uint32_t b = 0; i + b < avail; ++b) v[(b >> 2) & 3u] |= (uint32_t)in[ws + i + b] << ((b & 3u) * 8u); }
+        *reinterpret_cast<u32x4*>(&wbytes[i]) = v;
+    }
+}
+__device__ __forceinline__ bool seam_next(const uint8_t* wbytes, uint32_t ws, cgu8* in, uint32_t len, uint32_t p, uint32_t& nx) {
+    const uint32_t wb_a = lds_addr(wbytes);
+    uint32_t w;
+    asm volatile("ds_read_b32 %0, %1\n\ts_waitcnt lgkmcnt(0)" : "=v"(w) : "v"(wb_a + (p - ws)) : "memory");
+    const uint32_t L0 = (w >> 4) & 15u, M0 = w & 15u, b1 = (w >> 8) & 255u;
+    const uint32_t q2 = p + 1u + (L0 == 15u ? 1u + 15u + b1 : L0);
+    if (!(L0 == 15u && b1 == 255u) && q2 + 3u <= len && q2 - ws + 3u <= kWinStage &&
+        !(M0 == 15u && wbytes[q2 + 2u - ws] == 255u)) { nx = q2 + 2u + (M0 == 15u ? 1u : 0u); return true; }
+    auto rdb = [&](uint32_t q) -> uint32_t { const uint32_t r_ = q - ws; if (r_ < kWinStage) return (uint32_t)wbytes[r_]; return (uint32_t)in[q]; };
+    auto rd8 = [&](uint32_t q) -> uint64_t { const uint32_t r_ = q - ws; if (r_ + 8u <= kWinStage) return lds_ld64u(wb_a + r_); return ld8(in + q); };
+    return token_next_gen(len, p, nx, rd8, rdb);
+}
+
+__device__ __forceinline__ bool seam_fed(const seg_ctx& c, uint32_t j, uint32_t lane, cgu8* __restrict__ in, uint32_t len,
+                                         uint16_t* patch, uint8_t* wbytes, uint32_t* wbits) {
+    const uint32_t S_ = c.fed_s, per = lzf_fedgeom::chunks_per_stretch(len, S_);
+    LZF_GLOBAL uint32_t* const X = (LZF_GLOBAL uint32_t*)c.xexit + (size_t)j * S_;
+    LZF_GLOBAL uint32_t* const VF = (LZF_GLOBAL uint32_t*)c.vfrom + (size_t)j * S_;
+    LZF_GLOBAL uint32_t* const B = (LZF_GLOBAL uint32_t*)c.bits + (size_t)j * c.fed_words;
+    auto clear = [&](uint32_t a, uint32_t b) {
+        if (a >= b) return;
+        const uint32_t wa = a >> 5, wb = (b - 1u) >> 5;
+        for (uint32_t w = wa + lane; w <= wb; w += 64u) {
+            uint32_t m = ~0u;
+            if (w == wa) m &= ~0u << (a & 31u);
+            if (w == wb && (b & 31u)) m &= (1u << (b & 31u)) - 1u;
+            atomicAnd((uint32_t*)&B[w], ~m);
+        }
+    };
+    if (len == 0u) return true;
+    if (lane == 0u) VF[0] = 0u;
+    uint32_t e = X[0];
+    for (uint32_t s = 1; s < S_; ++s) {
+        if (lzf_fedgeom::stretch_empty(len, per, s)) break;
+        const uint32_t os = lzf_fedgeom::own_start(per, s), oe = lzf_fedgeom::own_end(len, per, s);
+        if (e >= oe) {
+            clear(os, oe);
+            if (lane == 0u) VF[s] = kNone;
+            continue;
+        }
+        if ((B[e >> 5] >> (e & 31u)) & 1u) {
+            clear(os, e);
+            if (lane == 0u) VF[s] = e;
+            e = X[s];
+            continue;
+        }
+        uint32_t p = e, clr = os, mg = 0, err = 0;
+        while (p < oe && !mg && !err) {
+            const uint32_t ws = p, w0 = ws >> 5;
+            uint32_t np = 0;
+            __syncthreads();
+            seam_stage(wbytes, in, len, ws, lane);
+            for (uint32_t i = lane; i < kWin / 32u + 2u; i += 64u) wbits[i] = w0 + i < c.fed_words ? B[w0 + i] : 0u;
+            __syncthreads();
+            if (lane == 0u) {
+                while (p < oe && p - ws < kWin) {
+                    const uint32_t rbit = p - (w0 << 5);
+                    if ((wbits[rbit >> 5] >> (rbit & 31u)) & 1u) { mg = 1; break; }
+                    patch[np++] = (uint16_t)(p - ws);
+                    uint32_t nx;
+                    if (!seam_next(wbytes, ws, in, len, p, nx)) { err = 1; break; }
+                    p = nx;
+                }
+            }
+            p = __builtin_amdgcn_readfirstlane(p); np = __builtin_amdgcn_readfirstlane(np);
+            mg = __builtin_amdgcn_readfirstlane(mg); err = __builtin_amdgcn_readfirstlane(err);
+            if (err) break;
+            __syncthreads();
+            const uint32_t upto = p < oe ? p : oe;
+            clear(clr, upto);
+            __threadfence();
+            for (uint32_t i = lane; i < np; i += 64u) {
+                const uint32_t q = ws + (uint32_t)patch[i];
+                atomicOr((uint32_t*)&B[q >> 5], 1u << (q & 31u));
+            }
+            __threadfence();
+            clr = upto;
+        }
+        if (err) return false;
+        if (lane == 0u) VF[s] = os;
+        e = mg ? X[s] : p;
+    }
+    return true;
+}
+}
+
 __global__ __launch_bounds__(64) void lzf_seg_seam_kernel(seg_ctx c) {
     __shared__ uint16_t patch[kSegStride / 3u + 8u];
-    constexpr uint32_t kWin = 2048;
-    __shared__ __attribute__((aligned(16))) uint8_t wbytes[kWin + 128u];
+    __shared__ __attribute__((aligned(16))) uint8_t wbytes[kWinStage];
     __shared__ uint32_t wbits[kWin / 32u + 2u];
     if (blockIdx.x >= c.g_n) return;
     const uint32_t j = c.grouped ? seg_job_of(c, blockIdx.x) : blockIdx.x;
@@ -379,6 +514,10 @@
     const lzf_decompress_job job = c.jobs[j];
     cgu8* __restrict__ in = as_global(job.input);
     const uint32_t len = (uint32_t)job.input_len;
+    if (c.fed) {
+        if (!seam_fed(c, j, lane, in, len, patch, wbytes, wbits) && lane == 0u) c.st[j].failed = 1u;
+        return;
+    }
     LZF_GLOBAL uint32_t* const X = (LZF_GLOBAL uint32_t*)c.xexit + (size_t)j * c.maxch;
     LZF_GLOBAL uint32_t* const VF = (LZF_GLOBAL uint32_t*)c.vfrom + (size_t)j * c.maxch;
     LZF_GLOBAL uint32_t* const B = (LZF_GLOBAL uint32_t*)c.bits + (size_t)j * c.maxch * kSegChunkWords;
@@ -422,37 +561,20 @@
                     const uint32_t ws = p;
                     __syncthreads();
                     {
-                        const uint32_t avail = len - ws < kWin + 128u ? len - ws : kWin + 128u;
-                        for (uint32_t i = lane * 16u; i < kWin + 128u; i += 1024u) {
-                            u32x4 v = u32x4{0, 0, 0, 0};
-                            if (i + 16u <= avail) v = ld16(in + ws + i);
-                            else if (i < avail) { for (uint32_t b = 0; i + b < avail; ++b) v[(b >> 2) & 3u] |= (uint32_t)in[ws + i + b] << ((b & 3u) * 8u); }
-                            *reinterpret_cast<u32x4*>(&wbytes[i]) = v;
-                        }
+                        seam_stage(wbytes, in, len, ws, lane);
                         const uint32_t w0 = (ws - base) >> 5;
                         for (uint32_t i = lane; i < kWin / 32u + 2u; i += 64u)
                             wbits[i] = w0 + i < kSegChunkWords ? B[(size_t)hk * kSegChunkWords + w0 + i] : 0u;
                     }
                     __syncthreads();
                     if (lane == 0u) {
-                        const uint32_t wb_a = lds_addr(wbytes);
-                        auto rdb = [&](uint32_t q) -> uint32_t { const uint32_t r_ = q - ws; if (r_ < kWin + 128u) return (uint32_t)wbytes[r_]; return (uint32_t)in[q]; };
-                        auto rd8 = [&](uint32_t q) -> uint64_t { const uint32_t r_ = q - ws; if (r_ + 8u <= kWin + 128u) return lds_ld64u(wb_a + r_); return ld8(in + q); };
                         const uint32_t bit0 = ((ws - base) >> 5) << 5;
                         while (p < endk && p < len && p - ws < kWin) {
                             const uint32_t rbit = p - base - bit0;
                             if (p != e_true && ((wbits[rbit >> 5] >> (rbit & 31u)) & 1u)) { mg = 1; break; }
                             patch[np++] = (uint16_t)(p - ostart);
                             uint32_t nx;
-                            {
-                                uint32_t w;
-                                asm volatile("ds_read_b32 %0, %1\n\ts_waitcnt lgkmcnt(0)" : "=v"(w) : "v"(wb_a + (p - ws)) : "memory");
-                                const uint32_t L0 = (w >> 4) & 15u, M0 = w & 15u, b1 = (w >> 8) & 255u;
-                                const uint32_t q2 = p + 1u + (L0 == 15u ? 1u + 15u + b1 : L0);
-                                if (!(L0 == 15u && b1 == 255u) && q2 + 3u <= len && q2 - ws + 3u <= kWin + 128u &&
-                                    !(M0 == 15u && wbytes[q2 + 2u - ws] == 255u)) { p = q2 + 2u + (M0 == 15u ? 1u : 0u); continue; }
-                            }
-                            if (!token_next_gen(len, p, nx, rd8, rdb)) { err = 1; break; }
+                            if (!seam_next(wbytes, ws, in, len, p, nx)) { err = 1; break; }
                             p = nx;
                         }
                     }
diff --git a/rust-lz-fear_amd/csrc/lzf_fed_parse_geometry.h b/rust-lz-fear_amd/csrc/lzf_fed_parse_geometry.h
--- /dev/null
+++ b/rust-lz-fear_amd/csrc/lzf_fed_parse_geometry.h
@@ -0,0 +1,50 @@
+#ifndef LZF_FED_PARSE_GEOMETRY_H
+#define LZF_FED_PARSE_GEOMETRY_H
+
+#include <stdint.h>
+
+#ifdef __HIPCC__
+#define LZF_GEOM_HD __host__ __device__
+#else
+#define LZF_GEOM_HD
+#endif
+
+namespace lzf_fedgeom {
+
+constexpr uint32_t kChunk = 16384;
+constexpr uint32_t kRegion = 256;
+constexpr uint32_t kRunUp = 2048;
+constexpr uint32_t kRunUpLanes = kRunUp / kRegion;
+constexpr uint32_t kMaxStretches = 64;
+
+constexpr uint32_t kStretchesMin = 4, kStretchesMax = 22, kParseWgPerCu = 256;
+LZF_GEOM_HD inline uint32_t stretches_for(uint32_t n, uint32_t n_cu) {
+    const uint64_t want = n ? ((uint64_t)kParseWgPerCu * n_cu + n - 1u) / n : kStretchesMax;
+    return want < kStretchesMin ? kStretchesMin : want > kStretchesMax ? kStretchesMax : (uint32_t)want;
+}
+
+LZF_GEOM_HD inline uint32_t row_words(uint32_t max_in) { return ((max_in + 2047u) / 2048u) * 64u; }
+
+LZF_GEOM_HD inline uint32_t chunks_per_stretch(uint32_t len, uint32_t S) {
+    if (len <= kChunk || S <= 1u) return len <= kChunk ? 1u : (len + kChunk - 1u) / kChunk;
+    const uint32_t share = (len - kRunUp + S - 1u) / S;
+    return (share + kRunUp + kChunk - 1u) / kChunk;
+}
+LZF_GEOM_HD inline uint32_t stretch_pitch(uint32_t per) { return per * kChunk - kRunUp; }
+LZF_GEOM_HD inline uint32_t parse_start(uint32_t per, uint32_t s) { return s * stretch_pitch(per); }
+LZF_GEOM_HD inline uint32_t own_start(uint32_t per, uint32_t s) { return s ? s * stretch_pitch(per) + kRunUp : 0u; }
+LZF_GEOM_HD inline uint64_t own_end64(uint32_t per, uint32_t s) { return (uint64_t)(s + 1u) * stretch_pitch(per) + kRunUp; }
+LZF_GEOM_HD inline uint32_t own_end(uint32_t len, uint32_t per, uint32_t s) { const uint64_t e = own_end64(per, s); return e < len ? (uint32_t)e : len; }
+LZF_GEOM_HD inline bool stretch_empty(uint32_t len, uint32_t per, uint32_t s) {
+    return s ? (uint64_t)s * stretch_pitch(per) + kRunUp >= len : len == 0u;
+}
+LZF_GEOM_HD inline uint64_t chunk_start64(uint32_t per, uint32_t s, uint32_t k) { return (uint64_t)s * stretch_pitch(per) + (uint64_t)k * kChunk; }
+LZF_GEOM_HD inline uint32_t first_store_lane(uint32_t s, uint32_t k) { return (s && k == 0u) ? kRunUpLanes : 0u; }
+LZF_GEOM_HD inline uint32_t map_word(uint32_t cstart, uint32_t lane) { return (cstart >> 5) + lane * (kRegion / 32u); }
+LZF_GEOM_HD inline bool lane_stores(uint32_t cstart, uint32_t lane, uint32_t s, uint32_t k, uint32_t words) {
+    return lane >= first_store_lane(s, k) && map_word(cstart, lane) < words;
+}
+
+}
+
+#endif
```
